# acids-ircam/RAVE

Measured on AMD Instinct MI355X. Metric: audio samples/sec/GPU (RAVE v2 training step, 44.1 kHz, n_signal=65536), higher is better.
Workload: dtype f32; 1 GPU; v2 config, batch 32 mono 44.1 kHz n_signal=65536, VAE-phase training step per GPU (--phase vae); global_batch=32, parallelism=dp1, phase=vae

## Files before the change

include/rave_hip.h:

```cpp
#ifndef RAVE_HIP_H
#define RAVE_HIP_H

#include <stddef.h>
#include <stdint.h>

#ifdef __cplusplus
extern "C" {
#endif

#define RH_VERSION 100

#define RH_OK 0
#define RH_ERR_INVALID (-1)
#define RH_ERR_UNSUPPORTED (-2)
#define RH_ERR_WORKSPACE (-3)

typedef void* rh_stream_t;

enum rh_act {
    RH_ACT_NONE = 0,
    RH_ACT_LEAKY = 1,
    RH_ACT_SNAKE = 2
};

typedef struct rh_conv1d_desc {
    int32_t batch;
    int32_t c_in;
    int32_t c_out;
    int32_t l_in;
    int32_t l_out;
    int32_t kernel;
    int32_t stride;
    int32_t dilation;
    int32_t pad_left;
    int32_t transposed;
    int32_t groups;
    int32_t inner;
    int32_t in_valid;
    int32_t act;
    float act_slope;
    int32_t out_act;
    float out_slope;
} rh_conv1d_desc;

int rh_version(void);
const char* rh_last_error(void);



int rh_weight_norm_fwd_f32(const float* v, const float* g, int64_t rows, int64_t cols, float* w,
                           float* norms, rh_stream_t stream);
int rh_weight_norm_bwd_f32(const float* dw, const float* v, const float* g, const float* norms,
                           int64_t rows, int64_t cols, float* dv, float* dg, rh_stream_t stream);
typedef struct rh_wn_bwd_item {
    const float* dw;
    const float* v;
    const float* g;
    const float* norms;
    float* dv;
    float* dg;
    int64_t rows;
    int64_t cols;
} rh_wn_bwd_item;
int rh_weight_norm_bwd_batched_f32(const rh_wn_bwd_item* items, int32_t n_items, rh_stream_t stream);
typedef struct rh_reduce_item {
    const float* part;
    float* out;
    int64_t n;
    int32_t Z;
    int32_t reserved;
} rh_reduce_item;
int rh_defer_reduce(rh_reduce_item* item);
int rh_reduce_partials_batched_f32(const rh_reduce_item* items, int32_t n_items, rh_stream_t stream);

int64_t rh_conv1d_packed_floats(const rh_conv1d_desc* d, int which);
int rh_conv1d_pack_f32(const rh_conv1d_desc* d, const float* w, float* wp_fwd, float* wp_bwd,
                       rh_stream_t stream);

int rh_conv1d_pack_wn_f32(const rh_conv1d_desc* d, const float* v, const float* g, float* norms,
                          float* scale, float* wp_fwd, float* wp_bwd, rh_stream_t stream);

int64_t rh_prep_item_bytes(void);
int64_t rh_prep_array_bytes(int32_t n);
int rh_prep_fill_item(const rh_conv1d_desc* d, const float* v, const float* g, float* norms, float* scale,
                      float* wp_fwd, float* wp_bwd, void* item_host);
int rh_prep_link(void* items_host, int32_t n, int64_t* total_rows, int64_t* total_blocks);
int rh_prep_run_f32(const void* items_dev, int32_t n, int64_t total_rows, int64_t total_blocks, rh_stream_t stream);


int rh_conv1d_fwd_f32(const rh_conv1d_desc* d, const float* x, const float* wp_fwd,
                      const float* bias, const float* snake_alpha, const float* residual,
                      float* y, void* workspace, int64_t workspace_bytes, rh_stream_t stream);
int64_t rh_conv1d_fwd_workspace_bytes(const rh_conv1d_desc* d);
int64_t rh_conv1d_bwd_data_workspace_bytes(const rh_conv1d_desc* d);
int rh_conv1d_kernel_family(const rh_conv1d_desc* d, int which, int has_bias, int has_add);
int rh_residual_unit_fused(const rh_conv1d_desc* d3, const rh_conv1d_desc* d1);
int rh_residual_unit_fwd_f32(const rh_conv1d_desc* d3, const rh_conv1d_desc* d1, const float* x, const float* wp3_fwd,
                             const float* wp1_fwd, float* h, float* y, rh_stream_t stream);

int rh_x6_uses_ranges(void);
int rh_x6_range_words(void);
int rh_x6_set_ranges(const uint32_t* in_a, const uint32_t* in_b, uint32_t* out, uint32_t* out2);
int rh_amax_f32(const float* x, int64_t n, uint32_t* slot, rh_stream_t stream);

int rh_conv1d_plan_info(const rh_conv1d_desc* d, int which, int has_bias, int has_add, int32_t* out8);
int rh_conv1d_bwd_weight_kernel_family(const rh_conv1d_desc* d);
int rh_conv1d_bwd_weight_plan_info(const rh_conv1d_desc* d, int32_t* out4);

int rh_conv1d_bwd_data_f32(const rh_conv1d_desc* d, const float* dy, const float* wp_bwd,
                           const float* x, const float* snake_alpha, const float* add, float* dx,
                           void* workspace, int64_t workspace_bytes, rh_stream_t stream);

int64_t rh_conv1d_workspace_bytes(const rh_conv1d_desc* d);
int rh_conv1d_bwd_weight_f32(const rh_conv1d_desc* d, const float* dy, const float* x,
                             const float* snake_alpha, float* dw, float* dbias, void* workspace,
                             int64_t workspace_bytes, rh_stream_t stream);
int rh_conv1d_bwd_weight_wn_f32(const rh_conv1d_desc* d, const float* dy, const float* x, const float* snake_alpha,
                                const float* v, const float* g, const float* norms, float* dw_scratch, float* dv,
                                float* dg, float* dbias, void* workspace, int64_t workspace_bytes, rh_stream_t stream);
int64_t rh_conv1d_bwd_weight_wn_fused_launches(void);


int rh_pqmf_analysis_fwd_f32(const float* x, const float* w, int32_t rows, int32_t t_len,
                             int32_t n_band, int32_t kernel, int32_t pad_left, int32_t n_frames,
                             float* y, rh_stream_t stream);
int rh_pqmf_analysis_bwd_f32(const float* dy, const float* w, int32_t rows, int32_t t_len,
                             int32_t n_band, int32_t kernel, int32_t pad_left, int32_t n_frames,
                             float* dx, rh_stream_t stream);
int rh_pqmf_synthesis_fwd_f32(const float* y, const float* w, int32_t rows, int32_t n_frames,
                              int32_t n_band, int32_t kernel, int32_t pad_left, int32_t n_out,
                              float* x, rh_stream_t stream);
int rh_pqmf_synthesis_bwd_f32(const float* dx, const float* w, int32_t rows, int32_t n_frames,
                              int32_t n_band, int32_t kernel, int32_t pad_left, int32_t n_out,
                              float* dy, rh_stream_t stream);

int rh_pqmf_fold_k1_f32(const float* in, const float* tab, int32_t rows, int32_t t_len, int32_t n_frames, int32_t o0,
                        float scale, float* out, rh_stream_t stream);
int rh_pqmf_fold_k2_f32(const float* in, const float* tab, int32_t rows, int32_t n_frames, int32_t n_out, int32_t dp,
                        float scale, float* out, rh_stream_t stream);


int rh_amp_tanh_fwd_f32(const float* x, int32_t batch, int32_t c, int32_t l, float* y,
                        rh_stream_t stream);
int rh_amp_tanh_bwd_f32(const float* dy, const float* x, int32_t batch, int32_t c, int32_t l,
                        float* dx, rh_stream_t stream);
int rh_act_fwd_f32(const float* x, const float* snake_alpha, int32_t act, float slope,
                   int32_t batch, int32_t c, int32_t l, float* y, rh_stream_t stream);
int64_t rh_snake_bwd_workspace_bytes(int32_t batch, int32_t c);
int rh_snake_bwd_f32(const float* dy, const float* x, const float* alpha, int32_t batch, int32_t c,
                     int32_t l, float* dx, float* dalpha, void* workspace, int64_t workspace_bytes,
                     rh_stream_t stream);
int rh_act_bwd_f32(const float* dy, const float* y, int32_t act, float slope, int64_t n, float* g, rh_stream_t stream);
int64_t rh_act_bwd_bias_workspace_bytes(int32_t M);
int rh_act_bwd_bias_f32(const float* dy, const float* y, int32_t act, float slope, int32_t B, int32_t M, int64_t plane, float* g,
                        float* dbias, void* workspace, int64_t workspace_bytes, rh_stream_t stream);
int rh_adain_stats_update_f32(const float* x, int64_t rows, int32_t l, const float* num_updates, float* mean_buf,
                              float* std_buf, rh_stream_t stream);
int rh_adain_transfer_f32(const float* x, int64_t rows, int32_t l, const float* mean_x, const float* std_x,
                          const float* mean_y, const float* std_y, float* y, rh_stream_t stream);
int rh_avgpool2_fwd_f32(const float* x, int64_t rows, int32_t l_in, float* y, rh_stream_t stream);
int rh_avgpool2_bwd_f32(const float* dy, int64_t rows, int32_t l_in, float* dx, rh_stream_t stream);


typedef struct rh_conv2d_desc {
    int32_t batch;
    int32_t c_in;
    int32_t c_out;
    int32_t h_in, w_in;
    int32_t h_out, w_out;
    int32_t kh, kw;
    int32_t sh, sw;
    int32_t dh, dw;
    int32_t ph, pw;
    int32_t act;
    float act_slope;
} rh_conv2d_desc;

int64_t rh_conv2d_packed_floats(const rh_conv2d_desc* d, int which);
int rh_conv2d_pack_f32(const rh_conv2d_desc* d, const float* w, float* wp_fwd, float* wp_bwd, rh_stream_t stream);
int rh_conv2d_fwd_f32(const rh_conv2d_desc* d, const float* x, const float* wp_fwd, const float* bias ,
                      float* y, rh_stream_t stream);
int rh_conv2d_bwd_data_f32(const rh_conv2d_desc* d, const float* dy, const float* y, const float* wp_bwd, float* dx,
                           rh_stream_t stream);
int rh_conv2d_plan_info(const rh_conv2d_desc* d, int32_t which, int64_t* out);
int rh_conv2d_bwd_weight_kernel_family(const rh_conv2d_desc* d);
int64_t rh_conv2d_workspace_bytes(const rh_conv2d_desc* d);
int rh_conv2d_bwd_weight_f32(const rh_conv2d_desc* d, const float* dy, const float* y, const float* x, float* dw,
                             float* dbias, void* workspace, int64_t workspace_bytes, rh_stream_t stream);


int64_t rh_vq_loss_partials(int64_t n_vectors);
int rh_vq_assign_f32(const float* x, const float* embed, int64_t n_vectors, int32_t dim, int32_t codebook_size,
                     int64_t* indices, float* residual, float* quantized_sum, float* loss_partials, rh_stream_t stream);
int64_t rh_vq_assign_workspace_bytes(int64_t n_vectors, int32_t dim, int32_t codebook_size);
int rh_vq_assign_ws_f32(const float* x, const float* embed, int64_t n_vectors, int32_t dim, int32_t codebook_size,
                        int64_t* indices, float* residual, float* quantized_sum, float* loss_partials, void* workspace,
                        int64_t workspace_bytes, rh_stream_t stream);
int rh_vq_ema_update_f32(const float* x, const int64_t* indices, int64_t n_vectors, int32_t dim, int32_t codebook_size,
                         float decay, float epsilon, float* cluster_size, float* embed_avg, float* embed,
                         rh_stream_t stream);


int rh_feed_batch_i16_f32(const int16_t* pcm, const int64_t* src_offset, const double* coef, const float* noise,
                          int32_t rows, int32_t n_signal, int32_t bit_depth, float* out, rh_stream_t stream);

typedef struct rh_feed_pitch_row {
    int64_t base;
    int64_t in_point;
    double mean;
    double coef[5];
    int32_t length;
    int32_t up, down;
    int32_t tap_offset;
    int32_t mute;
    int32_t reserved;
} rh_feed_pitch_row;
int rh_feed_batch_pitch_i16_f32(const int16_t* pcm, int64_t pcm_samples, const rh_feed_pitch_row* rows,
                                const rh_feed_pitch_row* rows_dev, const double* taps, int32_t n_taps, const float* noise,
                                int32_t n_rows, int32_t n_signal, int32_t bit_depth, float* out, rh_stream_t stream);


int rh_stft_frame_fwd_f32(const float* x, const float* window, int64_t rows, int32_t t_len, int32_t n_fft,
                          int32_t hop, int32_t n_frames, float* frames, rh_stream_t stream);
int rh_stft_frame_bwd_f32(const float* dframes, const float* window, int64_t rows, int32_t t_len, int32_t n_fft,
                          int32_t hop, int32_t n_frames, float* dx, rh_stream_t stream);
int rh_stft_frame_bwd_acc_f32(const float* dframes, const float* window, int64_t rows, int32_t t_len, int32_t n_fft,
                              int32_t hop, int32_t n_frames, float* dx, int32_t accumulate, rh_stream_t stream);

int64_t rh_spectral_distance_workspace_bytes(void);
int rh_spectral_distance_fwd_f32(const float* sx, const float* sy, int64_t n_complex, float eps, float* sums,
                                 void* workspace, int64_t workspace_bytes, rh_stream_t stream);
int rh_spectral_distance_bwd_f32(const float* sx, const float* sy, const float* sums, const float* grad_out,
                                 int64_t n_complex, float eps, float* dsx, float* dsy, int32_t half_bins,
                                 rh_stream_t stream);

int rh_spectral_total_f32(const float* sums, const float* inv_n, int32_t n_scales, float* out, rh_stream_t stream);

int rh_stft_loss_supported(int32_t n_fft, int32_t hop, int32_t t_len, int64_t rows);
int rh_stft_loss_plan_info(int32_t n_fft, int32_t t_len, int64_t rows, int64_t* out6);
int64_t rh_stft_loss_workspace_bytes(int32_t n_fft, int32_t t_len, int64_t rows);
int rh_stft_loss_fwd_f32(const float* x, const float* y, const float* window, const float* twiddle, int64_t rows,
                         int32_t t_len, int32_t n_fft, float eps, float* sums, void* workspace, int64_t workspace_bytes,
                         rh_stream_t stream);
int rh_stft_loss_finalize_all_f32(const float* const* partials, const int64_t* partial_bytes, int32_t n_scales,
                                  const float* inv_n, float* sums, float* total, rh_stream_t stream);
int rh_stft_loss_bwd_f32(const float* x, const float* y, const float* window, const float* twiddle, int64_t rows,
                         int32_t t_len, int32_t n_fft, float eps, const float* sums, const float* grad_out, float* dx,
                         float* dy, int32_t accumulate, rh_stream_t stream);

int rh_set_kernel_events(void* start_event, void* stop_event);
int rh_kernel_events_used(void);
int rh_event_create(void** event);
int rh_event_destroy(void* event);
int rh_event_elapsed_ms(void* start_event, void* stop_event, float* ms);

typedef struct rh_loss_item {
    const float* value;
    const float* w1_dev;
    float w1;
    float w2;
} rh_loss_item;
int rh_loss_combine_fwd_f32(const rh_loss_item* items, int32_t n_items, float* scaled, float* total, rh_stream_t stream);
int rh_loss_combine_bwd_f32(const rh_loss_item* items, int32_t n_items, const float* grad_total, float* grads,
                            rh_stream_t stream);

typedef struct rh_adam_item {
    float* p;
    const float* g;
    float* m;
    float* v;
    int64_t n;
    float* step;
} rh_adam_item;
int rh_adam_step_f32(const rh_adam_item* items, int32_t n_items, const float* lr, float beta1, float beta2, float eps,
                     float* aux, rh_stream_t stream);

typedef struct rh_pair_item {
    float* a;
    float* b;
    int64_t n;
} rh_pair_item;
int rh_ema_update_f32(const rh_pair_item* items, int32_t n_items, double factor, rh_stream_t stream);
int rh_swap_f32(const rh_pair_item* items, int32_t n_items, rh_stream_t stream);

typedef struct rh_fm_item {
    const float* f;
    float* df;
    int64_t half;
    float w;
} rh_fm_item;
int64_t rh_feature_matching_workspace_bytes(const rh_fm_item* items, int32_t n_items);
int rh_feature_matching_fwd_f32(const rh_fm_item* items, int32_t n_items, int32_t relative, void* workspace,
                                int64_t workspace_bytes, float* sums, float* out, rh_stream_t stream);
int rh_feature_matching_bwd_f32(const rh_fm_item* items, int32_t n_items, int32_t relative, const float* sums,
                                const float* grad_out, rh_stream_t stream);

int64_t rh_reparam_workspace_bytes(void);
int rh_reparam_fwd_f32(const float* z, const float* eps, int32_t batch, int32_t c, int32_t l, float* zs, float* kl,
                       void* workspace, int64_t workspace_bytes, rh_stream_t stream);
int rh_reparam_bwd_f32(const float* z, const float* eps, const float* dzs, const float* dkl, int32_t batch, int32_t c,
                       int32_t l, float* dz, rh_stream_t stream);

#ifdef __cplusplus
}
#endif
#endif
```

rave_amd/_lib.py:

```python
from __future__ import annotations

import ctypes as C
import os

import torch

_HERE = os.path.dirname(os.path.abspath(__file__))
LIB_PATH = os.environ.get("RAVE_HIP_LIB") or os.path.join(_HERE, "librave_hip.so")

ACT_NONE, ACT_LEAKY, ACT_SNAKE = 0, 1, 2


class ConvDesc(C.Structure):
    _fields_ = [
        ("batch", C.c_int32), ("c_in", C.c_int32), ("c_out", C.c_int32),
        ("l_in", C.c_int32), ("l_out", C.c_int32), ("kernel", C.c_int32),
        ("stride", C.c_int32), ("dilation", C.c_int32), ("pad_left", C.c_int32),
        ("transposed", C.c_int32), ("groups", C.c_int32), ("inner", C.c_int32),
        ("in_valid", C.c_int32), ("act", C.c_int32), ("act_slope", C.c_float),
        ("out_act", C.c_int32), ("out_slope", C.c_float),
    ]


class AdamItem(C.Structure):
    _fields_ = [("p", C.c_void_p), ("g", C.c_void_p), ("m", C.c_void_p), ("v", C.c_void_p), ("n", C.c_int64), ("step", C.c_void_p)]


class PairItem(C.Structure):
    _fields_ = [("a", C.c_void_p), ("b", C.c_void_p), ("n", C.c_int64)]


class WnBwdItem(C.Structure):
    _fields_ = [("dw", C.c_void_p), ("v", C.c_void_p), ("g", C.c_void_p), ("norms", C.c_void_p), ("dv", C.c_void_p),
                ("dg", C.c_void_p), ("rows", C.c_int64), ("cols", C.c_int64)]


class ReduceItem(C.Structure):
    _fields_ = [("part", C.c_void_p), ("out", C.c_void_p), ("n", C.c_int64), ("Z", C.c_int32), ("reserved", C.c_int32)]


class LossItem(C.Structure):
    _fields_ = [("value", C.c_void_p), ("w1_dev", C.c_void_p), ("w1", C.c_float), ("w2", C.c_float)]


class FmItem(C.Structure):
    _fields_ = [("f", C.c_void_p), ("df", C.c_void_p), ("half", C.c_int64), ("w", C.c_float)]


class Conv2dDesc(C.Structure):
    _fields_ = [(n, C.c_int32) for n in (
        "batch", "c_in", "c_out", "h_in", "w_in", "h_out", "w_out", "kh", "kw", "sh", "sw", "dh", "dw", "ph", "pw",
        "act")] + [("act_slope", C.c_float)]


def _load() -> C.CDLL:
    if not os.path.exists(LIB_PATH):
        raise RuntimeError(
            f"rave_amd: {LIB_PATH} not found. Build it with `python -m rave_amd.build` "
            "(or __graft_entry__.build()). There is no CPU / PyTorch fallback for the HIP hot path.")
    lib = C.CDLL(LIB_PATH)
    P, I32, I64, F = C.c_void_p, C.c_int32, C.c_int64, C.c_float
    D = C.POINTER(ConvDesc)
    D2 = C.POINTER(Conv2dDesc)
    sig = {
        "rh_version": ([], C.c_int),
        "rh_last_error": ([], C.c_char_p),
        "rh_weight_norm_fwd_f32": ([P, P, I64, I64, P, P, P], C.c_int),
        "rh_weight_norm_bwd_f32": ([P, P, P, P, I64, I64, P, P, P], C.c_int),
        "rh_weight_norm_bwd_batched_f32": ([C.POINTER(WnBwdItem), I32, P], C.c_int),
        "rh_defer_reduce": ([C.POINTER(ReduceItem)], C.c_int),
        "rh_reduce_partials_batched_f32": ([C.POINTER(ReduceItem), I32, P], C.c_int),
        "rh_conv1d_packed_floats": ([D, C.c_int], I64),
        "rh_conv1d_pack_f32": ([D, P, P, P, P], C.c_int),
        "rh_conv1d_pack_wn_f32": ([D, P, P, P, P, P, P, P], C.c_int),
        "rh_prep_item_bytes": ([], I64),
        "rh_prep_array_bytes": ([I32], I64),
        "rh_prep_fill_item": ([D, P, P, P, P, P, P, P], C.c_int),
        "rh_prep_link": ([P, I32, C.POINTER(I64), C.POINTER(I64)], C.c_int),
        "rh_prep_run_f32": ([P, I32, I64, I64, P], C.c_int),
        "rh_conv1d_fwd_f32": ([D, P, P, P, P, P, P, P, I64, P], C.c_int),
        "rh_conv1d_bwd_data_f32": ([D, P, P, P, P, P, P, P, I64, P], C.c_int),
        "rh_conv1d_kernel_family": ([D, C.c_int, C.c_int, C.c_int], C.c_int),
        "rh_conv1d_bwd_weight_kernel_family": ([D], C.c_int),
        "rh_conv1d_bwd_weight_plan_info": ([D, C.POINTER(C.c_int32)], C.c_int),
        "rh_residual_unit_fused": ([D, D], C.c_int),
        "rh_residual_unit_fwd_f32": ([D, D, P, P, P, P, P, P], C.c_int),
        "rh_conv1d_plan_info": ([D, C.c_int, C.c_int, C.c_int, C.POINTER(C.c_int32)], C.c_int),
        "rh_conv1d_fwd_workspace_bytes": ([D], I64),
        "rh_conv1d_bwd_data_workspace_bytes": ([D], I64),
        "rh_conv1d_workspace_bytes": ([D], I64),
        "rh_conv1d_bwd_weight_f32": ([D, P, P, P, P, P, P, I64, P], C.c_int),
        "rh_conv1d_bwd_weight_wn_f32": ([D, P, P, P, P, P, P, P, P, P, P, P, I64, P], C.c_int),
        "rh_conv1d_bwd_weight_wn_fused_launches": ([], I64),
        "rh_conv2d_packed_floats": ([D2, C.c_int], I64),
        "rh_conv2d_pack_f32": ([D2, P, P, P, P], C.c_int),
        "rh_conv2d_fwd_f32": ([D2, P, P, P, P, P], C.c_int),
        "rh_conv2d_bwd_data_f32": ([D2, P, P, P, P, P], C.c_int),
        "rh_conv2d_workspace_bytes": ([D2], I64),
        "rh_conv2d_plan_info": ([D2, I32, C.POINTER(I64)], C.c_int),
        "rh_conv2d_bwd_weight_kernel_family": ([D2], C.c_int),
        "rh_conv2d_bwd_weight_f32": ([D2, P, P, P, P, P, P, I64, P], C.c_int),
        "rh_feed_batch_i16_f32": ([P, P, P, P, I32, I32, I32, P, P], C.c_int),
        "rh_feed_batch_pitch_i16_f32": ([P, I64, P, P, P, I32, P, I32, I32, I32, P, P], C.c_int),
        "rh_vq_loss_partials": ([I64], I64),
        "rh_vq_assign_f32": ([P, P, I64, I32, I32, P, P, P, P, P], C.c_int),
        "rh_vq_assign_workspace_bytes": ([I64, I32, I32], I64),
        "rh_vq_assign_ws_f32": ([P, P, I64, I32, I32, P, P, P, P, P, I64, P], C.c_int),
        "rh_vq_ema_update_f32": ([P, P, I64, I32, I32, F, F, P, P, P, P], C.c_int),
        "rh_pqmf_analysis_fwd_f32": ([P, P, I32, I32, I32, I32, I32, I32, P, P], C.c_int),
        "rh_pqmf_analysis_bwd_f32": ([P, P, I32, I32, I32, I32, I32, I32, P, P], C.c_int),
        "rh_pqmf_synthesis_fwd_f32": ([P, P, I32, I32, I32, I32, I32, I32, P, P], C.c_int),
        "rh_pqmf_synthesis_bwd_f32": ([P, P, I32, I32, I32, I32, I32, I32, P, P], C.c_int),
        "rh_pqmf_fold_k1_f32": ([P, P, I32, I32, I32, I32, F, P, P], C.c_int),
        "rh_pqmf_fold_k2_f32": ([P, P, I32, I32, I32, I32, F, P, P], C.c_int),
        "rh_amp_tanh_fwd_f32": ([P, I32, I32, I32, P, P], C.c_int),
        "rh_amp_tanh_bwd_f32": ([P, P, I32, I32, I32, P, P], C.c_int),
        "rh_act_fwd_f32": ([P, P, I32, F, I32, I32, I32, P, P], C.c_int),
        "rh_act_bwd_f32": ([P, P, I32, F, I64, P, P], C.c_int),
        "rh_act_bwd_bias_workspace_bytes": ([I32], I64),
        "rh_act_bwd_bias_f32": ([P, P, I32, F, I32, I32, I64, P, P, P, I64, P], C.c_int),
        "rh_snake_bwd_workspace_bytes": ([I32, I32], I64),
        "rh_snake_bwd_f32": ([P, P, P, I32, I32, I32, P, P, P, I64, P], C.c_int),
        "rh_stft_frame_fwd_f32": ([P, P, I64, I32, I32, I32, I32, P, P], C.c_int),
        "rh_stft_frame_bwd_f32": ([P, P, I64, I32, I32, I32, I32, P, P], C.c_int),
        "rh_stft_frame_bwd_acc_f32": ([P, P, I64, I32, I32, I32, I32, P, I32, P], C.c_int),
        "rh_spectral_total_f32": ([P, P, I32, P, P], C.c_int),
        "rh_feature_matching_workspace_bytes": ([C.POINTER(FmItem), I32], I64),
        "rh_feature_matching_fwd_f32": ([C.POINTER(FmItem), I32, I32, P, I64, P, P, P], C.c_int),
        "rh_feature_matching_bwd_f32": ([C.POINTER(FmItem), I32, I32, P, P, P], C.c_int),
        "rh_reparam_workspace_bytes": ([], I64),
        "rh_reparam_fwd_f32": ([P, P, I32, I32, I32, P, P, P, I64, P], C.c_int),
        "rh_reparam_bwd_f32": ([P, P, P, P, I32, I32, I32, P, P], C.c_int),
        "rh_loss_combine_fwd_f32": ([C.POINTER(LossItem), I32, P, P, P], C.c_int),
        "rh_loss_combine_bwd_f32": ([C.POINTER(LossItem), I32, P, P, P], C.c_int),
        "rh_adam_step_f32": ([C.POINTER(AdamItem), I32, P, F, F, F, P, P], C.c_int),
        "rh_ema_update_f32": ([C.POINTER(PairItem), I32, C.c_double, P], C.c_int),
        "rh_swap_f32": ([C.POINTER(PairItem), I32, P], C.c_int),
        "rh_x6_uses_ranges": ([], C.c_int),
        "rh_x6_range_words": ([], C.c_int),
        "rh_x6_set_ranges": ([P, P, P, P], C.c_int),
        "rh_amax_f32": ([P, I64, P, P], C.c_int),
        "rh_set_kernel_events": ([P, P], C.c_int),
        "rh_kernel_events_used": ([], C.c_int),
        "rh_event_create": ([C.POINTER(C.c_void_p)], C.c_int),
        "rh_event_destroy": ([P], C.c_int),
        "rh_event_elapsed_ms": ([P, P, C.POINTER(C.c_float)], C.c_int),
        "rh_stft_loss_supported": ([I32, I32, I32, I64], C.c_int),
        "rh_stft_loss_plan_info": ([I32, I32, I64, C.POINTER(I64)], C.c_int),
        "rh_stft_loss_workspace_bytes": ([I32, I32, I64], I64),
        "rh_stft_loss_fwd_f32": ([P, P, P, P, I64, I32, I32, F, P, P, I64, P], C.c_int),
        "rh_stft_loss_finalize_all_f32": ([C.POINTER(C.c_void_p), C.POINTER(I64), I32, P, P, P, P], C.c_int),
        "rh_stft_loss_bwd_f32": ([P, P, P, P, I64, I32, I32, F, P, P, P, P, I32, P], C.c_int),
        "rh_spectral_distance_workspace_bytes": ([], I64),
        "rh_spectral_distance_fwd_f32": ([P, P, I64, F, P, P, I64, P], C.c_int),
        "rh_spectral_distance_bwd_f32": ([P, P, P, P, I64, F, P, P, I32, P], C.c_int),
        "rh_adain_stats_update_f32": ([P, I64, I32, P, P, P, P], C.c_int),
        "rh_adain_transfer_f32": ([P, I64, I32, P, P, P, P, P, P], C.c_int),
        "rh_avgpool2_fwd_f32": ([P, I64, I32, P, P], C.c_int),
        "rh_avgpool2_bwd_f32": ([P, I64, I32, P, P], C.c_int),
    }
    for name, (args, res) in sig.items():
        fn = getattr(lib, name)
        fn.argtypes = args
        fn.restype = res
    return lib


lib = _load()


def check(rc: int, what: str = "") -> None:
    if rc != 0:
        msg = lib.rh_last_error().decode(errors="replace")
        raise RuntimeError(f"librave_hip {what} failed (code {rc}): {msg}")


def ptr(t) -> int | None:
    return None if t is None else t.data_ptr()


def stream() -> int:
    return torch.cuda.current_stream().cuda_stream
```

rave_amd/csrc/conv_host.hip:

```cpp
#include "conv_params.hpp"

int64_t rh_wgrad_workspace(const rh_conv1d_desc* d);

namespace {

struct TapPlan {
    int nphase = 0;
    int oph[kMaxPhases], ntaps[kMaxPhases], tap0[kMaxPhases], minoff[kMaxPhases], maxoff[kMaxPhases];
    int nslots = 0;
    int kk[kMaxTaps], off[kMaxTaps];
    int is = 1, os = 1;
    int rows = 0;
    int C = 0, M = 0;
    bool src_m_major = true;
};

int validate(const rh_conv1d_desc* d) {
    RH_REQUIRE(d, RH_ERR_INVALID, "conv1d: null descriptor");
    RH_REQUIRE(d->batch >= 0 && d->c_in > 0 && d->c_out > 0 && d->l_in >= 0 && d->l_out >= 0,
               RH_ERR_INVALID, "conv1d: bad sizes");
    RH_REQUIRE(d->kernel >= 1 && d->stride >= 1 && d->dilation >= 1 && d->inner >= 1,
               RH_ERR_INVALID, "conv1d: kernel/stride/dilation/inner must be >= 1");
    RH_REQUIRE(d->groups == 1, RH_ERR_UNSUPPORTED, "conv1d: groups = %d not implemented", d->groups);
    RH_REQUIRE(d->kernel <= kMaxTaps, RH_ERR_UNSUPPORTED, "conv1d: kernel %d > %d", d->kernel, kMaxTaps);
// ... 506 lines not shown
    p->ncols = t.rows * d->inner;
    p->in_act = RH_ACT_NONE;
    p->in_slope = 0.f;
    p->epi_act = d->act;
    p->epi_slope = d->act_slope;
    p->out_act = RH_ACT_NONE;
    p->out_slope = 0.f;
    plan_to_x6(t, d->inner, p);
    return RH_OK;
}

extern "C" int64_t rh_conv1d_packed_floats(const rh_conv1d_desc* d, int which) {
    if (validate(d)) return -1;
    const int64_t M = which == 0 ? d->c_out : d->c_in;
    const int64_t C = which == 0 ? d->c_in : d->c_out;
    const int64_t n32 = (int64_t)d->kernel * C * round32((int)M);
    TapPlan t;
    if (build_plan(d, which, &t)) return -1;
    const long units = x6_units(t, x6_mode_of(t, d->inner), nullptr, d->inner);
    return (units > 0 && units * 4 < 0x7fffffffl) ? n32 + units * 4 + 4 : n32;
}

extern "C" int rh_conv1d_pack_f32(const rh_conv1d_desc* d, const float* w, float* wp_fwd,
                                  float* wp_bwd, rh_stream_t stream) {
    if (int e = validate(d)) return e;
    RH_REQUIRE(w, RH_ERR_INVALID, "conv1d_pack: null weight");
    return pack_both(d, w, nullptr, wp_fwd, wp_bwd, (hipStream_t)stream);
}

int rh_weight_norm_scales(const float* v, const float* g, int64_t rows, int64_t cols, float* norms, float* scale,
                          hipStream_t stream);

struct PrepItem {
    const float* v;
    const float* g;
    float* norms;
    float* scale;
    PackP fwd, bwd;
    long rows, cols;
    long row_begin;
    long blk_begin;
};

namespace {

__device__ __forceinline__ int find_item(const PrepItem* items, int n, long key, bool rows) {
    const long* tab = reinterpret_cast<const long*>(items + n) + (rows ? 0 : n);
    int lo = 0, hi = n - 1;
    while (lo < hi) {
        const int mid = (lo + hi + 1) >> 1;
        if (tab[mid] <= key) lo = mid; else hi = mid - 1;
    }
    return lo;
}

__global__ __launch_bounds__(256) void prep_range_kernel(const PrepItem* __restrict__ items, int n) {
    __shared__ float red[8];
    const PrepItem& p = items[blockIdx.x];
    float mx = 0.f, l1 = 0.f;
    for (long r = threadIdx.x; r < p.rows; r += 256) { mx = fmaxf(mx, p.scale[p.rows + r]); l1 = fmaxf(l1, p.scale[2 * p.rows + r]); }
#pragma unroll
    for (int o = 32; o > 0; o >>= 1) { mx = fmaxf(mx, __shfl_down(mx, o, 64)); l1 = fmaxf(l1, __shfl_down(l1, o, 64)); }
    if ((threadIdx.x & 63) == 0) { red[threadIdx.x >> 6] = mx; red[4 + (threadIdx.x >> 6)] = l1; }
    __syncthreads();
    if (threadIdx.x == 0) {
        const unsigned m = __float_as_uint(fmaxf(fmaxf(red[0], red[1]), fmaxf(red[2], red[3])));
        const unsigned l = __float_as_uint(fmaxf(fmaxf(red[4], red[5]), fmaxf(red[6], red[7])));
        for (unsigned* r : {p.fwd.range, p.bwd.range})
            if (r) { r[0] = m; r[1] = l; r[2] = 0u; r[3] = 0u; }
    }
}

__global__ __launch_bounds__(256) void prep_scales_kernel(const PrepItem* __restrict__ items, int n) {
    __shared__ float red[12];
    const int it = find_item(items, n, blockIdx.x, true);
    const PrepItem& p = items[it];
    const long r = (long)blockIdx.x - p.row_begin;
    const float* vr = p.v + r * p.cols;
    float s = 0.f, mx = 0.f, sm = 0.f;
    long e = threadIdx.x;
    for (; e + 768 < p.cols; e += 1024) {
        const float a0 = vr[e], a1 = vr[e + 256], a2 = vr[e + 512], a3 = vr[e + 768];
        s += a0 * a0; s += a1 * a1; s += a2 * a2; s += a3 * a3;
        mx = fmaxf(fmaxf(mx, fmaxf(fabsf(a0), fabsf(a1))), fmaxf(fabsf(a2), fabsf(a3)));
        sm += fabsf(a0); sm += fabsf(a1); sm += fabsf(a2); sm += fabsf(a3);
    }
    for (; e < p.cols; e += 256) {
        const float a = vr[e];
        s += a * a;
        mx = fmaxf(mx, fabsf(a));
        sm += fabsf(a);
    }
#pragma unroll
    for (int o = 32; o > 0; o >>= 1) {
        s += __shfl_down(s, o, 64);
        mx = fmaxf(mx, __shfl_down(mx, o, 64));
        sm += __shfl_down(sm, o, 64);
    }
    if ((threadIdx.x & 63) == 0) { red[threadIdx.x >> 6] = s; red[4 + (threadIdx.x >> 6)] = mx; red[8 + (threadIdx.x >> 6)] = sm; }
    __syncthreads();
    if (threadIdx.x == 0) {
        const float norm = sqrtf(red[0] + red[1] + red[2] + red[3]);
        const float sc = p.g[r] / norm;
        p.norms[r] = norm;
        p.scale[r] = sc;
        const float m = fabsf(sc) * fmaxf(fmaxf(red[4], red[5]), fmaxf(red[6], red[7]));
        const float l1 = fabsf(sc) * ((red[8] + red[9]) + (red[10] + red[11]));
        p.scale[p.rows + r] = m;
        p.scale[2 * p.rows + r] = l1;
    }
}

__global__ __launch_bounds__(256) void prep_pack_kernel(const PrepItem* __restrict__ items, int n) {
    __shared__ float lds[kPackSlots * 32 * 33];
    const int it = find_item(items, n, blockIdx.x, false);
    const PrepItem& p = items[it];
    const long t = (long)blockIdx.x - p.blk_begin;
    const long nf = pack_tiles(p.fwd);
    if (t < nf) pack_tile(p.fwd, t, lds);
    else if (t - nf < pack_tiles(p.bwd)) pack_tile(p.bwd, t - nf, lds);
}

}

extern "C" int64_t rh_prep_item_bytes(void) { return (int64_t)sizeof(PrepItem); }
extern "C" int64_t rh_prep_array_bytes(int32_t n) { return (int64_t)n * (int64_t)sizeof(PrepItem) + 2 * (int64_t)n * (int64_t)sizeof(long); }

extern "C" int rh_prep_fill_item(const rh_conv1d_desc* d, const float* v, const float* g, float* norms, float* scale,
                                 float* wp_fwd, float* wp_bwd, void* item) {
    if (int e = validate(d)) return e;
    RH_REQUIRE(v && g && norms && scale && wp_fwd && item, RH_ERR_INVALID, "prep_fill_item: null pointer");
    PrepItem* p = (PrepItem*)item;
    *p = PrepItem{};
    p->v = v; p->g = g; p->norms = norms; p->scale = scale;
    p->rows = d->transposed ? d->c_in : d->c_out;
    p->cols = (long)(d->transposed ? d->c_out : d->c_in) * d->kernel;
    if (int e = fill_pack(d, 0, v, scale, wp_fwd, &p->fwd)) return e;
    if (int e = fill_pack(d, 1, v, scale, wp_bwd, &p->bwd)) return e;
    return RH_OK;
}

extern "C" int rh_prep_link(void* items, int32_t n, int64_t* total_rows, int64_t* total_blocks) {
    RH_REQUIRE(items && total_rows && total_blocks && n >= 0, RH_ERR_INVALID, "prep_link: bad arguments");
    PrepItem* p = (PrepItem*)items;
    long rows = 0, blks = 0;
    for (int i = 0; i < n; ++i) {
        p[i].row_begin = rows;
        p[i].blk_begin = blks;
        rows += p[i].rows;
        for (const PackP* q : {&p[i].fwd, &p[i].bwd}) blks += pack_tiles(*q);
    }
    long* tab = reinterpret_cast<long*>(p + n);
    for (int i = 0; i < n; ++i) { tab[i] = p[i].row_begin; tab[n + i] = p[i].blk_begin; }
    *total_rows = rows;
    *total_blocks = blks;
    return RH_OK;
}

extern "C" int rh_prep_run_f32(const void* items_dev, int32_t n, int64_t total_rows, int64_t total_blocks,
                               rh_stream_t stream) {
    RH_REQUIRE(items_dev && n > 0, RH_ERR_INVALID, "prep_run: bad arguments");
    if (total_rows > 0) {
        hipLaunchKernelGGL(prep_scales_kernel, dim3((unsigned)total_rows), dim3(256), 0, (hipStream_t)stream,
                           (const PrepItem*)items_dev, n);
        if (int e = rh_check_launch("prep_scales")) return e;
        hipLaunchKernelGGL(prep_range_kernel, dim3((unsigned)n), dim3(256), 0, (hipStream_t)stream, (const PrepItem*)items_dev, n);
        if (int e = rh_check_launch("prep_range")) return e;
    }
    if (total_blocks > 0) {
        hipLaunchKernelGGL(prep_pack_kernel, dim3((unsigned)total_blocks), dim3(256), 0, (hipStream_t)stream,
                           (const PrepItem*)items_dev, n);
        return rh_check_launch("prep_pack");
    }
    return RH_OK;
}

extern "C" int rh_conv1d_pack_wn_f32(const rh_conv1d_desc* d, const float* v, const float* g, float* norms,
                                     float* scale, float* wp_fwd, float* wp_bwd, rh_stream_t stream) {
    if (int e = validate(d)) return e;
    RH_REQUIRE(v && g && norms && scale, RH_ERR_INVALID, "conv1d_pack_wn: null pointer");
    const int64_t rows = d->transposed ? d->c_in : d->c_out;
    const int64_t cols = (int64_t)(d->transposed ? d->c_out : d->c_in) * d->kernel;
    if (int e = rh_weight_norm_scales(v, g, rows, cols, norms, scale, (hipStream_t)stream)) return e;
    return pack_both(d, v, scale, wp_fwd, wp_bwd, (hipStream_t)stream);
}

extern "C" int64_t rh_conv1d_fwd_workspace_bytes(const rh_conv1d_desc* d) {
    ConvP p{};
    if (rh_conv_fill_fwd(d, &p)) return -1;
    return rh_conv_splitk_workspace(p);
}

extern "C" int64_t rh_conv1d_bwd_data_workspace_bytes(const rh_conv1d_desc* d) {
    ConvP p{};
    if (rh_conv_fill_dgrad(d, &p)) return -1;
    p.epi_act = d->act;
    return rh_conv_splitk_workspace(p);
}

extern "C" int rh_conv1d_kernel_family(const rh_conv1d_desc* d, int which, int has_bias, int has_add) {
    ConvP p{};
    if (int e = which == 0 ? rh_conv_fill_fwd(d, &p) : rh_conv_fill_dgrad(d, &p)) return e;
    if (which == 0 ? rh_smallc_fwd_eligible(d, has_add != 0) : rh_smallc_dgrad_eligible(d, has_add != 0)) return 2;
    alignas(16) static const float dummy[4] = {0.f, 0.f, 0.f, 0.f};
    p.in = dummy; p.wp = dummy; p.wq = reinterpret_cast<const unsigned*>(dummy);
    p.bias = has_bias ? dummy : nullptr;
    p.add = has_add ? dummy : nullptr;
    p.mul_src = (which == 1 && d->act != RH_ACT_NONE) ? dummy : nullptr;
    if (p.B <= 0 || p.ncols <= 0 || p.M <= 0 || !rh_conv_dma_eligible(p)) return 0;
    return (rh_conv_x6_workspace(p) >= 0 || rh_conv_c2x_query(p)) ? 1 : 0;
}

extern "C" int rh_conv1d_plan_info(const rh_conv1d_desc* d, int which, int has_bias, int has_add, int32_t* out8) {
    RH_REQUIRE(out8, RH_ERR_INVALID, "conv1d_plan_info: null output");
    for (int i = 0; i < 8; ++i) out8[i] = 0;
    ConvP p{};
    if (int e = which == 0 ? rh_conv_fill_fwd(d, &p) : rh_conv_fill_dgrad(d, &p)) return e;
    if (which == 0 ? rh_smallc_fwd_eligible(d, has_add != 0) : rh_smallc_dgrad_eligible(d, has_add != 0)) { out8[0] = 2; return RH_OK; }
    alignas(16) static const float dummy[4] = {0.f, 0.f, 0.f, 0.f};
    p.in = dummy; p.wp = dummy; p.wq = reinterpret_cast<const unsigned*>(dummy);
    p.bias = has_bias ? dummy : nullptr;
    p.add = has_add ? dummy : nullptr;
    p.mul_src = (which == 1 && d->act != RH_ACT_NONE) ? dummy : nullptr;
    if (p.B <= 0 || p.ncols <= 0 || p.M <= 0 || !rh_conv_dma_eligible(p)) return RH_OK;
    int q[7];
    if (rh_conv_x6_plan_query(p, q)) {
        out8[0] = 1;
        for (int i = 0; i < 7; ++i) out8[i + 1] = q[i];
    }
    return RH_OK;
}

extern "C" int rh_conv1d_fwd_f32(const rh_conv1d_desc* d, const float* x, const float* wp_fwd,
                                 const float* bias, const float* snake_alpha, const float* residual,
                                 float* y, void* workspace, int64_t workspace_bytes, rh_stream_t stream) {
    const RhKernelEventsScope events;
    ConvP p{};
    rh_take_ranges(nullptr, &p.in_range, &p.out_range, nullptr);
    const unsigned* const in_range = p.in_range;
    unsigned* const out_range = p.out_range;
    if (int e = rh_conv_fill_fwd(d, &p)) return e;
    p.in_range = in_range; p.out_range = out_range;
    if (d->batch == 0 || d->l_out == 0) return RH_OK;
    RH_REQUIRE(x && wp_fwd && y, RH_ERR_INVALID, "conv1d_fwd: null pointer");
    RH_REQUIRE(d->act != RH_ACT_SNAKE || snake_alpha, RH_ERR_INVALID, "conv1d_fwd: snake needs alpha");
    if (rh_smallc_fwd_eligible(d, residual != nullptr)) {
        return rh_smallc_fwd(d, x, wp_fwd, bias, y, (hipStream_t)stream, p.out_range);
    }
    p.in = x; p.wp = wp_fwd; p.out = y; p.bias = bias; p.add = residual; p.mul_src = nullptr;
    p.wq = reinterpret_cast<const unsigned*>(wp_fwd + p.x6_wofs);
    p.in_alpha = snake_alpha; p.mul_alpha = nullptr;
    return rh_conv_launch(p, (hipStream_t)stream, d->transposed ? "conv_transpose1d_fwd" : "conv1d_fwd", workspace,
                          workspace_bytes);
}

extern "C" int rh_conv1d_bwd_data_f32(const rh_conv1d_desc* d, const float* dy, const float* wp_bwd,
                                      const float* x, const float* snake_alpha, const float* add,
                                      float* dx, void* workspace, int64_t workspace_bytes,
                                      rh_stream_t stream) {
    const RhKernelEventsScope events;
    ConvP p{};
    rh_take_ranges(nullptr, &p.in_range, &p.out_range, nullptr);
    const unsigned* const in_range = p.in_range;
    unsigned* const out_range = p.out_range;
    if (int e = rh_conv_fill_dgrad(d, &p)) return e;
    p.in_range = in_range; p.out_range = out_range;
    if (d->batch == 0 || d->l_in == 0) return RH_OK;
    RH_REQUIRE(dy && wp_bwd && dx, RH_ERR_INVALID, "conv1d_bwd_data: null pointer");
    RH_REQUIRE(d->act == RH_ACT_NONE || x, RH_ERR_INVALID, "conv1d_bwd_data: act needs the forward input");
    RH_REQUIRE(d->act != RH_ACT_SNAKE || snake_alpha, RH_ERR_INVALID, "conv1d_bwd_data: snake needs alpha");
    if (rh_smallc_dgrad_eligible(d, add != nullptr)) {
        TapPlan t;
        if (int e = build_plan(d, 1, &t)) return e;
        int slot_of_tap[kMaxTaps];
        for (int i = 0; i < t.nslots; ++i) slot_of_tap[t.kk[i]] = i;
        if (int e = rh_smallc_dgrad(d, dy, wp_bwd, slot_of_tap, dx, (hipStream_t)stream)) return e;
        p.out = dx;
        return rh_range_after(p, (hipStream_t)stream);
    }
    p.in = dy; p.wp = wp_bwd; p.out = dx; p.bias = nullptr; p.add = add;
    p.wq = reinterpret_cast<const unsigned*>(wp_bwd + p.x6_wofs);
    p.mul_src = d->act == RH_ACT_NONE ? nullptr : x;
    p.in_alpha = nullptr; p.mul_alpha = snake_alpha;
    return rh_conv_launch(p, (hipStream_t)stream, d->transposed ? "conv_transpose1d_bwd_data" : "conv1d_bwd_data",
                          workspace, workspace_bytes);
}

extern "C" int64_t rh_conv1d_workspace_bytes(const rh_conv1d_desc* d) {
    if (validate(d)) return -1;
    return rh_wgrad_workspace(d);
}

extern "C" int rh_conv1d_bwd_weight_f32(const rh_conv1d_desc* d, const float* dy, const float* x,
                                        const float* snake_alpha, float* dw, float* dbias,
                                        void* workspace, int64_t workspace_bytes, rh_stream_t stream) {
    const RhKernelEventsScope events;
    const RhWgradArmed armed = rh_wgrad_take_armed(true);
    if (int e = validate(d)) return e;
    RH_REQUIRE(dw && (d->batch == 0 || (dy && x)), RH_ERR_INVALID, "conv1d_bwd_weight: null pointer");
    RH_REQUIRE(d->act != RH_ACT_SNAKE || snake_alpha, RH_ERR_INVALID, "conv1d_bwd_weight: snake needs alpha");
    return rh_wgrad_run(d, dy, x, snake_alpha, dw, dbias, workspace, workspace_bytes, (hipStream_t)stream, armed);
}

extern "C" int rh_conv1d_bwd_weight_wn_f32(const rh_conv1d_desc* d, const float* dy, const float* x, const float* snake_alpha,
                                           const float* v, const float* g, const float* norms, float* dw_scratch, float* dv,
                                           float* dg, float* dbias, void* workspace, int64_t workspace_bytes, rh_stream_t stream) {
    const RhKernelEventsScope events;
    const RhWgradArmed armed = rh_wgrad_take_armed(false);
    if (int e = validate(d)) return e;
    RH_REQUIRE(dw_scratch && v && g && norms && dv && dg && (d->batch == 0 || (dy && x)), RH_ERR_INVALID,
               "conv1d_bwd_weight_wn: null pointer");
    RH_REQUIRE(d->act != RH_ACT_SNAKE || snake_alpha, RH_ERR_INVALID, "conv1d_bwd_weight_wn: snake needs alpha");
    const RhWnTail tail{v, g, norms, dv, dg};
    return rh_wgrad_run(d, dy, x, snake_alpha, dw_scratch, dbias, workspace, workspace_bytes, (hipStream_t)stream, armed, &tail);
}
```

rave_amd/csrc/conv_params.hpp:

```cpp
#pragma once
#include "common.hpp"

constexpr int kMaxPhases = 8;
constexpr int kMaxTaps = 64;

struct ConvP {
    const float* in;
    const float* wp;
    float* out;
    const float* bias;
    const float* mul_src;
    const float* add;
    const float* in_alpha;
    const float* mul_alpha;
    int B, C, M, Mp;
    int in_row, in_valid, out_row, out_valid;
    int ncols, inner, is, os;
    int bnl, bnl_shift, nb, tiles_per_b;
    int pitch;
    int ck;
    int wlds_floats;
    int in_act, epi_act, out_act;
    float in_slope, epi_slope, out_slope;
    int segs;
    unsigned magic_segs, magic_ck, magic_lpr;
    int stage_floats;
    int ksplit;
    int chunks_per_split;
    float* part;
    unsigned* tickets;
    long part_stride;
    unsigned in_bytes, w_bytes;
    const unsigned* wq;
    unsigned wq_bytes;
    const unsigned* in_range;
    unsigned* out_range;
    const unsigned* w_range;
    int x6_mode;
    int x6_P;
    int x6_a_units, x6_b_units;
    int x6_nu;
    int v_s;
    long v_q2ofs;
    int vs;
    int Mr;
    int v_o0;
    int v_U, v_b0;
    long ph_q2ofs[kMaxPhases];
    long x6_wofs;
    int nphase;
    int ph_oph[kMaxPhases], ph_ntaps[kMaxPhases], ph_tap0[kMaxPhases], ph_minoff[kMaxPhases],
        ph_maxoff[kMaxPhases];
    long ph_wofs[kMaxPhases];
    int off[kMaxTaps];
};

struct WgradP {
    const float* R;
    const float* S;
    float* out;
    const float* r_alpha;
    const float* s_alpha;
    int B, M, C, T;
    int r_row;
    int s_row, s_valid;
    int inner, is;
    int r_act, s_act;
    float r_slope, s_slope;
    int rk;
    int chunks_per_b;
    int total_chunks;
    int chunks_per_z;
    int pr;
    int ps;
    int nc_max;
    int minoff, maxoff;
    unsigned magic_ps, magic_cpb, magic_pr, magic_lpr_r, magic_lpr_s;
    int vec;
    int r_floats, s_floats;
    int stage_floats;
    unsigned r_bytes, s_bytes;
    int off[kMaxTaps];
};

struct PackP {
    const float* w;
    const float* scale;
    float* wp;
    unsigned* wq;
    unsigned* range;
    long total;
    int C, M, Mp, k;
    int nslots;
    int m_major;
    int x6_mode;
    int x6_nu;
    int bf16x3;
    int x6_vs, x6_U, x6_Mvp, vz_n;
    long x6_vofs;
    int q2j[kMaxTaps], vq2a[kMaxTaps];
    int vz_j[2 * kMaxPhases], vz_u[2 * kMaxPhases];
    int kk[kMaxTaps];
    int q2a[kMaxTaps];
    int q2n[kMaxTaps];
};
int rh_pack_launch(const PackP& a, const PackP& b, hipStream_t stream, const char* what, const float* w = nullptr, long rows = 0,
                   long cols = 0);
int64_t rh_bias_grad_workspace(int M);
int rh_bias_grad_launch(const float* dy, const float* y, float* part, float* db, int B, int M, long plane, int act,
                        float slope, hipStream_t stream, float* g_out = nullptr, unsigned* g_range = nullptr);
int rh_reduce_partials_launch(const float* part, float* out, long n, int Z, hipStream_t stream, const char* what);
struct RhWnTail {
    const float* v;
    const float* g;
    const float* norms;
    float* dv;
    float* dg;
};
struct RhWgradArmed {
    rh_reduce_item* defer;
    const unsigned* dy_range;
    const unsigned* x_range;
};
RhWgradArmed rh_wgrad_take_armed(bool may_defer);
int rh_wgrad_run(const rh_conv1d_desc* d, const float* dy, const float* x, const float* alpha, float* dw, float* dbias, void* ws,
                 int64_t ws_bytes, hipStream_t stream, const RhWgradArmed& armed, const RhWnTail* tail = nullptr);

int rh_conv_fill_fwd(const rh_conv1d_desc* d, ConvP* p);
int rh_conv_fill_dgrad(const rh_conv1d_desc* d, ConvP* p);
int rh_conv_launch(ConvP& p, hipStream_t stream, const char* what, void* ws = nullptr, int64_t ws_bytes = 0);
int rh_conv_launch_sync(ConvP& p, hipStream_t stream, const char* what);
int rh_range_after(const ConvP& p, hipStream_t stream);
int rh_conv_launch_dma(ConvP& p, hipStream_t stream, const char* what, void* ws, int64_t ws_bytes);
bool rh_conv_dma_eligible(const ConvP& p);
int64_t rh_conv_splitk_workspace(ConvP p);
int64_t rh_conv_x6_workspace(ConvP p);
inline int rh_x6_mode(int C, int nphase, int is, int inner, int ntaps0, const int* off, const int* kk) {
    if (is == 1) return (C & 15) == 0 ? 1 : 0;
    if (is == 3) return (nphase == 1 && inner == 1 && (C & 15) == 0) ? 1 : 0;
    if (nphase != 1 || inner != 1 || (is != 2 && is != 4) || (C * is) % 16 != 0) return 0;
    for (int t = 0; t < ntaps0; ++t)
        if (off[t] != off[0] + t || kk[t] != t) return 0;
    return is;
}
inline bool rh_x6_epi_instantiated(int is, int tm, bool leaky, int epi) {
    const int m = epi & 15, v = epi >> 4;
    if (v) {
        if (is != 1 || tm < 2 || v > 2) return false;
        return leaky ? (m == 0 || m == 1 || m == 5) : (m == 0 || m == 1 || m == 2 || m == 4 || m == 5 || m == 6);
    }
    return leaky ? (m == 0 || m == 1 || m == 4 || m == 5) : (m == 0 || m == 1 || m == 2 || m == 4 || m == 5 || m == 6 || m == 9 || m == 13);
}
int rh_conv_launch_x6(ConvP& p, hipStream_t stream, const char* what, void* ws, int64_t ws_bytes, bool* used);
int rh_conv_launch_c2x(ConvP& p, hipStream_t stream, const char* what, bool* used);
bool rh_conv_c2x_query(ConvP p);
bool rh_conv_x6_plan_query(ConvP p, int* out7);

bool rh_smallc_fwd_eligible(const rh_conv1d_desc* d, bool has_residual);
int rh_smallc_fwd(const rh_conv1d_desc* d, const float* x, const float* wp_fwd, const float* bias, float* y, hipStream_t stream,
                  unsigned* out_range = nullptr);
bool rh_smallc_dgrad_eligible(const rh_conv1d_desc* d, bool has_add);
int rh_smallc_dgrad(const rh_conv1d_desc* d, const float* dy, const float* wp_bwd, const int* slot_of_tap, float* dx,
                    hipStream_t stream);
bool rh_smallc_wgrad_eligible(const rh_conv1d_desc* d);
int64_t rh_smallc_wgrad_workspace(const rh_conv1d_desc* d);
int rh_smallc_wgrad(const rh_conv1d_desc* d, const float* dy, const float* x, float* dw, float* dbias, void* ws,
                    hipStream_t stream);
```

rave_amd/csrc/conv_wgrad.hip:

```cpp
#include <atomic>
#include <cstdlib>
#include <mutex>
#include "conv_params.hpp"

namespace {

template <int TM, int TN, int WM, int WN>
__global__ __launch_bounds__(WM* WN * 64) void wgrad_kernel(const WgradP p) {
    constexpr int BM = TM * WM * 32, BN = TN * WN * 32;
    constexpr int NW = WM * WN;
    extern __shared__ __attribute__((aligned(16))) float smem[];
    float* r_lds = smem;
    float* s_lds = smem + BM * p.pr;

    const int tid = threadIdx.x, lane = tid & 63, wave = tid >> 6;
    const int j = lane & 31, kh = lane >> 5;
    const int wm = wave / WN, wn = wave - wm * WN;
    const int m0 = blockIdx.y * BM, col0 = blockIdx.x * BN, z = blockIdx.z;
    const int ncols = p.C * p.T;
    const int inner = p.inner, is = p.is;
    const int c_lo = col0 / p.T;

    int sb[TN], ar[TM];
#pragma unroll
// ... 378 lines not shown
        const int lo = q0 * is + p.minoff;
        const bool interior = (q0 + p.rk <= r_rows) && lo >= 0 && lo + 4 * ((s_width + 3) >> 2) <= p.s_valid;
        if (!interior) { issue(ch, stage); return; }
        const unsigned rbase = (b * p.M) * (unsigned)p.r_row + (unsigned)q0;
        const unsigned sbase = (b * p.C) * (unsigned)p.s_row + (unsigned)lo;
        float* ss = stage + p.r_floats;
#pragma unroll
        for (int i = 0; i < kNI; ++i) {
            if (i < ni_r && (wave + NW * i) * 256 < p.r_floats) {
                const unsigned off = rc[i] == kOOB ? kOOB : (rbase + rc[i]) * 4u;
                __builtin_amdgcn_raw_ptr_buffer_load_lds(r_rsrc, (lds_void*)(stage + (wave + NW * i) * 256), 16, off, 0, 0, 0);
            }
        }
#pragma unroll
        for (int i = 0; i < kNI; ++i) {
            if (i < ni_s && (wave + NW * i) * 256 < p.s_floats) {
                const unsigned off = sc[i] == kOOB ? kOOB : (sbase + sc[i]) * 4u;
                __builtin_amdgcn_raw_ptr_buffer_load_lds(s_rsrc, (lds_void*)(ss + (wave + NW * i) * 256), 16, off, 0, 0, 0);
            }
        }
    };

    const int ch0 = z * p.chunks_per_z;
    const int nch = min(p.chunks_per_z, p.total_chunks - ch0);
    if (nch > 0) issue_any(ch0, smem);
    for (int i = 0; i < nch; ++i) {
        asm volatile("s_waitcnt vmcnt(0)" ::: "memory");
        __syncthreads();
        if (i + 1 < nch) issue_any(ch0 + i + 1, smem + ((i + 1) & 1) * p.stage_floats);
        const float* r_lds = smem + (i & 1) * p.stage_floats;
        const float* s_lds = r_lds + p.r_floats;
        for (int w = 0; w < inner; ++w) {
            const float* rl = r_lds + w;
            const float* sl = s_lds + w;
            int rr = 0;
            if (p.vec) {
                for (; rr + 8 <= p.rk; rr += 8) {
                    f32x4 a4[TM];
                    float bb[4][TN];
#pragma unroll
                    for (int tm = 0; tm < TM; ++tm)
                        a4[tm] = *reinterpret_cast<const f32x4*>(rl + ar[tm] - kh + rr + 4 * kh);
#pragma unroll
                    for (int u = 0; u < 4; ++u)
#pragma unroll
                        for (int tn = 0; tn < TN; ++tn) bb[u][tn] = sl[sb[tn] - kh * is + (rr + 4 * kh + u) * is];
                    __builtin_amdgcn_sched_barrier(0);
#pragma unroll
                    for (int u = 0; u < 4; ++u) {
#pragma unroll
                        for (int tn = 0; tn < TN; ++tn)
                            if (SLEAKY) bb[u][tn] = bb[u][tn] > 0.f ? bb[u][tn] : bb[u][tn] * p.s_slope;
#pragma unroll
                        for (int tm = 0; tm < TM; ++tm) {
                            float av = a4[tm][u];
                            if (RLEAKY) av = av > 0.f ? av : av * p.r_slope;
#pragma unroll
                            for (int tn = 0; tn < TN; ++tn)
                                acc[tm][tn] = __builtin_amdgcn_mfma_f32_32x32x2f32(av, bb[u][tn], acc[tm][tn], 0, 0, 0);
                        }
                    }
                    __builtin_amdgcn_sched_barrier(0);
                }
            }
            for (; rr + 8 <= p.rk; rr += 8) {
                float a[4][TM], bb[4][TN];
#pragma unroll
                for (int u = 0; u < 4; ++u) {
#pragma unroll
                    for (int tm = 0; tm < TM; ++tm) a[u][tm] = rl[ar[tm] + (rr + 2 * u) * inner];
#pragma unroll
                    for (int tn = 0; tn < TN; ++tn) bb[u][tn] = sl[sb[tn] + (rr + 2 * u) * is * inner];
                }
                __builtin_amdgcn_sched_barrier(0);
#pragma unroll
                for (int u = 0; u < 4; ++u) {
#pragma unroll
                    for (int tm = 0; tm < TM; ++tm)
                        if (RLEAKY) a[u][tm] = a[u][tm] > 0.f ? a[u][tm] : a[u][tm] * p.r_slope;
#pragma unroll
                    for (int tn = 0; tn < TN; ++tn)
                        if (SLEAKY) bb[u][tn] = bb[u][tn] > 0.f ? bb[u][tn] : bb[u][tn] * p.s_slope;
#pragma unroll
                    for (int tm = 0; tm < TM; ++tm)
#pragma unroll
                        for (int tn = 0; tn < TN; ++tn)
                            acc[tm][tn] = __builtin_amdgcn_mfma_f32_32x32x2f32(a[u][tm], bb[u][tn], acc[tm][tn], 0, 0, 0);
                }
                __builtin_amdgcn_sched_barrier(0);
            }
            for (; rr < p.rk; rr += 2) {
                float a[TM], bb[TN];
#pragma unroll
                for (int tm = 0; tm < TM; ++tm) {
                    float v = rl[ar[tm] + rr * inner];
                    if (RLEAKY) v = v > 0.f ? v : v * p.r_slope;
                    a[tm] = v;
                }
#pragma unroll
                for (int tn = 0; tn < TN; ++tn) {
                    float v = sl[sb[tn] + rr * is * inner];
                    if (SLEAKY) v = v > 0.f ? v : v * p.s_slope;
                    bb[tn] = v;
                }
#pragma unroll
                for (int tm = 0; tm < TM; ++tm)
#pragma unroll
                    for (int tn = 0; tn < TN; ++tn)
                        acc[tm][tn] = __builtin_amdgcn_mfma_f32_32x32x2f32(a[tm], bb[tn], acc[tm][tn], 0, 0, 0);
            }
        }
    }
    float* out = p.out + (long)z * p.M * ncols;
#pragma unroll
    for (int tn = 0; tn < TN; ++tn) {
        const int col = col0 + (wn * TN + tn) * 32 + j;
        if (col >= ncols) continue;
#pragma unroll
        for (int tm = 0; tm < TM; ++tm)
#pragma unroll
            for (int r = 0; r < 16; ++r) {
                const int m = m0 + (wm * TM + tm) * 32 + (r & 3) + 8 * (r >> 2) + 4 * kh;
                if (m < p.M) out[(long)m * ncols + col] = acc[tm][tn][r];
            }
    }
}

struct WPlan {
    int bm, bn, mt, ct, Z, rk, chunks_per_b, total_chunks, chunks_per_z;
};

void fill(const rh_conv1d_desc* d, WgradP* p) {
    const int k = d->kernel;
    p->B = d->batch;
    p->T = k;
    p->inner = d->inner;
    p->is = d->stride;
    const int x_valid = d->in_valid ? d->in_valid : d->l_in * d->inner;
    if (!d->transposed) {
        p->M = d->c_out; p->C = d->c_in;
        p->r_row = d->l_out * d->inner;
        p->s_row = x_valid; p->s_valid = x_valid;
        p->r_act = RH_ACT_NONE; p->s_act = d->act;
        p->r_slope = 0.f; p->s_slope = d->act_slope;
        for (int t = 0; t < k; ++t) p->off[t] = t * d->dilation - d->pad_left;
    } else {
        p->M = d->c_in; p->C = d->c_out;
        p->r_row = d->l_in;
        p->s_row = d->l_out; p->s_valid = d->l_out;
        p->r_act = d->act; p->s_act = RH_ACT_NONE;
        p->r_slope = d->act_slope; p->s_slope = 0.f;
        for (int t = 0; t < k; ++t) p->off[t] = t - d->pad_left;
    }
    int lo = p->off[0], hi = p->off[0];
    for (int t = 1; t < k; ++t) { lo = lo < p->off[t] ? lo : p->off[t]; hi = hi > p->off[t] ? hi : p->off[t]; }
    p->minoff = lo; p->maxoff = hi;
}

void tile_of(int M, int ncols, int* bm, int* bn) {
    if (M <= 32) { *bm = 32; *bn = 256; }
    else if (M <= 64) { *bm = 64; *bn = 128; }
    else if (M % 96 == 0 || M < 96) {
        *bm = 96;
        *bn = (ncols % 96 == 0 && ncols % 128 != 0) ? 96 : 128;
    }
    else { *bm = 128; *bn = 128; }
}

WPlan plan(const WgradP& p) {
    WPlan w{};
    tile_of(p.M, p.C * p.T, &w.bm, &w.bn);
    w.mt = rh_cdiv(p.M, w.bm);
    w.ct = rh_cdiv(p.C * p.T, w.bn);
    static const int rk_env = [] { const char* e = getenv("RH_WGRAD_RK"); return e ? atoi(e) : 0; }();
    static const int rk_inner_env = [] { const char* e = getenv("RH_WGRAD_RK_INNER"); return e ? atoi(e) : 0; }();
    int rk = ((rk_env > 0 ? rk_env : 32) / p.inner) & ~1;
    if (p.inner > 1) rk = ((rk_inner_env > 0 ? rk_inner_env : 32) / p.inner) & ~1;
    if (rk < 2) rk = 2;
    const int r_rows = p.r_row / p.inner;
    if (r_rows < rk) rk = (r_rows + 1) & ~1;
    if (rk < 2) rk = 2;
    w.rk = rk;
    w.chunks_per_b = rh_cdiv(r_rows, rk);
    w.total_chunks = p.B * w.chunks_per_b;
    static const int ztarget = [] { const char* e = getenv("RH_WGRAD_BLOCKS"); return e ? atoi(e) : 1024; }();
    static const int zmin_chunks = [] { const char* e = getenv("RH_WGRAD_MINCHUNKS"); return e ? atoi(e) : 16; }();
    int Z = ztarget / (w.mt * w.ct);
    const int zmax = w.total_chunks / (rk * p.inner >= 64 ? zmin_chunks / 2 : zmin_chunks);
    if (Z > zmax) Z = zmax;
    if (Z < 1) Z = 1;
    w.chunks_per_z = rh_cdiv(w.total_chunks, Z);
    w.Z = rh_cdiv(w.total_chunks, w.chunks_per_z);
    if (w.Z < 1) w.Z = 1;
    return w;
}

inline unsigned magic_of(int d) { return d <= 1 ? 0u : (unsigned)(((1ull << 32) + d - 1) / (unsigned long long)d); }

template <int TM, int TN, int WM, int WN>
int launch_w(WgradP& p, const WPlan& w, hipStream_t stream) {
    constexpr int BM = TM * WM * 32, BN = TN * WN * 32;
    p.rk = w.rk;
    p.chunks_per_b = w.chunks_per_b;
    p.total_chunks = w.total_chunks;
    p.chunks_per_z = w.chunks_per_z;
    {
        const unsigned long long rb = 4ull * p.B * p.M * (unsigned long long)p.r_row;
        const unsigned long long sbytes = 4ull * p.B * p.C * (unsigned long long)p.s_row;
        const bool ok = p.r_act != RH_ACT_SNAKE && p.s_act != RH_ACT_SNAKE && rb < 0x7fffffffull &&
                        sbytes < 0x7fffffffull && w.rk * p.inner <= 64 && w.total_chunks < 32768;
        if (ok) {
            p.nc_max = (BN - 1) / p.T + 2;
            if (p.nc_max > p.C) p.nc_max = p.C;
            const int s_width = ((w.rk - 1) * p.is + (p.maxoff - p.minoff) + 1) * p.inner;
            static const int novec = [] { const char* e = getenv("RH_WGRAD_NOVEC"); return e ? atoi(e) : 0; }();
            p.vec = !novec && p.inner == 1 && (w.rk % 4) == 0 && (p.r_row % 4) == 0 && (p.s_row % 4) == 0 &&
                    ((uintptr_t)p.R % 16) == 0 && ((uintptr_t)p.S % 16) == 0;
            if (p.vec) {
                p.pr = w.rk + 4;
                p.ps = ((s_width + 3) & ~3) + 4;
                if ((p.ps & 31) == 0) p.ps += 4;
                const int ni_r = rh_cdiv(BM * (p.pr >> 2), 64 * WM * WN);
                const int ni_s = rh_cdiv(p.nc_max * (p.ps >> 2), 64 * WM * WN);
                if (ni_r > 12 || ni_s > 12) p.vec = 0;
            }
            if (!p.vec) {
                p.ps = s_width | 1;
                p.pr = (w.rk * p.inner) | 1;
            }
            p.magic_pr = magic_of(p.pr);
            p.magic_lpr_r = magic_of(p.pr >> 2);
            p.magic_lpr_s = magic_of(p.ps >> 2);
            p.r_floats = (BM * p.pr + 255) & ~255;
            p.s_floats = (p.nc_max * p.ps + 255) & ~255;
            p.stage_floats = p.r_floats + p.s_floats;
            p.magic_ps = magic_of(p.ps);
            p.magic_cpb = magic_of(w.chunks_per_b);
            p.r_bytes = (unsigned)rb;
            p.s_bytes = (unsigned)sbytes;
            const size_t lds = sizeof(float) * 2 * (size_t)p.stage_floats;
            if (lds <= 160 * 1024 && (unsigned)p.s_floats < (1u << 15)) {
                dim3 grid(w.ct, w.mt, w.Z);
                auto go = [&](auto kern) {
                    static std::once_flag once;
                    std::call_once(once, [&] { (void)hipFuncSetAttribute(reinterpret_cast<const void*>(kern), hipFuncAttributeMaxDynamicSharedMemorySize, 160 * 1024); });
                    rh_launch_main(kern, grid, dim3(WM * WN * 64), lds, stream, p);
                };
                if (p.r_act == RH_ACT_LEAKY) go(wgrad_dma_kernel<TM, TN, WM, WN, true, false>);
                else if (p.s_act == RH_ACT_LEAKY) go(wgrad_dma_kernel<TM, TN, WM, WN, false, true>);
                else go(wgrad_dma_kernel<TM, TN, WM, WN, false, false>);
                return rh_check_launch("conv1d_bwd_weight(dma)");
            }
        }
    }
    p.pr = (w.rk * p.inner) | 1;
    p.ps = (((w.rk - 1) * p.is + (p.maxoff - p.minoff) + 1) * p.inner) | 1;
    p.nc_max = (BN - 1) / p.T + 2;
    if (p.nc_max > p.C) p.nc_max = p.C;
    const size_t lds = sizeof(float) * ((size_t)BM * p.pr + (size_t)p.nc_max * p.ps);
    RH_REQUIRE(lds <= 160 * 1024, RH_ERR_UNSUPPORTED, "conv1d_bwd_weight: tile needs %zu B of LDS", lds);
    auto kern = wgrad_kernel<TM, TN, WM, WN>;
    static std::once_flag once;
    std::call_once(once, [&] {
        (void)hipFuncSetAttribute(reinterpret_cast<const void*>(kern),
                                  hipFuncAttributeMaxDynamicSharedMemorySize, 160 * 1024);
    });
    dim3 grid(w.ct, w.mt, w.Z);
    rh_launch_main(kern, grid, dim3(WM * WN * 64), lds, stream, p);
    return rh_check_launch("conv1d_bwd_weight");
}

}

int64_t rh_wgrad_x6_workspace(const WgradP& w);
int rh_wgrad_x6_launch(const WgradP& w, float* dw, float* rsum_out, void* ws, hipStream_t stream, bool* used, int* left_z,
                       const unsigned* r_range, const unsigned* s_range);
int rh_reduce_wn_bwd_launch(const float* part, int Z, long M, long N, const float* v, const float* g, const float* norms,
                            float* dv, float* dg, hipStream_t stream, bool* used);

extern "C" int rh_conv1d_bwd_weight_kernel_family(const rh_conv1d_desc* d) {
    if (!d || d->batch <= 0) return 0;
    WgradP p{};
    fill(d, &p);
    if (rh_smallc_wgrad_eligible(d)) return 2;
    alignas(16) static const float dummy[4] = {0.f, 0.f, 0.f, 0.f};
    p.R = dummy; p.S = dummy;
    return d->act != RH_ACT_SNAKE && rh_wgrad_x6_workspace(p) >= 0 ? 1 : 0;
}

bool rh_wgrad_x6_plan_info(const WgradP& w, int32_t* out4);

extern "C" int rh_conv1d_bwd_weight_plan_info(const rh_conv1d_desc* d, int32_t* out4) {
    if (!d || !out4) return RH_ERR_INVALID;
    for (int i = 0; i < 4; ++i) out4[i] = 0;
    if (d->batch <= 0 || rh_conv1d_bwd_weight_kernel_family(d) != 1) return RH_OK;
    WgradP p{};
    fill(d, &p);
    alignas(16) static const float dummy[4] = {0.f, 0.f, 0.f, 0.f};
    p.R = dummy; p.S = dummy;
    (void)rh_wgrad_x6_plan_info(p, out4);
    return RH_OK;
}

int64_t rh_wgrad_workspace(const rh_conv1d_desc* d) {
    WgradP p{};
    fill(d, &p);
    const int64_t bias = rh_bias_grad_workspace(d->c_out);
    if (rh_smallc_wgrad_eligible(d)) return bias + rh_smallc_wgrad_workspace(d);
    int64_t x6 = -1;
    if (d->act != RH_ACT_SNAKE) {
        x6 = rh_wgrad_x6_workspace(p);
        if (x6 >= 0 && !RH_X6_F16) return bias + x6;
    }
    const WPlan w = plan(p);
    const int64_t f32 = w.Z <= 1 ? 0 : (int64_t)w.Z * p.M * p.C * p.T * (int64_t)sizeof(float);
    return bias + (x6 > f32 ? x6 : f32);
}

extern "C" int rh_weight_norm_bwd_f32(const float* dw, const float* v, const float* g, const float* norms, int64_t rows,
                                      int64_t cols, float* dv, float* dg, rh_stream_t stream);

thread_local rh_reduce_item* g_defer_item = nullptr;
extern "C" int rh_defer_reduce(rh_reduce_item* item) {
    g_defer_item = item;
    if (item) *item = rh_reduce_item{};
    return RH_OK;
}

extern "C" int rh_reduce_partials_batched_f32(const rh_reduce_item* items, int32_t n_items, rh_stream_t stream) {
    RH_REQUIRE(n_items >= 0 && (n_items == 0 || items), RH_ERR_INVALID, "reduce_partials_batched: bad arguments");
    for (int i0 = 0; i0 < n_items; i0 += kReduceBatch) {
        ReduceTable tb{};
        long blocks = 0;
        for (int i = i0; i < n_items && i < i0 + kReduceBatch; ++i) {
            const rh_reduce_item& q = items[i];
            if (q.Z <= 0 || q.n <= 0) continue;
            RH_REQUIRE(q.part && q.out, RH_ERR_INVALID, "reduce_partials_batched: null pointer in item %d", i);
            const int k = tb.items++;
            tb.part[k] = q.part; tb.out[k] = q.out; tb.Z[k] = q.Z;
            tb.vec4[k] = reduce_is_vec4(q.part, q.out, q.n, q.Z) ? 1 : 0;
            tb.n[k] = tb.vec4[k] ? q.n / 4 : q.n;
            tb.blk_begin[k] = blocks;
            blocks += tb.vec4[k] ? rh_cdiv64(tb.n[k], 256) : rh_cdiv64(q.n, 64);
        }
        if (tb.items == 0) continue;
        tb.blk_begin[tb.items] = blocks;
        RH_REQUIRE(blocks < 0x7fffffffl, RH_ERR_UNSUPPORTED, "reduce_partials_batched: too many workgroups");
        hipLaunchKernelGGL(reduce_partials_batched_kernel, dim3((unsigned)blocks), dim3(256), 0, (hipStream_t)stream, tb);
        if (int e = rh_check_launch("reduce_partials_batched")) return e;
    }
    return RH_OK;
}

RhWgradArmed rh_wgrad_take_armed(bool may_defer) {
    RhWgradArmed a{may_defer ? g_defer_item : nullptr, nullptr, nullptr};
    g_defer_item = nullptr;
    rh_take_ranges(&a.dy_range, &a.x_range, nullptr, nullptr);
    return a;
}

int rh_wgrad_run(const rh_conv1d_desc* d, const float* dy, const float* x, const float* alpha,
                 float* dw, float* dbias, void* ws, int64_t ws_bytes, hipStream_t stream, const RhWgradArmed& armed,
                 const RhWnTail* tail) {
    rh_reduce_item* const defer = tail ? nullptr : armed.defer;
    WgradP p{};
    fill(d, &p);
    const unsigned* const dy_range = armed.dy_range;
    const unsigned* const x_range = armed.x_range;
    const bool have_ranges = !RH_X6_F16 || (dy_range && x_range);
    auto through_dw = [&](int e) {
        if (e || !tail) return e;
        return rh_weight_norm_bwd_f32(dw, tail->v, tail->g, tail->norms, p.M, (int64_t)p.C * p.T, tail->dv, tail->dg, (rh_stream_t)stream);
    };
    if (!d->transposed) { p.R = dy; p.S = x; p.r_alpha = nullptr; p.s_alpha = alpha; }
    else                { p.R = x; p.S = dy; p.r_alpha = alpha; p.s_alpha = nullptr; }
    const long nw = (long)p.M * p.C * p.T;
    const int64_t bias_ws = rh_bias_grad_workspace(d->c_out);
    if (rh_smallc_wgrad_eligible(d)) {
        const int64_t need = rh_smallc_wgrad_workspace(d);
        RH_REQUIRE(ws && ws_bytes >= need, RH_ERR_WORKSPACE, "conv1d_bwd_weight: workspace %lld B < %lld B",
                   (long long)ws_bytes, (long long)need);
        return through_dw(rh_smallc_wgrad(d, dy, x, dw, dbias, ws, stream));
    }
    const bool x6_path = have_ranges && d->act != RH_ACT_SNAKE && p.B > 0 && p.r_row > 0 && rh_wgrad_x6_workspace(p) >= 0;
    const bool fuse_bias = x6_path && !d->transposed && dbias != nullptr;
    if (dbias && d->batch > 0 && !fuse_bias) {
        RH_REQUIRE(ws && ws_bytes >= bias_ws, RH_ERR_WORKSPACE, "conv1d_bwd_weight: workspace %lld B < %lld B",
                   (long long)ws_bytes, (long long)bias_ws);
        if (int e = rh_bias_grad_launch(dy, nullptr, (float*)ws, dbias, d->batch, d->c_out,
                                        (long)d->l_out * d->inner, RH_ACT_NONE, 0.f, stream))
            return e;
    }
    ws = ws ? (void*)((char*)ws + bias_ws) : nullptr;
    ws_bytes = ws_bytes > bias_ws ? ws_bytes - bias_ws : 0;
    if (p.B <= 0 || p.r_row <= 0) {
        (void)hipMemsetAsync(dw, 0, nw * sizeof(float), stream);
        if (dbias) (void)hipMemsetAsync(dbias, 0, d->c_out * sizeof(float), stream);
        return through_dw(RH_OK);
    }
    if (d->act != RH_ACT_SNAKE && have_ranges) {
        const int64_t x6 = rh_wgrad_x6_workspace(p);
        if (x6 >= 0) {
            RH_REQUIRE(x6 == 0 || (ws && ws_bytes >= x6), RH_ERR_WORKSPACE,
                       "conv1d_bwd_weight: workspace %lld B < %lld B", (long long)ws_bytes, (long long)x6);
            bool used = false;
            int left_z = 0;
            if (int e = rh_wgrad_x6_launch(p, dw, fuse_bias ? dbias : nullptr, ws, stream, &used, (tail || defer) ? &left_z : nullptr,
                                           d->transposed ? x_range : dy_range, d->transposed ? dy_range : x_range))
                return e;
            if (used && left_z > 1 && defer) {
                defer->part = (const float*)ws; defer->out = dw; defer->n = nw; defer->Z = left_z;
                return RH_OK;
            }
            if (used && left_z > 1) {
                bool fused = false;
                if (int e = rh_reduce_wn_bwd_launch((const float*)ws, left_z, p.M, (long)p.C * p.T, tail->v, tail->g, tail->norms,
                                                    tail->dv, tail->dg, stream, &fused))
                    return e;
                if (fused) return RH_OK;
                return through_dw(rh_reduce_partials_launch((const float*)ws, dw, nw, left_z, stream, "conv1d_bwd_weight_reduce"));
            }
            if (used) return through_dw(RH_OK);
        }
    }
    const WPlan w = plan(p);
    const int64_t need = w.Z > 1 ? (int64_t)w.Z * nw * (int64_t)sizeof(float) : 0;
    RH_REQUIRE(need == 0 || (ws && ws_bytes >= need), RH_ERR_WORKSPACE,
               "conv1d_bwd_weight: workspace %lld B < %lld B", (long long)ws_bytes, (long long)need);
    p.out = w.Z > 1 ? (float*)ws : dw;
    int e;
    if (w.bm == 32) e = launch_w<1, 2, 1, 4>(p, w, stream);
    else if (w.bm == 64) e = launch_w<2, 1, 1, 4>(p, w, stream);
    else if (w.bm == 96 && w.bn == 96) e = launch_w<3, 1, 1, 3>(p, w, stream);
    else if (w.bm == 96) e = launch_w<3, 1, 1, 4>(p, w, stream);
    else e = launch_w<2, 2, 2, 2>(p, w, stream);
    if (e) return e;
    if (w.Z > 1) {
        if (tail) {
            bool fused = false;
            if (int e2 = rh_reduce_wn_bwd_launch((const float*)ws, w.Z, p.M, nw / p.M, tail->v, tail->g, tail->norms, tail->dv,
                                                 tail->dg, stream, &fused))
                return e2;
            if (fused) return RH_OK;
        }
        if (defer) {
            defer->part = (const float*)ws; defer->out = dw; defer->n = nw; defer->Z = w.Z;
            return RH_OK;
        }
        reduce_partials_go((const float*)ws, dw, nw, w.Z, stream);
        return through_dw(rh_check_launch("conv1d_bwd_weight_reduce"));
    }
    return through_dw(RH_OK);
}

int rh_reduce_partials_launch(const float* part, float* out, long n, int Z, hipStream_t stream, const char* what) {
    if (n <= 0) return RH_OK;
    reduce_partials_go(part, out, n, Z, stream);
    return rh_check_launch(what);
}

static std::atomic<int64_t> g_rwn_launches{0};
int rh_reduce_wn_bwd_launch(const float* part, int Z, long M, long N, const float* v, const float* g, const float* norms,
                            float* dv, float* dg, hipStream_t stream, bool* used) {
    *used = false;
    const char* e = getenv("RH_WN_FUSED");
    if (!(e && atoi(e) == 1)) return RH_OK;
    if (Z < 2 || M <= 0 || N <= 0 || (N & 3) || N > kRwnMaxN || ((uintptr_t)part & 15)) return RH_OK;
    const long n = M * N;
    const int order4 = Z <= 16 && n >= (1l << 16);
    hipLaunchKernelGGL(reduce_wn_bwd_kernel, dim3((unsigned)M), dim3(1024), (size_t)(4096 + N) * sizeof(float), stream, part, n, Z,
                       (int)N, order4, v, g, norms, dv, dg);
    *used = true;
    ++g_rwn_launches;
    return rh_check_launch("conv1d_bwd_weight_reduce_wn");
}

extern "C" int64_t rh_conv1d_bwd_weight_wn_fused_launches(void) { return g_rwn_launches.load(); }

int64_t rh_bias_grad_workspace(int M) { return (int64_t)M * kBiasSlices * (int64_t)sizeof(float); }

int rh_bias_grad_launch(const float* dy, const float* y, float* part, float* db, int B, int M, long plane, int act,
                        float slope, hipStream_t stream, float* g_out, unsigned* g_range) {
    hipLaunchKernelGGL(bias_grad2d_kernel, dim3(M, kBiasSlices), dim3(256), 0, stream, dy, y, part, B, M, plane, act, slope, g_out,
                       g_out ? g_range : nullptr);
    if (int e = rh_check_launch("bias_grad")) return e;
    hipLaunchKernelGGL(bias_grad2d_finalize_kernel, dim3(rh_cdiv(M, 64)), dim3(64), 0, stream, (const float*)part, db, M);
    return rh_check_launch("bias_grad_finalize");
}

extern "C" int64_t rh_act_bwd_bias_workspace_bytes(int32_t M) { return rh_bias_grad_workspace(M); }
extern "C" int rh_act_bwd_bias_f32(const float* dy, const float* y, int32_t act, float slope, int32_t B, int32_t M, int64_t plane,
                                   float* g, float* dbias, void* workspace, int64_t workspace_bytes, rh_stream_t stream) {
    unsigned* g_range = nullptr;
    rh_take_ranges(nullptr, nullptr, &g_range, nullptr);
    RH_REQUIRE(dy && y && g && dbias && B >= 0 && M > 0 && plane > 0, RH_ERR_INVALID, "act_bwd_bias: bad arguments");
    RH_REQUIRE(act == RH_ACT_NONE || act == RH_ACT_LEAKY, RH_ERR_UNSUPPORTED, "act_bwd_bias: activation must be none or leaky");
    RH_REQUIRE(workspace && workspace_bytes >= rh_bias_grad_workspace(M), RH_ERR_WORKSPACE, "act_bwd_bias: workspace too small");
    if (B == 0) return hipMemsetAsync(dbias, 0, (size_t)M * sizeof(float), (hipStream_t)stream) == hipSuccess ? RH_OK : RH_ERR_INVALID;
    return rh_bias_grad_launch(dy, y, (float*)workspace, dbias, B, M, plane, act, slope, (hipStream_t)stream, g, g_range);
}
```

rave_amd/csrc/conv_wgrad_x6.hip:

```cpp
#include <cstdlib>
#include <mutex>
#include <type_traits>
#include "conv_params.hpp"

namespace {

typedef unsigned u32x4 __attribute__((ext_vector_type(4)));
constexpr unsigned kOOB = 0x80000000u;

struct Wx6P {
    const float* R;
    const float* S;
    float* out;
    float* rsum;
    int B, M, C, T, N;
    int r_row, s_row, s_valid, is;
    float r_slope, s_slope;
    int steps_per_b;
    int total_steps, steps_per_z;
    unsigned r_bytes, s_bytes;
    int minoff, maxoff;
    int p8, cpb, chmax;
    int av;
    unsigned b_stage;
    const unsigned* r_range;
    const unsigned* s_range;
    int off[kMaxTaps];
};

typedef u32x4 u32x4_u __attribute__((aligned(2)));

__device__ __forceinline__ void emit(const float (&v)[8], float slope, float sc, u32x4* dst, int piece_stride) {
#if RH_X6_F16
    u32x4 hi, lo;
#pragma unroll
    for (int k = 0; k < 4; ++k) {
        float a = v[2 * k] * sc, b = v[2 * k + 1] * sc;
        a = rh_max1(a, a * slope);
        b = rh_max1(b, b * slope);
        const rh_h2 h = rh_h2_split(a, b);
        hi[k] = h.hi; lo[k] = h.lo;
    }
    dst[0] = hi;
    dst[piece_stride] = lo;
#else
    unsigned h[3][8];
#pragma unroll
    for (int i = 0; i < 8; ++i) {
        const float x = rh_max1(v[i], v[i] * slope);
        rh_bf3_split(x, h[0][i], h[1][i], h[2][i]);
    }
#pragma unroll
    for (int s3 = 0; s3 < 3; ++s3) {
        u32x4 pk;
#pragma unroll
        for (int k = 0; k < 4; ++k) pk[k] = __builtin_amdgcn_perm(h[s3][2 * k + 1], h[s3][2 * k], 0x07060302u);
        dst[s3 * piece_stride] = pk;
    }
#endif
}

constexpr int kKS = 2;
constexpr int kOct = 2 * kKS;
constexpr int kSpan = 16 * kKS;

constexpr int wx6_gs(int rows) { return kX6P * rows + 4; }
constexpr int wx6_stage(int rows) { return kKS * 2 * wx6_gs(rows); }
constexpr int wx6_slot(int o, int row, int rows) { return (o >> 1) * 2 * wx6_gs(rows) + (o & 1) * wx6_gs(rows) + row; }

struct Wx6Scale { float r, s, out; };
__device__ __forceinline__ Wx6Scale wx6_scales(const Wx6P& p) {
#if RH_X6_F16
    int inv_r, inv_s;
    Wx6Scale sc;
    sc.r = __uint_as_float(rh_x6_scale_bits(rh_range_max(p.r_range), &inv_r));
    sc.s = __uint_as_float(rh_x6_scale_bits(rh_range_max(p.s_range), &inv_s));
    sc.out = __uint_as_float(rh_x6_unscale_bits(inv_r, inv_s));
    return sc;
#else
    return Wx6Scale{1.f, 1.f, 1.f};
#endif
}

struct Wx6Step {
    int n;
    unsigned rs, ss;
    bool r_tail, s_edge;
};
template <bool PL>
__device__ __forceinline__ Wx6Step wx6_step(const Wx6P& p, int st) {
    Wx6Step sp;
    const int b = st / p.steps_per_b;
    sp.n = (st - b * p.steps_per_b) * kSpan;
    sp.rs = (unsigned)((b * p.M * p.r_row + sp.n) * 4);
    sp.ss = (unsigned)((b * p.C * p.s_row + sp.n * p.is) * 4);
    sp.r_tail = sp.n + kSpan > p.r_row;
    sp.s_edge = PL ? (sp.n + p.minoff < 0 || sp.n + p.minoff + 8 * p.p8 > p.s_valid || sp.r_tail)
                   : (sp.n * p.is + p.minoff < 0 || (sp.n + kSpan - 1) * p.is + p.maxoff >= p.s_valid || sp.r_tail);
    return sp;
}

template <int NT, int BM>
struct Wx6RTasks {
    static constexpr int NA = (kOct * BM + NT - 1) / NT;
    unsigned off[NA];
    int dst[NA], pos[NA];
    float v[NA][8];
    float sum[NA];

    __device__ __forceinline__ void init(const Wx6P& p, int tid, int m0) {
#pragma unroll
        for (int q = 0; q < NA; ++q) {
            const int u = tid + NT * q;
            const int o = u % kOct, m = u / kOct;
            const bool ok = m < BM && m0 + m < p.M;
            dst[q] = m < BM ? wx6_slot(o, m, BM) : -1;
            pos[q] = 8 * o;
            off[q] = ok ? (unsigned)(((m0 + m) * p.r_row + 8 * o) * 4) : kOOB;
            sum[q] = 0.f;
#pragma unroll
            for (int i = 0; i < 8; ++i) v[q][i] = 0.f;
        }
    }
    template <class RSRC>
    __device__ __forceinline__ void load(const Wx6P& p, RSRC rsrc, const Wx6Step& sp, bool av) {
#pragma unroll
        for (int q = 0; q < NA; ++q) {
            const unsigned base = off[q] == kOOB ? kOOB : off[q] + sp.rs;
            if (av) {
#pragma unroll
                for (int h = 0; h < 2; ++h) {
                    unsigned o = base == kOOB ? kOOB : base + 16u * h;
                    if (sp.r_tail) o = sp.n + pos[q] + 4 * h < p.r_row ? o : kOOB;
                    const u32x4 x = __builtin_bit_cast(u32x4, __builtin_amdgcn_raw_buffer_load_b128(rsrc, o, 0, 0));
#pragma unroll
                    for (int i = 0; i < 4; ++i) v[q][4 * h + i] = __uint_as_float(x[i]);
                }
            } else {
#pragma unroll
                for (int i = 0; i < 8; ++i) {
                    unsigned o = base == kOOB ? kOOB : base + 4u * i;
                    if (sp.r_tail) o = sp.n + pos[q] + i < p.r_row ? o : kOOB;
                    v[q][i] = __builtin_bit_cast(float, __builtin_amdgcn_raw_buffer_load_b32(rsrc, o, 0, 0));
                }
            }
        }
    }
    __device__ __forceinline__ void add_rows() {
#pragma unroll
        for (int q = 0; q < NA; ++q)
            sum[q] += ((v[q][0] + v[q][1]) + (v[q][2] + v[q][3])) + ((v[q][4] + v[q][5]) + (v[q][6] + v[q][7]));
    }
    __device__ __forceinline__ void store_sums(const Wx6P& p, int tid, int m0, int z) const {
#pragma unroll
        for (int q = 0; q < NA; ++q) {
            float s = sum[q];
            s += __shfl_xor(s, 1, 64);
            s += __shfl_xor(s, 2, 64);
            const int u = tid + NT * q;
            const int m = u / kOct;
            if ((u % kOct) == 0 && m < BM && m0 + m < p.M) p.rsum[(long)z * p.M + m0 + m] = s;
        }
    }
    __device__ __forceinline__ void convert(const Wx6P& p, float sc, u32x4* a_stage) const {
#pragma unroll
        for (int q = 0; q < NA; ++q)
            if (dst[q] >= 0) emit(v[q], p.r_slope, sc, a_stage + dst[q], BM);
    }
};

template <int NT, int NB, int BN, bool PL>
struct Wx6STasks {
    static_assert(PL || NT * NB == kOct * BN, "the (column, octet) tasks fill NB whole rounds");
    unsigned off[NB];
    int dst[NB], p0[NB];
    float v[NB][8];
    int c_lo;
    unsigned piece;

    __device__ __forceinline__ void init(const Wx6P& p, int first, int n0, bool part) {
        c_lo = PL ? n0 / p.T : 0;
        const int n_ch = PL ? min(p.N - 1, n0 + BN - 1) / p.T - c_lo + 1 : 0;
        piece = PL ? (unsigned)(p.chmax * p.cpb) : 16u * BN;
#pragma unroll
        for (int q = 0; q < NB; ++q) {
            const int u = first + NT * q;
            if constexpr (PL) {
                const int ch = u / p.p8, o = u - ch * p.p8;
                const bool ok = ch < n_ch;
                dst[q] = ok ? ch * p.cpb + o * 16 : -1;
                p0[q] = p.minoff + 8 * o;
                off[q] = ok ? (unsigned)(((c_lo + ch) * p.s_row + p0[q]) * 4) : kOOB;
            } else {
                const int o = u % kOct, col = u / kOct;
                const int cc = (n0 + col) / p.T, t = (n0 + col) - cc * p.T;
                const bool ok = n0 + col < p.N;
                dst[q] = (ok || !part) ? wx6_slot(o, col, BN) * 16 : -1;
                p0[q] = 8 * o * p.is + (ok ? p.off[t] : 0);
                off[q] = ok ? (unsigned)((cc * p.s_row + p0[q]) * 4) : kOOB;
            }
        }
    }
    __device__ __forceinline__ unsigned column(const Wx6P& p, int n, int tn) const {
        if constexpr (PL) {
            if (n >= p.N) return 0u;
            const int cc = n / p.T, t = n - cc * p.T;
            return (unsigned)((cc - c_lo) * p.cpb + (p.off[t] - p.minoff) * 2);
        } else {
            return 16u * 32u * tn;
        }
    }
    __device__ __forceinline__ static int kblock(int kb, int g, int colj) {
        return PL ? (kb * 16 + g * 8) * 2 : (kb * 2 * wx6_gs(BN) + g * wx6_gs(BN) + colj) * 16;
    }
    template <class RSRC>
    __device__ __forceinline__ void load(const Wx6P& p, RSRC rsrc, const Wx6Step& sp, int nq) {
#pragma unroll
        for (int q = 0; q < NB; ++q) {
            if (q >= nq) continue;
            const unsigned base = off[q] == kOOB ? kOOB : off[q] + sp.ss;
#pragma unroll
            for (int i = 0; i < 8; ++i) {
                unsigned o = base == kOOB ? kOOB : base + 4u * (unsigned)(i * p.is);
                if (sp.s_edge) {
                    const int pos = sp.n * p.is + p0[q] + i * p.is;
                    o = (pos >= 0 && pos < p.s_valid) ? o : kOOB;
                }
                v[q][i] = __builtin_bit_cast(float, __builtin_amdgcn_raw_buffer_load_b32(rsrc, o, 0, 0));
            }
        }
    }
    __device__ __forceinline__ void convert(const Wx6P& p, float sc, unsigned char* b_stage, int nq) const {
#pragma unroll
        for (int q = 0; q < NB; ++q) {
            if (q >= nq || dst[q] < 0) continue;
            emit(v[q], p.s_slope, sc, reinterpret_cast<u32x4*>(b_stage + dst[q]), (int)(piece >> 4));
        }
    }
};

template <int TM, int TN, int BM, bool PL>
__device__ __forceinline__ void wx6_mma(f32x16 (&acc)[TM][TN], const u32x4* al, const unsigned char* bl, const unsigned (&bcol)[TN],
                                        unsigned piece, bool live2) {
    constexpr int SA[RH_X6_NPROD] = RH_X6_SA, SB[RH_X6_NPROD] = RH_X6_SB;
    rh_x6_frag afr[TM][kX6P], bfr[TN][kX6P];
#pragma unroll
    for (int tm = 0; tm < TM; ++tm)
#pragma unroll
        for (int s3 = 0; s3 < kX6P; ++s3) afr[tm][s3] = __builtin_bit_cast(rh_x6_frag, al[s3 * BM + tm * 32]);
#pragma unroll
    for (int tn = 0; tn < TN; ++tn)
#pragma unroll
        for (int s3 = 0; s3 < kX6P; ++s3) {
            const unsigned char* f = bl + bcol[tn] + (unsigned)s3 * piece;
            if constexpr (PL) bfr[tn][s3] = __builtin_bit_cast(rh_x6_frag, *reinterpret_cast<const u32x4_u*>(f));
            else bfr[tn][s3] = __builtin_bit_cast(rh_x6_frag, *reinterpret_cast<const u32x4*>(f));
        }
#pragma unroll
    for (int q = 0; q < RH_X6_NPROD; ++q)
#pragma unroll
        for (int tm = 0; tm < TM; ++tm) {
            acc[tm][0] = RH_X6_MFMA(afr[tm][SA[q]], bfr[0][SB[q]], acc[tm][0]);
            if constexpr (TN == 2) {
                if (live2) acc[tm][1] = RH_X6_MFMA(afr[tm][SA[q]], bfr[1][SB[q]], acc[tm][1]);
            }
        }
}

__device__ __forceinline__ void wx6_store_tile(const Wx6P& p, float* __restrict__ outz, const f32x16& acc, int mb, int col, float osc) {
#pragma unroll
    for (int r = 0; r < 16; ++r) {
        const int m = mb + (r & 3) + 8 * (r >> 2);
        if (m < p.M) outz[(long)m * p.N + col] = RH_X6_F16 ? acc[r] * osc : acc[r];
    }
}

template <int TM, int WM, int WN, bool AV, bool PART, bool PL>
__global__ __launch_bounds__(256, 2) void wgrad_x6_kernel(const Wx6P p) {
    static_assert(WM * WN == 4, "four waves");
    constexpr int NT = 256, BM = 32 * TM * WM, BN = 64 * WN;
    constexpr int NB = PL ? ((BN / 2 + 2) * 7 + NT - 1) / NT : kOct * BN / NT;
    extern __shared__ __attribute__((aligned(16))) unsigned char smem_raw[];
    u32x4* const a_st = reinterpret_cast<u32x4*>(smem_raw);
    unsigned char* const b_st = smem_raw + wx6_stage(BM) * 16;

    const int tid = threadIdx.x, lane = tid & 63;
    const int wave = __builtin_amdgcn_readfirstlane(tid >> 6);
    const int j = lane & 31, g = lane >> 5;
    const int wm = wave / WN, wn = wave - wm * WN;
    const int m0 = blockIdx.y * BM, n0 = blockIdx.x * BN, z = blockIdx.z;

    const auto r_rsrc = __builtin_amdgcn_make_buffer_rsrc(const_cast<float*>(p.R), 0, p.r_bytes, 0x00020000);
    const auto s_rsrc = __builtin_amdgcn_make_buffer_rsrc(const_cast<float*>(p.S), 0, p.s_bytes, 0x00020000);
    const Wx6Scale sc = wx6_scales(p);

    Wx6RTasks<NT, BM> rt;
    Wx6STasks<NT, NB, BN, PL> stk;
    rt.init(p, tid, m0);
    stk.init(p, tid, n0, PART);
    unsigned bcol[2];
#pragma unroll
    for (int tn = 0; tn < 2; ++tn) bcol[tn] = stk.column(p, n0 + wn * 64 + tn * 32 + j, tn);

    f32x16 acc[TM][2];
#pragma unroll
    for (int tm = 0; tm < TM; ++tm)
#pragma unroll
        for (int tn = 0; tn < 2; ++tn)
#pragma unroll
            for (int r = 0; r < 16; ++r) acc[tm][tn][r] = 0.f;

    const bool want_rsum = p.rsum != nullptr && blockIdx.x == 0;
    auto load = [&](int st) {
        const Wx6Step sp = wx6_step<PL>(p, st);
        rt.load(p, r_rsrc, sp, AV);
        stk.load(p, s_rsrc, sp, NB);
    };
    auto convert = [&]() {
        if (want_rsum) rt.add_rows();
        rt.convert(p, sc.r, a_st);
        stk.convert(p, sc.s, b_st, NB);
    };

    const int st0 = z * p.steps_per_z;
    const int nst = min(p.steps_per_z, p.total_steps - st0);
    if (nst > 0) {
        load(st0);
        convert();
    }
    __syncthreads();
    const u32x4* const al = a_st + g * wx6_gs(BM) + wm * TM * 32 + j;
    const int live_tn = !PART ? 2 : (n0 + wn * 64 >= p.N ? 0 : (n0 + wn * 64 + 32 >= p.N ? 1 : 2));
    const bool live1 = live_tn >= 1, live2 = live_tn == 2;
    for (int s = 0; s < nst; ++s) {
        const bool more = s + 1 < nst;
        if (more) load(st0 + s + 1);
        if (live1) {
#pragma unroll
            for (int kb = 0; kb < kKS; ++kb)
                wx6_mma<TM, 2, BM, PL>(acc, al + kb * 2 * wx6_gs(BM), b_st + stk.kblock(kb, g, wn * 64 + j), bcol, stk.piece, live2);
        }
        __syncthreads();
        if (more) convert();
        __syncthreads();
    }

    if (want_rsum) rt.store_sums(p, tid, m0, z);
    float* __restrict__ outz = p.out + (long)z * p.M * p.N;
#pragma unroll
    for (int tn = 0; tn < 2; ++tn) {
        const int col = n0 + wn * 64 + tn * 32 + j;
        if (col >= p.N) continue;
#pragma unroll
        for (int tm = 0; tm < TM; ++tm) wx6_store_tile(p, outz, acc[tm][tn], m0 + (wm * TM + tm) * 32 + 4 * g, col, sc.out);
    }
}

template <int NW, bool PL>
__global__ __launch_bounds__(64 * NW) void wgrad_x6_wide_kernel(const Wx6P p) {
    constexpr int TM = 3, BM = 32 * TM, BN = 32 * NW, NT = 64 * NW;
    constexpr int NB = 2;
    extern __shared__ __attribute__((aligned(16))) unsigned char smem_raw[];
    u32x4* const a_st = reinterpret_cast<u32x4*>(smem_raw);
    unsigned char* const b_st = smem_raw + 2 * wx6_stage(BM) * 16;

    const int tid = threadIdx.x, lane = tid & 63;
    const int wave = __builtin_amdgcn_readfirstlane(tid >> 6);
    const int j = lane & 31, g = lane >> 5;
    const int z = blockIdx.x;

    const auto r_rsrc = __builtin_amdgcn_make_buffer_rsrc(const_cast<float*>(p.R), 0, p.r_bytes, 0x00020000);
    const auto s_rsrc = __builtin_amdgcn_make_buffer_rsrc(const_cast<float*>(p.S), 0, p.s_bytes, 0x00020000);
    const Wx6Scale sc = wx6_scales(p);

    Wx6RTasks<NT, BM> rt;
    Wx6STasks<NT, NB, BN, PL> stk;
    rt.init(p, tid, 0);
    stk.init(p, NT - 1 - tid, 0, true);
    const int nq = PL ? (p.C * p.p8 + NT - 1) / NT : NB;
    const bool r_wave = !(NT > kOct * BM && 64 * wave >= kOct * BM);
    const int col = 32 * wave + j;
    const bool live = 32 * wave < p.N;
    const unsigned bcol[1] = {stk.column(p, col, 0)};

    f32x16 acc[TM][1];
#pragma unroll
    for (int tm = 0; tm < TM; ++tm)
#pragma unroll
        for (int r = 0; r < 16; ++r) acc[tm][0][r] = 0.f;

    const bool want_rsum = p.rsum != nullptr;
    auto load = [&](int st) {
        const Wx6Step sp = wx6_step<PL>(p, st);
        if (r_wave) rt.load(p, r_rsrc, sp, p.av != 0);
        stk.load(p, s_rsrc, sp, nq);
    };
    auto convert = [&](int stage) {
        if (want_rsum) rt.add_rows();
        rt.convert(p, sc.r, a_st + stage * wx6_stage(BM));
        stk.convert(p, sc.s, b_st + stage * p.b_stage, nq);
    };
    auto multiply = [&](int stage) {
        const u32x4* const al = a_st + stage * wx6_stage(BM) + g * wx6_gs(BM) + j;
        const unsigned char* const bs = b_st + stage * p.b_stage;
#pragma unroll
        for (int kb = 0; kb < kKS; ++kb)
            wx6_mma<TM, 1, BM, PL>(acc, al + kb * 2 * wx6_gs(BM), bs + stk.kblock(kb, g, col), bcol, stk.piece, false);
    };

    const int st0 = z * p.steps_per_z;
    const int nst = min(p.steps_per_z, p.total_steps - st0);
    if (nst > 0) {
        load(st0);
        convert(0);
    }
    __syncthreads();
    for (int s = 0; s < nst; ++s) {
        const bool more = s + 1 < nst;
        if (more) load(st0 + s + 1);
        if (live) multiply(s & 1);
        if (more) convert((s + 1) & 1);
        __syncthreads();
    }

    if (want_rsum) rt.store_sums(p, tid, 0, z);
    if (col < p.N) {
        float* __restrict__ outz = p.out + (long)z * p.M * p.N;
#pragma unroll
        for (int tm = 0; tm < TM; ++tm) wx6_store_tile(p, outz, acc[tm][0], tm * 32 + 4 * g, col, sc.out);
    }
}

struct Wx6Plan {
    int tm, wm, rt, ct, Z, steps_per_z;
    int planes;
    int nw;
    int own_z;
    size_t lds;
};

struct Wx6Env {
    bool off;
    int planes;
    int wide;
    int blocks;
    int all;
    int tm;
    bool forced_tm() const { return tm >= 1 && tm <= 3; }
};

Wx6Env read_wx6_env() {
    const auto num = [](const char* name, int dflt) { const char* e = getenv(name); return e ? atoi(e) : dflt; };
    static const int all = num("RH_WGRAD_X6_ALL", 0), tm = num("RH_WGRAD_X6_TM", 0);
    const char* pe = getenv("RH_WGRAD_X6_PLANES");
    return Wx6Env{num("RH_WGRAD_X6", 1) == 0, pe ? (pe[0] == '1' ? 1 : 0) : -1, num("RH_WGRAD_X6_WIDE", 1), num("RH_WGRAD_X6_BLOCKS", 0), all, tm};
}

bool wx6_eligible(const WgradP& w, const Wx6Env& env, const unsigned* r_range, const unsigned* s_range) {
    if (env.off) return false;
    if (RH_X6_F16 && (!r_range || !s_range)) return false;
    if (w.inner != 1 || w.T > kMaxTaps || w.B <= 0 || w.r_row <= 0) return false;
    if ((w.r_act != RH_ACT_NONE && w.r_act != RH_ACT_LEAKY) || (w.s_act != RH_ACT_NONE && w.s_act != RH_ACT_LEAKY)) return false;
    if ((w.r_act == RH_ACT_LEAKY && !(w.r_slope >= 0.f && w.r_slope <= 1.f)) || (w.s_act == RH_ACT_LEAKY && !(w.s_slope >= 0.f && w.s_slope <= 1.f))) return false;
    if (w.M < 32 || (long)w.C * w.T < 64) return false;
    if (!env.all && w.M <= 64 && w.r_row > 1024) return false;
    return 4ull * w.B * w.M * (unsigned long long)w.r_row < 0x7fffffffull && 4ull * w.B * w.C * (unsigned long long)w.s_row < 0x7fffffffull;
}

bool wx6_plane_geometry(const WgradP& w, int chmax, Wx6P* p, size_t* bytes) {
    const int reach = w.maxoff - w.minoff;
    p->p8 = (32 + reach + 7) / 8;
    p->cpb = 16 * ((p->p8 & 1) ? p->p8 : p->p8 + 1);
    p->chmax = chmax;
    *bytes = (size_t)kX6P * chmax * p->cpb + 32;
    return w.is == 1 && w.T >= 2 && reach >= 0 && p->p8 <= 7 && 4l * (w.s_row + 64) * w.C * w.B < 0x7fffffffl;
}

int wx6_choose_tile(const WgradP& w, const Wx6Env& env, Wx6P* p, Wx6Plan* pl) {
    const int Mp = (w.M + 31) & ~31;
    pl->tm = (Mp % 128 == 0 && Mp >= 256 && w.T > 1) ? 2 : (Mp % 96 == 0 ? 3 : (Mp % 64 == 0 ? 2 : 1));
    if (env.forced_tm()) pl->tm = env.tm;
    pl->wm = Mp >= 64 * pl->tm ? 2 : 1;
    const int BM = 32 * pl->tm * pl->wm, BN = 64 * (4 / pl->wm);
    pl->rt = rh_cdiv(w.M, BM);
    pl->ct = rh_cdiv(p->N, BN);
    const int four_wave_tiles = pl->rt * pl->ct;
    pl->nw = 0; pl->own_z = 0;
    size_t plane_bytes;
    if (env.wide != 0 && env.planes < 0 && !env.forced_tm() && w.M > 64 && w.M <= 96 && p->N <= 288) {
        const int tiles = rh_cdiv(p->N, 32);
        pl->nw = tiles <= 3 ? 3 : (tiles <= 4 ? 4 : (tiles <= 6 ? 6 : 9));
        pl->own_z = env.wide != 2;
        pl->tm = 3; pl->wm = 1; pl->rt = 1; pl->ct = 1;
        pl->planes = wx6_plane_geometry(w, w.C, p, &plane_bytes);
        p->av = w.r_row % 4 == 0 && ((uintptr_t)w.R & 15) == 0;
        p->b_stage = (unsigned)(pl->planes ? (plane_bytes + 15) / 16 * 16 : (size_t)wx6_stage(32 * pl->nw) * 16);
        pl->lds = 2 * ((size_t)wx6_stage(96) * 16 + p->b_stage);
    } else {
        const bool on = env.planes >= 0 ? env.planes == 1 : Mp <= 96;
        pl->planes = wx6_plane_geometry(w, BN / w.T + 2, p, &plane_bytes) && on && pl->tm >= 2;
        pl->lds = (size_t)wx6_stage(BM) * 16 + (pl->planes ? plane_bytes : (size_t)wx6_stage(BN) * 16);
    }
    return four_wave_tiles;
}

void wx6_slice_k(const Wx6Env& env, int four_wave_tiles, Wx6P* p, Wx6Plan* pl) {
    const int dflt = pl->nw == 9 && pl->own_z ? 256 : 512;
    const int target = env.blocks > 0 ? env.blocks : (env.blocks < 0 ? (pl->tm == 2 ? 768 : 512) : dflt);
    int Z = rh_cdiv(target, pl->own_z ? 1 : four_wave_tiles);
    const int zmax = p->total_steps / 4 > 0 ? p->total_steps / 4 : 1;
    if (Z > zmax) Z = zmax;
    if (Z < 1) Z = 1;
    pl->steps_per_z = rh_cdiv(p->total_steps, Z);
    pl->Z = rh_cdiv(p->total_steps, pl->steps_per_z);
    p->steps_per_z = pl->steps_per_z;
}

bool plan_wx6(const WgradP& w, Wx6P* p, Wx6Plan* pl, const unsigned* r_range, const unsigned* s_range) {
    const Wx6Env env = read_wx6_env();
    if (!wx6_eligible(w, env, r_range, s_range)) return false;
    *p = Wx6P{};
    p->R = w.R; p->S = w.S;
    p->B = w.B; p->M = w.M; p->C = w.C; p->T = w.T; p->N = w.C * w.T;
    p->r_row = w.r_row; p->s_row = w.s_row; p->s_valid = w.s_valid; p->is = w.is;
    p->r_slope = w.r_act == RH_ACT_LEAKY ? w.r_slope : 1.f;
    p->s_slope = w.s_act == RH_ACT_LEAKY ? w.s_slope : 1.f;
    p->steps_per_b = rh_cdiv(w.r_row, kSpan);
    p->total_steps = w.B * p->steps_per_b;
    p->r_bytes = (unsigned)(4ull * w.B * w.M * w.r_row); p->s_bytes = (unsigned)(4ull * w.B * w.C * w.s_row);
    p->minoff = w.minoff; p->maxoff = w.maxoff;
    p->r_range = r_range; p->s_range = s_range;
    for (int t = 0; t < w.T; ++t) p->off[t] = w.off[t];
    wx6_slice_k(env, wx6_choose_tile(w, env, p, pl), p, pl);
    return true;
}

using Wx6Launch = void (*)(dim3 grid, int threads, size_t lds, hipStream_t stream, const Wx6P& p);

template <void (*KERN)(Wx6P)>
void launch_wx6(dim3 grid, int threads, size_t lds, hipStream_t stream, const Wx6P& p) {
    static std::once_flag once;
    std::call_once(once, [] {
        (void)hipFuncSetAttribute(reinterpret_cast<const void*>(KERN), hipFuncAttributeMaxDynamicSharedMemorySize, 160 * 1024);
    });
    rh_launch_main(KERN, grid, dim3(threads), lds, stream, p);
}

template <int... Vs, class F>
Wx6Launch wx6_pick(int v, F f) {
    Wx6Launch r = nullptr;
    ((v == Vs ? (void)(r = f(std::integral_constant<int, Vs>{})) : (void)0), ...);
    return r;
}

Wx6Launch wx6_instance(const Wx6P& p, const Wx6Plan& pl) {
    if (pl.nw > 0)
        return wx6_pick<3, 4, 6, 9>(pl.nw, [&](auto NW) {
            return wx6_pick<0, 1>(pl.planes, [&](auto PL) -> Wx6Launch { return launch_wx6<wgrad_x6_wide_kernel<decltype(NW)::value, decltype(PL)::value != 0>>; });
        });
    const int av = p.r_row % 4 == 0 && ((uintptr_t)p.R & 15) == 0;
    const int part = rh_cdiv(p.N, 32) % (2 * (4 / pl.wm)) != 0;
    return wx6_pick<1, 2, 3>(pl.tm, [&](auto TM) {
        return wx6_pick<1, 2>(pl.wm, [&](auto WM) {
            return wx6_pick<0, 1>(av, [&](auto AV) {
                return wx6_pick<0, 1>(part, [&](auto PART) {
                    return wx6_pick<0, 1>(pl.planes, [&](auto PL) -> Wx6Launch {
                        constexpr int tm = decltype(TM)::value, wm = decltype(WM)::value;
                        constexpr bool planes = decltype(PL)::value != 0 && tm >= 2;
                        return launch_wx6<wgrad_x6_kernel<tm, wm, 4 / wm, decltype(AV)::value != 0, decltype(PART)::value != 0, planes>>;
                    });
                });
            });
        });
    });
}

}

int64_t rh_wgrad_x6_workspace(const WgradP& w) {
    Wx6P p;
    Wx6Plan pl{};
    static const unsigned any_range[kRangeSlotWords] = {};
    if (!plan_wx6(w, &p, &pl, any_range, any_range)) return -1;
    return (pl.Z > 1 ? (int64_t)pl.Z * w.M * w.C * w.T : 0) * (int64_t)sizeof(float) + (int64_t)pl.Z * w.M * (int64_t)sizeof(float);
}

bool rh_wgrad_x6_plan_info(const WgradP& w, int32_t* out4) {
    Wx6P p;
    Wx6Plan pl{};
    static const unsigned any_range[kRangeSlotWords] = {};
    if (!plan_wx6(w, &p, &pl, any_range, any_range)) return false;
    out4[0] = pl.nw > 0 ? pl.nw : 4;
    out4[1] = pl.rt * pl.ct * pl.Z;
    out4[2] = pl.Z;
    out4[3] = pl.planes;
    return true;
}

int rh_wgrad_x6_launch(const WgradP& w, float* dw, float* rsum_out, void* ws, hipStream_t stream, bool* used, int* left_z,
                       const unsigned* r_range, const unsigned* s_range) {
    *used = false;
    if (left_z) *left_z = 0;
    Wx6P p;
    Wx6Plan pl{};
    if (!plan_wx6(w, &p, &pl, r_range, s_range)) return RH_OK;
    p.out = pl.Z > 1 ? (float*)ws : dw;
    float* const rs_part = (float*)ws + (pl.Z > 1 ? (long)pl.Z * w.M * w.C * w.T : 0);
    p.rsum = rsum_out ? (pl.Z > 1 ? rs_part : rsum_out) : nullptr;
    const dim3 grid = pl.nw > 0 ? dim3(pl.Z) : dim3(pl.ct, pl.rt, pl.Z);
    wx6_instance(p, pl)(grid, pl.nw > 0 ? 64 * pl.nw : 256, pl.lds, stream, p);
    if (int e = rh_check_launch("conv1d_bwd_weight_x6")) return e;
    *used = true;
    if (pl.Z > 1) {
        if (left_z) *left_z = pl.Z;
        else if (int e = rh_reduce_partials_launch((const float*)ws, dw, (long)w.M * w.C * w.T, pl.Z, stream, "conv1d_bwd_weight_reduce")) return e;
        if (rsum_out) return rh_reduce_partials_launch(rs_part, rsum_out, w.M, pl.Z, stream, "conv1d_bwd_bias_reduce");
    }
    return RH_OK;
}
```

rave_amd/ops.py:

```python
from __future__ import annotations

import ctypes as C
import os
from dataclasses import dataclass
from typing import Optional, Tuple

import torch

from . import _lib as L
from ._lib import ACT_LEAKY, ACT_NONE, ACT_SNAKE

Tensor = torch.Tensor


_PROFILE = None
_EVENT_POOL = []


def profile_begin() -> None:
    global _PROFILE
    _PROFILE = []


def _hip_event():
# ... 172 lines not shown

    def out_len(self, l_in: int, k: int) -> int:
        if self.transposed:
            return (l_in - 1) * self.stride - 2 * self.pad_left + k
        return (l_in + self.pad_left + self.pad_right - self.dilation * (k - 1) - 1) // self.stride + 1


def _desc(g: ConvGeom, batch, c_in, c_out, l_in, l_out, k, in_valid=0) -> L.ConvDesc:
    return L.ConvDesc(batch=batch, c_in=c_in, c_out=c_out, l_in=l_in, l_out=l_out, kernel=k,
                      stride=g.stride, dilation=g.dilation, pad_left=g.pad_left,
                      transposed=int(g.transposed), groups=1, inner=g.inner, in_valid=in_valid,
                      act=g.act, act_slope=g.slope, out_act=g.out_act, out_slope=g.out_slope)


def _ws(nbytes: int, device) -> Optional[Tensor]:
    return torch.empty(nbytes // 4, device=device, dtype=torch.float32) if nbytes > 0 else None


_RANGES = L.lib.rh_x6_uses_ranges() == 1
_RANGE_WORDS = L.lib.rh_x6_range_words()
_RANGE_SLOTS = 2048
_RANGE_POOLS = {}


def range_reset(device=None, _exhausted: bool = False) -> None:
    if not _RANGES:
        return
    for dev in ([device] if device is not None else list(_RANGE_POOLS)):
        st = _RANGE_POOLS.get(dev)
        prev = st[0] if st else None
        cur = torch.cuda.current_stream(dev)
        pool = torch.zeros(_RANGE_SLOTS * _RANGE_WORDS, device=dev, dtype=torch.int32)
        if _exhausted:
            ev = torch.cuda.Event()
            ev.record(cur)
            d_ = dev if isinstance(dev, torch.device) else torch.device(dev)
            for other in [st[3] if st else None, _SIDE.get(d_.index if d_.index is not None else torch.cuda.current_device())]:
                if other is not None and other != cur:
                    other.wait_event(ev)
            main = st[3] if st else cur
        else:
            main = cur
        _RANGE_POOLS[dev] = [pool, 0, prev, main, torch.cuda.is_current_stream_capturing()]


def range_capture_end(device=None) -> list:
    out = []
    for dev in ([device] if device is not None else list(_RANGE_POOLS)):
        st = _RANGE_POOLS.get(dev)
        if st is not None and st[4]:
            out += [t for t in (st[0], st[2]) if t is not None]
            del _RANGE_POOLS[dev]
    return out


def _ranges_on() -> bool:
    return _RANGES and os.environ.get("RH_CONV_X6", "1") != "0"


def _new_range(device) -> Tensor:
    st = _RANGE_POOLS.get(device)
    if st is not None and st[4] and not torch.cuda.is_current_stream_capturing():
        range_reset(device)
        st = _RANGE_POOLS[device]
    if st is None or st[1] >= _RANGE_SLOTS:
        range_reset(device, _exhausted=st is not None)
        st = _RANGE_POOLS[device]
    i = st[1]
    st[1] = i + 1
    return st[0][i * _RANGE_WORDS:(i + 1) * _RANGE_WORDS]


def _attach_range(t: Optional[Tensor], slot: Optional[Tensor]) -> None:
    if t is not None and slot is not None:
        t._rh_range = (slot, t._version)


def _disarm() -> None:
    L.lib.rh_x6_set_ranges(None, None, None, None)
    L.lib.rh_defer_reduce(None)


def _armed_call(fn):
    def wrapped(*a, **k):
        try:
            return fn(*a, **k)
        except BaseException:
            _disarm()
            raise
    return wrapped


_RANGE_MISS = None


def range_miss_log_begin() -> None:
    global _RANGE_MISS
    _RANGE_MISS = []


def range_miss_log_end():
    global _RANGE_MISS
    out, _RANGE_MISS = _RANGE_MISS, None
    return out


def _stream_of(handle, device) -> torch.cuda.Stream:
    cur = torch.cuda.current_stream(device)
    if cur.cuda_stream == handle:
        return cur
    for st in _SIDE.values():
        if st.cuda_stream == handle:
            return st
    return torch.cuda.ExternalStream(handle, device=device)


def _valid_slot(t: Tensor, s):
    r = getattr(t, "_rh_range", None)
    if r is None or r[1] != t._version or r[0].device != t.device:
        return None
    if len(r) > 2 and r[2][0] != s:
        _, captured, ev = r[2]
        now = torch.cuda.is_current_stream_capturing()
        if captured and not now:
            return None
        if captured == now:
            _stream_of(s, t.device).wait_event(ev)
    return r[0]


def _range_of(t: Tensor, s, tag: str = "") -> Tensor:
    slot = _valid_slot(t, s)
    if slot is not None:
        return slot
    base = t._base
    if base is not None and base.numel() == t.numel():
        slot = _valid_slot(base, s)
        if slot is not None:
            t._rh_range = (slot, t._version) + tuple(base._rh_range[2:])
            return slot
    if _RANGE_MISS is not None:
        _RANGE_MISS.append((tag, tuple(t.shape)))
    slot = _new_range(t.device)
    L.check(L.lib.rh_amax_f32(L.ptr(t), t.numel(), L.ptr(slot), s), "amax")
    _attach_range(t, slot)
    side = next((st for st in _SIDE.values() if st.cuda_stream == s), None)
    if side is not None:
        ev = torch.cuda.Event()
        ev.record(side)
        t._rh_range = (slot, t._version, (s, torch.cuda.is_current_stream_capturing(), ev))
    return slot


def _fwd(d, x, wp, bias, alpha, residual, y, s):
    _log_plan(d, 0, bias is not None, residual is not None)
    ws = _ws(L.lib.rh_conv1d_fwd_workspace_bytes(C.byref(d)), y.device)
    rin = rout = None
    if _ranges_on():
        if L.lib.rh_conv1d_kernel_family(C.byref(d), 0, int(bias is not None), int(residual is not None)) == 1:
            rin = _range_of(x, s, "fwd x")
        rout = _new_range(y.device)

    @_armed_call
    def run(out, ranges=True):
        if ranges and rout is not None:
            L.lib.rh_x6_set_ranges(None, L.ptr(rin), L.ptr(rout), None)
        return L.lib.rh_conv1d_fwd_f32(C.byref(d), L.ptr(x), L.ptr(wp), L.ptr(bias), L.ptr(alpha), L.ptr(residual), L.ptr(out),
                                       L.ptr(ws), ws.numel() * 4 if ws is not None else 0, s)

    rc = _launch("conv_fwd", d, lambda: run(y), bias is not None, residual is not None)
    if rc == 0:
        _attach_range(y, rout)
        _shadow("fwd", d, lambda o: run(o[0], False), [y])
    return rc


def _unit_fwd(d3, d1, x, wp3, wp1, h, y, s):
    rin = ry = rh = None
    if _RANGES:
        rin, ry = _range_of(x, s, "unit x"), _new_range(x.device)
        rh = _new_range(x.device) if h is not None else None

    @_armed_call
    def run(o_y, o_h):
        if rin is not None:
            L.lib.rh_x6_set_ranges(None, L.ptr(rin), L.ptr(ry), L.ptr(rh))
        return L.lib.rh_residual_unit_fwd_f32(C.byref(d3), C.byref(d1), L.ptr(x), L.ptr(wp3), L.ptr(wp1), L.ptr(o_h), L.ptr(o_y), s)

    if _PLAN_LOG is not None:
        _PLAN_LOG.append((2, (d3.c_in, d3.c_out, d3.kernel, d3.stride, d3.dilation, d3.l_in, d3.transposed), (3, d3.c_in // 32, 2, 1, 1, 1, 0, 0)))
    if _PROFILE is None:
        rc = run(y, h)
    else:
        f3, b3 = _conv_cost(d3)
        f1, b1 = _conv_cost(d1)
        rc = _timed("conv_fwd[x6]", f3 + f1, b3 + b1, lambda: run(y, h))
    if rc == 0:
        _attach_range(y, ry)
        _attach_range(h, rh)
    if rc == 0 and _SHADOW is not None:
        h2, y2 = torch.empty_like(x), torch.empty_like(x)
        with _ExactF32():
            nf3 = L.lib.rh_conv1d_fwd_workspace_bytes(C.byref(d3))
            nf1 = L.lib.rh_conv1d_fwd_workspace_bytes(C.byref(d1))
            ws = _ws(max(nf3, nf1, 4), x.device)
            L.check(L.lib.rh_conv1d_fwd_f32(C.byref(d3), L.ptr(x), L.ptr(wp3), None, None, None, L.ptr(h2), L.ptr(ws), ws.numel() * 4, s),
                    "shadow unit k3")
            L.check(L.lib.rh_conv1d_fwd_f32(C.byref(d1), L.ptr(h2), L.ptr(wp1), None, None, L.ptr(x), L.ptr(y2), L.ptr(ws), ws.numel() * 4, s),
                    "shadow unit k1")
        key = (d3.c_in, d3.c_out, d3.kernel, d3.stride, d3.dilation, d3.l_in, d3.transposed, d3.batch)
        _SHADOW.append(("unit", key, _rel(y, y2)))
        if h is not None:
            _SHADOW.append(("unit_h", key, _rel(h, h2)))
    return rc


def _dgrad(d, dy, wp, x, alpha, add, dx, s):
    _log_plan(d, 1, False, add is not None)
    ws = _ws(L.lib.rh_conv1d_bwd_data_workspace_bytes(C.byref(d)), dx.device)
    rin = rout = None
    if _ranges_on():
        if L.lib.rh_conv1d_kernel_family(C.byref(d), 1, 0, int(add is not None)) == 1:
            rin = _range_of(dy, s, "dgrad dy")
        rout = _new_range(dx.device)

    @_armed_call
    def run(out, ranges=True):
        if ranges and rout is not None:
            L.lib.rh_x6_set_ranges(None, L.ptr(rin), L.ptr(rout), None)
        return L.lib.rh_conv1d_bwd_data_f32(C.byref(d), L.ptr(dy), L.ptr(wp), L.ptr(x), L.ptr(alpha), L.ptr(add), L.ptr(out),
                                            L.ptr(ws), ws.numel() * 4 if ws is not None else 0, s)

    rc = _launch("conv_dgrad", d, lambda: run(dx), False, add is not None)
    if rc == 0:
        _attach_range(dx, rout)
        _shadow("dgrad", d, lambda o: run(o[0], False), [dx])
    return rc


_SIDE = {}
_SIDE_PENDING = [None]
_SIDE_HOLD = []


def _side_enabled() -> bool:
    import os
    return os.environ.get("RH_BWD_SIDE_STREAM", "1") != "0"


def _side_stream(device):
    k = device.index if device.index is not None else torch.cuda.current_device()
    st = _SIDE.get(k)
    if st is None:
        st = _SIDE[k] = torch.cuda.Stream(device=device)
    return st


_WN_PENDING = []
import os as _os
_WN_BATCH_MAX = int(_os.environ.get("RH_WN_BATCH_MAX", "64"))


def _wn_batch_enabled() -> bool:
    import os
    return os.environ.get("RH_WN_BATCH", "1") != "0"


_RED_PENDING = []
_RED_BATCH = 8


def _reduce_batch() -> int:
    import os
    e = os.environ.get("RH_REDUCE_BATCH")
    if e is not None:
        return int(e)
    return _RED_BATCH if torch.cuda.is_current_stream_capturing() else 0


def _flush_reduce_pending(stream_ptr) -> None:
    items, _RED_PENDING[:] = list(_RED_PENDING), []
    if not items:
        return
    arr = (L.ReduceItem * len(items))()
    for a, (it, _, _) in zip(arr, items):
        a.part, a.out, a.n, a.Z = it.part, it.out, it.n, it.Z
    L.check(L.lib.rh_reduce_partials_batched_f32(arr, len(items), stream_ptr), "reduce_partials_batched")


def _flush_wn_pending(stream_ptr) -> None:
    _flush_reduce_pending(stream_ptr)
    items, _WN_PENDING[:] = list(_WN_PENDING), []
    if not items:
        return
    arr = (L.WnBwdItem * len(items))()
    for a, (dw, v, g, norms, dv, dg) in zip(arr, items):
        a.dw, a.v, a.g, a.norms, a.dv, a.dg = L.ptr(dw), L.ptr(v), L.ptr(g), L.ptr(norms), L.ptr(dv), L.ptr(dg)
        a.rows = v.shape[0]
        a.cols = v.numel() // max(v.shape[0], 1)
    L.check(L.lib.rh_weight_norm_bwd_batched_f32(arr, len(items), stream_ptr), "weight_norm_bwd_batched")


def side_stream_for_collective(device):
    pend = _SIDE_PENDING[0]
    if pend is None:
        return None
    side = pend[1]
    if _WN_PENDING or _RED_PENDING:
        with torch.cuda.stream(side):
            _flush_wn_pending(L.stream())
    side.wait_stream(torch.cuda.current_stream(device))
    return side


def _graph_task_id() -> int:
    f = getattr(torch._C, "_current_graph_task_id", None)
    return int(f()) if f is not None else -1


def join_side_streams() -> None:
    pend = _SIDE_PENDING[0]
    if pend is not None:
        main, side = pend[0], pend[1]
        if _WN_PENDING or _RED_PENDING:
            with torch.cuda.stream(side):
                _flush_wn_pending(L.stream())
        main.wait_stream(side)
        torch.cuda.current_stream().wait_stream(side)
        _SIDE_PENDING[0] = None
        _SIDE_HOLD.clear()


def abandon_side_streams(rejoin: bool = False) -> None:
    if rejoin:
        cur = torch.cuda.current_stream()
        for st in _SIDE.values():
            try:
                cur.wait_stream(st)
            except Exception:
                pass
    _SIDE_PENDING[0] = None
    _SIDE_HOLD.clear()
    _WN_PENDING.clear()
    _RED_PENDING.clear()


def _note_use(ctx, *params) -> None:
    ps = [p for p in params if p is not None and p.requires_grad]
    for p in ps:
        p._rh_pending = getattr(p, "_rh_pending", 0) + 1
        if p._rh_pending > 1:
            p._rh_shared = True
    ctx.rh_params = ps


def _single_use(ctx) -> bool:
    ok = True
    for p in getattr(ctx, "rh_params", ()):
        n = getattr(p, "_rh_pending", 1)
        ok = ok and n == 1 and not getattr(p, "_rh_shared", False)
        if p.grad is not None:
            ok = False
        slot = getattr(p, "_rh_grad_slot", None)
        if slot is not None and len(slot) > 2 and slot[2] and not slot[1]:
            ok = False
        p._rh_pending = max(n - 1, 0)
        if p._rh_pending == 0:
            p._rh_shared = False
    return ok


class _OnSide:

    def __init__(self, device, *tensors, allow: bool = True, hold=()):
        self.device = device
        self.tensors = [t for t in tensors if t is not None]
        self.hold = [t for t in hold if t is not None]
        import os
        self.active = allow and _side_enabled()

    def __enter__(self):
        if not self.active:
            return self
        self.main = torch.cuda.current_stream(self.device)
        self.side = _side_stream(self.device)
        self.side.wait_stream(self.main)
        self.ctx = torch.cuda.stream(self.side)
        self.ctx.__enter__()
        return self

    def keep(self, *tensors):
        self.tensors += [t for t in tensors if t is not None]

    def __exit__(self, *exc):
        if not self.active:
            return False
        self.ctx.__exit__(*exc)
        for t in self.tensors:
            t.record_stream(self.side)
        task = _graph_task_id()
        pend = _SIDE_PENDING[0]
        if pend is not None and pend[2] != task:
            join_side_streams()
            pend = None
        if os.environ.get("RH_SIDE_HOLD", "1") != "0":
            _SIDE_HOLD.extend(self.hold)
        if pend is None:
            _SIDE_PENDING[0] = (self.main, self.side, task)
            try:
                torch.autograd.Variable._execution_engine.queue_callback(join_side_streams)
            except RuntimeError:
                join_side_streams()
        return False


def _arm_wgrad_ranges(dy, x, s, d=None) -> None:
    if _RANGES and os.environ.get("RH_WGRAD_X6", "1") != "0" and (d is None or L.lib.rh_conv1d_bwd_weight_kernel_family(C.byref(d)) == 1):
        L.lib.rh_x6_set_ranges(L.ptr(_range_of(dy, s, "wgrad dy")), L.ptr(_range_of(x, s, "wgrad x")), None, None)


def _wgrad(d, dy, x, alpha, dw, db, ws, nbytes, s, defer=None):
    @_armed_call
    def run(o_dw, o_db):
        _arm_wgrad_ranges(dy, x, s, d)
        if defer is not None:
            L.lib.rh_defer_reduce(C.byref(defer))
        return L.lib.rh_conv1d_bwd_weight_f32(C.byref(d), L.ptr(dy), L.ptr(x), L.ptr(alpha), L.ptr(o_dw), L.ptr(o_db), L.ptr(ws),
                                              nbytes, s)

    rc = _launch("conv_wgrad", d, lambda: run(dw, db))
    if rc == 0 and _SHADOW is not None:
        def run_exact(o):
            L.lib.rh_x6_set_ranges(None, None, None, None)
            nb2 = L.lib.rh_conv1d_workspace_bytes(C.byref(d))
            ws2 = torch.empty(max(nb2, 4) // 4, device=dy.device, dtype=torch.float32)
            return L.lib.rh_conv1d_bwd_weight_f32(C.byref(d), L.ptr(dy), L.ptr(x), L.ptr(alpha), L.ptr(o[0]), L.ptr(o[1]), L.ptr(ws2),
                                                  nb2, s)
        _shadow("wgrad", d, run_exact, [dw, db])
    return rc


def _shapes(x: Tensor, weight: Tensor, g: ConvGeom):
    k = weight.shape[2]
    if g.transposed:
        c_in, c_out = weight.shape[0], weight.shape[1]
    else:
        c_out, c_in = weight.shape[0], weight.shape[1]
    b = x.shape[0]
    if x.shape[1] != c_in:
        raise RuntimeError(f"rave_amd conv: input has {x.shape[1]} channels, weight expects {c_in}")
    in_valid = 0
    if g.inner > 1:
        if g.fold:
            t = x.shape[2]
            l_in = -(-t // g.inner)
            in_valid = t if l_in * g.inner != t else 0
        else:
            if x.dim() != 4 or x.shape[3] != g.inner:
                raise RuntimeError("rave_amd conv: expected (B, C, H, W) with W == inner")
            l_in = x.shape[2]
        l_out = g.out_len(l_in, k)
        out_shape = (b, c_out, l_out, g.inner)
    else:
        l_in = x.shape[2]
        l_out = g.out_len(l_in, k)
        out_shape = (b, c_out, l_out)
    return b, c_in, c_out, l_in, l_out, k, in_valid, out_shape


def _pack(d, w3, g, need_bwd, dev, s, prepacked=None):
    if prepacked is not None:
        return prepacked
    dref = C.byref(d)
    wp_f = torch.empty(L.lib.rh_conv1d_packed_floats(dref, 0), device=dev, dtype=torch.float32)
    wp_b = torch.empty(L.lib.rh_conv1d_packed_floats(dref, 1), device=dev, dtype=torch.float32) if need_bwd else None
    norms = None
    if g is not None:
        rows = w3.shape[0]
        ns = torch.empty(2, rows, device=dev, dtype=torch.float32)
        norms = ns[0]
        L.check(L.lib.rh_conv1d_pack_wn_f32(dref, L.ptr(w3), L.ptr(g), L.ptr(ns[0]), L.ptr(ns[1]), L.ptr(wp_f),
                                            L.ptr(wp_b), s), "conv1d_pack_wn")
    else:
        L.check(L.lib.rh_conv1d_pack_f32(dref, L.ptr(w3), L.ptr(wp_f), L.ptr(wp_b), s), "conv1d_pack")
    return wp_f, wp_b, norms


def _slot_of(p):
    return getattr(p, "_rh_grad_slot", None) if p is not None else None


def _grad_out(slot, shape, device) -> Tensor:
    if slot is not None and slot[1] and tuple(slot[0].shape) == tuple(shape) and slot[0].device == device:
        slot[1] = False
        return slot[0].detach()
    return torch.empty(tuple(shape), device=device, dtype=torch.float32)


def _wn_bwd(dw, v, g, norms, s, slot_v=None, slot_g=None):
    rows = v.shape[0]
    cols = v.numel() // max(rows, 1)
    dv = _grad_out(slot_v, v.shape, v.device)
    dg = _grad_out(slot_g, g.shape, g.device)
    L.check(L.lib.rh_weight_norm_bwd_f32(L.ptr(dw), L.ptr(v), L.ptr(g), L.ptr(norms), rows, cols, L.ptr(dv), L.ptr(dg), s),
            "weight_norm_bwd")
    return dv, dg


def _wgrad_wn(d, dy, x, alpha, dw, db, v, g, norms, ws, nbytes, s, slot_v=None, slot_g=None, side=None):
    if _PROFILE is not None or _SHADOW is not None:
        L.check(_wgrad(d, dy, x, alpha, dw, db, ws, nbytes, s), "conv1d_bwd_weight")
        return _wn_bwd(dw, v, g, norms, s, slot_v, slot_g)
    dv = _grad_out(slot_v, v.shape, v.device)
    dg = _grad_out(slot_g, g.shape, g.device)
    if side is not None and side.active and _wn_batch_enabled():
        nred = _reduce_batch()
        if nred > 0:
            own = torch.empty(max(nbytes, 4) // 4, device=dy.device, dtype=torch.float32)
            item = L.ReduceItem()
            L.check(_wgrad(d, dy, x, alpha, dw, db, own, nbytes, s, defer=item), "conv1d_bwd_weight")
            if item.Z > 1:
                _RED_PENDING.append((item, own, dw))
                if len(_RED_PENDING) >= nred:
                    _flush_reduce_pending(s)
        else:
            L.check(_wgrad(d, dy, x, alpha, dw, db, ws, nbytes, s), "conv1d_bwd_weight")
        _WN_PENDING.append((dw, v, g, norms, dv.detach(), dg.detach()))
        if len(_WN_PENDING) >= _WN_BATCH_MAX:
            _flush_wn_pending(s)
        return dv, dg

    @_armed_call
    def run():
        _arm_wgrad_ranges(dy, x, s, d)
        return L.lib.rh_conv1d_bwd_weight_wn_f32(C.byref(d), L.ptr(dy), L.ptr(x), L.ptr(alpha), L.ptr(v), L.ptr(g), L.ptr(norms),
                                                 L.ptr(dw), L.ptr(dv), L.ptr(dg), L.ptr(db), L.ptr(ws), nbytes, s)

    L.check(run(), "conv1d_bwd_weight_wn")
    return dv, dg


class _ConvFn(torch.autograd.Function):

    @staticmethod
    def forward(ctx, x, weight, g, bias, alpha, residual, geom: ConvGeom, prepacked=None):
        ctx.slots = (_slot_of(weight), _slot_of(g), _slot_of(bias))
        _note_use(ctx, weight, g, bias)
        _log_gate((weight, g, bias), x, geom.act)
        x = _chk(x, "x"); weight = _chk(weight, "weight"); g = _chk(g, "weight_g"); bias = _chk(bias, "bias")
        alpha = _chk(alpha, "alpha"); residual = _chk(residual, "residual")
        w3 = weight.reshape(weight.shape[0], weight.shape[1], -1) if weight.dim() == 4 else weight
        b, c_in, c_out, l_in, l_out, k, in_valid, out_shape = _shapes(x, w3, geom)
        d = _desc(geom, b, c_in, c_out, l_in, l_out, k, in_valid)
        s = L.stream()
        wp_f, wp_b, norms = _pack(d, w3, g, ctx.needs_input_grad[0], x.device, s, prepacked)
        y = torch.empty(out_shape, device=x.device, dtype=torch.float32)
        if residual is not None and residual.shape != y.shape:
            raise RuntimeError(f"rave_amd conv: residual shape {tuple(residual.shape)} != output {tuple(y.shape)}")
        L.check(_fwd(d, x, wp_f, bias, alpha, residual, y, s), "conv1d_fwd")
        ctx.save_for_backward(x, wp_b, alpha, weight if g is not None else None, g, norms,
                              y if geom.out_act != ACT_NONE else None)
        ctx.x_range = getattr(x, "_rh_range", None)
        ctx.d = d
        ctx.wshape = tuple(weight.shape)
        ctx.has_bias = bias is not None
        ctx.has_res = residual is not None
        return y

    @staticmethod
    def backward(ctx, dy):
        x, wp_b, alpha, v, g, norms, y_act = ctx.saved_tensors
        if ctx.x_range is not None and getattr(x, "_rh_range", None) is None:
            x._rh_range = ctx.x_range
        d = ctx.d
        dref = C.byref(d)
        dy = _chk(dy, "dy")
        s = L.stream()
        dx = dw = dg = db = dres = None
        side_ok = _single_use(ctx) and not (ctx.has_res and ctx.needs_input_grad[5])
        dy_in = dy if y_act is None else None
        if y_act is not None:
            gpre = torch.empty_like(dy)
            L.check(L.lib.rh_act_bwd_f32(L.ptr(dy), L.ptr(y_act), d.out_act, d.out_slope, dy.numel(), L.ptr(gpre), s),
                    "act_bwd")
            dy = gpre
        if ctx.needs_input_grad[0]:
            dx = torch.empty_like(x)
            L.check(_dgrad(d, dy, wp_b, x, alpha, None, dx, s), "conv1d_bwd_data")
        need_w = ctx.needs_input_grad[1] or (g is not None and ctx.needs_input_grad[2])
        need_b = ctx.has_bias and ctx.needs_input_grad[3]
        if need_w or need_b:
            slot_w, slot_g, slot_b = ctx.slots
            dw = _grad_out(slot_w if g is None else None, ctx.wshape, dy.device)
            if need_b:
                db = _grad_out(slot_b, (d.c_out,), dy.device)
            nbytes = L.lib.rh_conv1d_workspace_bytes(dref)
            ws = torch.empty(max(nbytes, 4) // 4, device=dy.device, dtype=torch.float32)
            with _OnSide(dy.device, dy, x, ws, dw, db, v, g, norms, alpha, allow=side_ok, hold=(dy_in,)) as side:
                s2 = L.stream()
                if g is None:
                    L.check(_wgrad(d, dy, x, alpha, dw, db, ws, nbytes, s2), "conv1d_bwd_weight")
                else:
                    dw_full = dw
                    dw, dg = _wgrad_wn(d, dy, x, alpha, dw, db, v, g, norms, ws, nbytes, s2, slot_w, slot_g, side)
                    side.keep(dw_full, dw, dg)
        if alpha is not None and ctx.needs_input_grad[4]:
            raise NotImplementedError("rave_amd: gradient w.r.t. a fused Snake alpha; use rave_amd.blocks.Snake + conv")
        if ctx.has_res and ctx.needs_input_grad[5]:
            dres = dy
        return dx, dw, dg, db, None, dres, None, None


def conv1d(x: Tensor, weight: Tensor, bias: Optional[Tensor] = None, *, geom: ConvGeom,
           alpha: Optional[Tensor] = None, residual: Optional[Tensor] = None,
           weight_g: Optional[Tensor] = None, prepacked=None) -> Tensor:
    return _ConvFn.apply(x, weight, weight_g, bias, alpha, residual, geom, prepacked)


class _WeightNormFn(torch.autograd.Function):

    @staticmethod
    def forward(ctx, v, g):
        v = _chk(v, "weight_v"); g = _chk(g, "weight_g")
        rows = v.shape[0]
        cols = v.numel() // max(rows, 1)
        w = torch.empty_like(v)
        norms = torch.empty(rows, device=v.device, dtype=torch.float32)
        L.check(L.lib.rh_weight_norm_fwd_f32(L.ptr(v), L.ptr(g), rows, cols, L.ptr(w), L.ptr(norms), L.stream()),
                "weight_norm_fwd")
        ctx.save_for_backward(v, g, norms)
        return w

    @staticmethod
    def backward(ctx, dw):
        v, g, norms = ctx.saved_tensors
        dw = _chk(dw, "dw")
        rows = v.shape[0]
        cols = v.numel() // max(rows, 1)
        dv = torch.empty_like(v)
        dg = torch.empty_like(g)
        L.check(L.lib.rh_weight_norm_bwd_f32(L.ptr(dw), L.ptr(v), L.ptr(g), L.ptr(norms), rows, cols,
                                             L.ptr(dv), L.ptr(dg), L.stream()), "weight_norm_bwd")
        return dv, dg


def weight_norm(v: Tensor, g: Tensor) -> Tensor:
    return _WeightNormFn.apply(v, g)


class _ResidualUnitFn(torch.autograd.Function):

    @staticmethod
    def forward(ctx, x, w3, g3w, w1, g1w, alpha0, alpha2, g3: ConvGeom, g1: ConvGeom, pre3=None, pre1=None):
        ctx.slots = (_slot_of(w3), _slot_of(g3w), _slot_of(w1), _slot_of(g1w))
        _note_use(ctx, w3, g3w, w1, g1w)
        gate_ids = ((w3, g3w), (w1, g1w))
        x = _chk(x, "x"); w3 = _chk(w3, "w3"); w1 = _chk(w1, "w1"); g3w = _chk(g3w, "g3"); g1w = _chk(g1w, "g1")
        alpha0 = _chk(alpha0, "alpha0"); alpha2 = _chk(alpha2, "alpha2")
        b, c, l = x.shape
        k = w3.shape[2]
        d3 = _desc(g3, b, c, c, l, l, k)
        d1 = _desc(g1, b, c, c, l, l, 1)
        s = L.stream()
        wp3f, wp3b, n3 = _pack(d3, w3, g3w, True, x.device, s, pre3)
        wp1f, wp1b, n1 = _pack(d1, w1, g1w, True, x.device, s, pre1)
        y = torch.empty_like(x)
        if alpha0 is None and alpha2 is None and L.lib.rh_residual_unit_fused(C.byref(d3), C.byref(d1)) == 1:
            h = torch.empty_like(x) if any(ctx.needs_input_grad[:5]) else None
            L.check(_unit_fwd(d3, d1, x, wp3f, wp1f, h, y, s), "residual_unit_fwd")
        else:
            h = torch.empty_like(x)
            L.check(_fwd(d3, x, wp3f, None, alpha0, None, h, s), "unit k3")
            L.check(_fwd(d1, h, wp1f, None, alpha2, x, y, s), "unit k1")
        _log_gate(gate_ids[0], x, g3.act)
        if h is not None:
            _log_gate(gate_ids[1], h, g1.act)
        ctx.save_for_backward(x, h, wp3b, wp1b, alpha0, alpha2, w3 if g3w is not None else None, g3w, n3,
                              w1 if g1w is not None else None, g1w, n1)
        ctx.d3, ctx.d1 = d3, d1
        ctx.w3shape, ctx.w1shape = tuple(w3.shape), tuple(w1.shape)
        ctx.x_range = getattr(x, "_rh_range", None)
        ctx.h_range = getattr(h, "_rh_range", None) if h is not None else None
        return y

    @staticmethod
    def backward(ctx, dy):
        x, h, wp3b, wp1b, alpha0, alpha2, v3, g3w, n3, v1, g1w, n1 = ctx.saved_tensors
        if ctx.x_range is not None and getattr(x, "_rh_range", None) is None:
            x._rh_range = ctx.x_range
        if ctx.h_range is not None and getattr(h, "_rh_range", None) is None:
            h._rh_range = ctx.h_range
        d3, d1 = ctx.d3, ctx.d1
        r3, r1 = C.byref(d3), C.byref(d1)
        dy = _chk(dy, "dy")
        s = L.stream()
        dev = dy.device
        if (alpha0 is not None and ctx.needs_input_grad[5]) or (alpha2 is not None and ctx.needs_input_grad[6]):
            raise NotImplementedError("rave_amd: Snake alpha gradient in the fused residual unit")
        dh = torch.empty_like(h)
        L.check(_dgrad(d1, dy, wp1b, h, alpha2, None, dh, s), "unit k1 dgrad")
        dw1 = dw3 = dg1 = dg3 = dx = None
        nb1 = L.lib.rh_conv1d_workspace_bytes(r1)
        nb3 = L.lib.rh_conv1d_workspace_bytes(r3)
        ws = torch.empty(max(nb1, nb3, 4) // 4, device=dev)
        with _OnSide(dev, dy, h, dh, x, ws, v3, g3w, n3, v1, g1w, n1, alpha0, alpha2, allow=_single_use(ctx), hold=(dy,)) as side:
            s2 = L.stream()
            if ctx.needs_input_grad[3] or (g1w is not None and ctx.needs_input_grad[4]):
                s3w, s3g, s1w, s1g = ctx.slots
                dw1 = _grad_out(s1w if g1w is None else None, ctx.w1shape, dev)
                side.keep(dw1)
                if g1w is None:
                    L.check(_wgrad(d1, dy, h, alpha2, dw1, None, ws, nb1, s2), "unit k1 wgrad")
                else:
                    dw1, dg1 = _wgrad_wn(d1, dy, h, alpha2, dw1, None, v1, g1w, n1, ws, nb1, s2, s1w, s1g, side)
                    side.keep(dw1, dg1)
            if ctx.needs_input_grad[1] or (g3w is not None and ctx.needs_input_grad[2]):
                s3w, s3g, s1w, s1g = ctx.slots
                dw3 = _grad_out(s3w if g3w is None else None, ctx.w3shape, dev)
                side.keep(dw3)
                if g3w is None:
                    L.check(_wgrad(d3, dh, x, alpha0, dw3, None, ws, nb3, s2), "unit k3 wgrad")
                else:
                    dw3, dg3 = _wgrad_wn(d3, dh, x, alpha0, dw3, None, v3, g3w, n3, ws, nb3, s2, s3w, s3g, side)
                    side.keep(dw3, dg3)
        if ctx.needs_input_grad[0]:
            dx = torch.empty_like(x)
            L.check(_dgrad(d3, dh, wp3b, x, alpha0, dy, dx, s), "unit k3 dgrad")
        return dx, dw3, dg3, dw1, dg1, None, None, None, None, None, None


def residual_unit(x, w3, w1, g3: ConvGeom, g1: ConvGeom, alpha0=None, alpha2=None, w3_g=None, w1_g=None,
                  pre3=None, pre1=None) -> Tensor:
    return _ResidualUnitFn.apply(x, w3, w3_g, w1, w1_g, alpha0, alpha2, g3, g1, pre3, pre1)


def _pair(v):
    return (int(v), int(v)) if isinstance(v, int) else (int(v[0]), int(v[1]))


def _conv2d_cost(d: "L.Conv2dDesc"):
    flops = 2.0 * d.batch * d.c_out * d.c_in * d.kh * d.kw * d.h_out * d.w_out
    elems = d.batch * (d.c_in * d.h_in * d.w_in + d.c_out * d.h_out * d.w_out) + d.c_out * d.c_in * d.kh * d.kw
    return flops, 4.0 * elems


def _launch2(kind: str, d, fn):
    if _PROFILE is None:
        return fn()
    if kind in ("conv2d_fwd", "conv2d_dgrad"):
        info = (C.c_int64 * 16)()
        if L.lib.rh_conv2d_plan_info(C.byref(d), 0 if kind == "conv2d_fwd" else 1, info) == 0:
            kind += _FAMILY.get(int(info[0]), "[f32]")
    elif kind == "conv2d_wgrad":
        kind += _FAMILY.get(L.lib.rh_conv2d_bwd_weight_kernel_family(C.byref(d)), "[f32]")
    f, b = _conv2d_cost(d)
    return _timed(kind, f, b, fn)


def _conv2d_ranges(d, which: int, t: Tensor, dev, s, tag: str):
    if not _ranges_on():
        return None, None
    info = (C.c_int64 * 16)()
    fam = int(info[0]) if L.lib.rh_conv2d_plan_info(C.byref(d), which, info) == 0 else 0
    rin = _range_of(t, s, tag) if fam == 1 else None
    return rin, _new_range(dev)


class _Conv2dFn(torch.autograd.Function):

    @staticmethod
    def forward(ctx, x, weight, bias, stride, padding, dilation, act: int, slope: float):
        x = _chk(x, "x"); weight = _chk(weight, "weight"); bias = _chk(bias, "bias")
        if x.dim() != 4 or weight.dim() != 4:
            raise RuntimeError("rave_amd conv2d: expects x (B,C,H,W) and weight (Co,Ci,kh,kw)")
        b, c_in, h_in, w_in = x.shape
        c_out, c_in_w, kh, kw = weight.shape
        if c_in != c_in_w:
            raise RuntimeError(f"rave_amd conv2d: input has {c_in} channels, weight expects {c_in_w}")
        (sh, sw), (ph, pw), (dh, dw) = _pair(stride), _pair(padding), _pair(dilation)
        h_out = (h_in + 2 * ph - dh * (kh - 1) - 1) // sh + 1
        w_out = (w_in + 2 * pw - dw * (kw - 1) - 1) // sw + 1
        d = L.Conv2dDesc(batch=b, c_in=c_in, c_out=c_out, h_in=h_in, w_in=w_in, h_out=h_out, w_out=w_out, kh=kh, kw=kw,
                         sh=sh, sw=sw, dh=dh, dw=dw, ph=ph, pw=pw, act=act, act_slope=slope)
        dref = C.byref(d)
        s = L.stream()
        dev = x.device
        nf = L.lib.rh_conv2d_packed_floats(dref, 0)
        if nf < 0:
            L.check(-1, "conv2d geometry")
        wp_f = torch.empty(nf, device=dev, dtype=torch.float32)
        wp_b = torch.empty(L.lib.rh_conv2d_packed_floats(dref, 1), device=dev, dtype=torch.float32) \
            if ctx.needs_input_grad[0] else None
        L.check(L.lib.rh_conv2d_pack_f32(dref, L.ptr(weight), L.ptr(wp_f), L.ptr(wp_b), s), "conv2d_pack")
        y = torch.empty(b, c_out, h_out, w_out, device=dev, dtype=torch.float32)
        rin, rout = _conv2d_ranges(d, 0, x, dev, s, "conv2d x")

        @_armed_call
        def run_fwd():
            if rout is not None:
                L.lib.rh_x6_set_ranges(None, L.ptr(rin), L.ptr(rout), None)
            return L.lib.rh_conv2d_fwd_f32(dref, L.ptr(x), L.ptr(wp_f), L.ptr(bias), L.ptr(y), s)

        L.check(_launch2("conv2d_fwd", d, run_fwd), "conv2d_fwd")
        _attach_range(y, rout)
        ctx.save_for_backward(x, y if act != ACT_NONE else None, wp_b)
        ctx.d = d
        ctx.wshape = tuple(weight.shape)
        ctx.has_bias = bias is not None
        return y

    @staticmethod
    def backward(ctx, dy):
        x, y, wp_b = ctx.saved_tensors
        d = ctx.d
        dy = _chk(dy, "dy")
        s = L.stream()
        dx = dw = db = None
        need_b = ctx.has_bias and ctx.needs_input_grad[2]
        if y is not None:
            g = torch.empty_like(dy)
            if need_b:
                db = torch.empty(d.c_out, device=dy.device, dtype=torch.float32)
                nb = L.lib.rh_act_bwd_bias_workspace_bytes(d.c_out)
                wsb = torch.empty(max(nb, 4) // 4, device=dy.device, dtype=torch.float32)
                rg = _new_range(dy.device) if _ranges_on() else None
                if rg is not None:
                    L.lib.rh_x6_set_ranges(None, None, L.ptr(rg), None)
                L.check(L.lib.rh_act_bwd_bias_f32(L.ptr(dy), L.ptr(y), d.act, d.act_slope, d.batch, d.c_out, d.h_out * d.w_out,
                                                  L.ptr(g), L.ptr(db), L.ptr(wsb), nb, s), "act_bwd_bias")
                _attach_range(g, rg)
                need_b = False
            else:
                L.check(L.lib.rh_act_bwd_f32(L.ptr(dy), L.ptr(y), d.act, d.act_slope, dy.numel(), L.ptr(g), s), "act_bwd")
            dy, y = g, None
            d = L.Conv2dDesc.from_buffer_copy(d)
            d.act = ACT_NONE
        dref = C.byref(d)
        if ctx.needs_input_grad[0]:
            dx = torch.empty_like(x)
            rin, rout = _conv2d_ranges(d, 1, dy, dy.device, s, "conv2d dy") if y is None else (None, None)

            @_armed_call
            def run_dgrad():
                if rout is not None:
                    L.lib.rh_x6_set_ranges(None, L.ptr(rin), L.ptr(rout), None)
                return L.lib.rh_conv2d_bwd_data_f32(dref, L.ptr(dy), L.ptr(y), L.ptr(wp_b), L.ptr(dx), s)

            L.check(_launch2("conv2d_dgrad", d, run_dgrad), "conv2d_bwd_data")
            _attach_range(dx, rout)
        if ctx.needs_input_grad[1] or need_b:
            dw = torch.empty(ctx.wshape, device=dy.device, dtype=torch.float32)
            if need_b:
                db = torch.empty(d.c_out, device=dy.device, dtype=torch.float32)
            nbytes = L.lib.rh_conv2d_workspace_bytes(dref)
            ws = torch.empty(max(nbytes, 4) // 4, device=dy.device, dtype=torch.float32)
            use_r = _ranges_on() and y is None and L.lib.rh_conv2d_bwd_weight_kernel_family(dref) == 1
            rdy = _range_of(dy, s, "conv2d wgrad dy") if use_r else None
            rx = _range_of(x, s, "conv2d wgrad x") if use_r else None

            @_armed_call
            def run_wgrad():
                if use_r:
                    L.lib.rh_x6_set_ranges(L.ptr(rdy), L.ptr(rx), None, None)
                return L.lib.rh_conv2d_bwd_weight_f32(dref, L.ptr(dy), L.ptr(y), L.ptr(x), L.ptr(dw), L.ptr(db) if need_b else None,
                                                      L.ptr(ws), nbytes, s)

            L.check(_launch2("conv2d_wgrad", d, run_wgrad), "conv2d_bwd_weight")
        return dx, dw, db, None, None, None, None, None


def conv2d(x: Tensor, weight: Tensor, bias: Optional[Tensor] = None, stride=1, padding=0, dilation=1,
           act: int = ACT_NONE, slope: float = 0.2) -> Tensor:
    return _Conv2dFn.apply(x, weight, bias, stride, padding, dilation, act, float(slope))


class _PqmfAnalysisFn(torch.autograd.Function):
    @staticmethod
    def forward(ctx, x, w, pad: Tuple[int, int], fold=None):
        x = _chk(x, "x"); w = _chk(w, "forward_conv.weight")
        rows, one, t = x.shape
        if one != 1:
            raise RuntimeError("pqmf analysis expects (B*C, 1, T)")
        m, _, k = w.shape
        n_frames = (t + pad[0] + pad[1] - k) // m + 1
        y = torch.empty(rows, m, n_frames, device=x.device, dtype=torch.float32)
        if fold is not None:
            tab, lpad = fold
            ry = _new_range(x.device) if _ranges_on() else None
            if ry is not None:
                L.lib.rh_x6_set_ranges(None, None, L.ptr(ry), None)
            L.check(L.lib.rh_pqmf_fold_k1_f32(L.ptr(x), L.ptr(tab), rows, t, n_frames, lpad - pad[0], 1.0, L.ptr(y), L.stream()),
                    "pqmf_fold_k1")
            _attach_range(y, ry)
        else:
            L.check(L.lib.rh_pqmf_analysis_fwd_f32(L.ptr(x), L.ptr(w), rows, t, m, k, pad[0], n_frames, L.ptr(y), L.stream()),
                    "pqmf_analysis_fwd")
        ctx.save_for_backward(w)
        ctx.geo = (rows, t, m, k, pad[0], n_frames)
        ctx.fold = fold
        return y

    @staticmethod
    def backward(ctx, dy):
        (w,) = ctx.saved_tensors
        rows, t, m, k, pl, n_frames = ctx.geo
        dy = _chk(dy, "dy")
        dx = torch.empty(rows, 1, t, device=dy.device, dtype=torch.float32)
        if ctx.fold is not None:
            tab, lpad = ctx.fold
            L.check(L.lib.rh_pqmf_fold_k2_f32(L.ptr(dy), L.ptr(tab), rows, n_frames, t, pl - lpad, 1.0, L.ptr(dx), L.stream()),
                    "pqmf_fold_k2")
        else:
            L.check(L.lib.rh_pqmf_analysis_bwd_f32(L.ptr(dy), L.ptr(w), rows, t, m, k, pl, n_frames, L.ptr(dx), L.stream()),
                    "pqmf_analysis_bwd")
        return dx, None, None, None


class _PqmfSynthesisFn(torch.autograd.Function):
    @staticmethod
    def forward(ctx, y, w, pad: Tuple[int, int], fold=None):
        y = _chk(y, "y"); w = _chk(w, "inverse_conv.weight")
        rows, m, n_frames = y.shape
        k = w.shape[2]
        n_out = n_frames + pad[0] + pad[1] - k + 1
        x = torch.empty(rows, 1, n_out * m, device=y.device, dtype=torch.float32)
        if fold is not None:
            tab, lpad = fold
            L.check(L.lib.rh_pqmf_fold_k2_f32(L.ptr(y), L.ptr(tab), rows, n_frames, n_out * m, 496 - 16 * pad[0] - lpad, 16.0,
                                              L.ptr(x), L.stream()), "pqmf_fold_k2")
        else:
            L.check(L.lib.rh_pqmf_synthesis_fwd_f32(L.ptr(y), L.ptr(w), rows, n_frames, m, k, pad[0], n_out, L.ptr(x), L.stream()),
                    "pqmf_synthesis_fwd")
        ctx.save_for_backward(w)
        ctx.geo = (rows, n_frames, m, k, pad[0], n_out)
        ctx.fold = fold
        return x

    @staticmethod
    def backward(ctx, dx):
        (w,) = ctx.saved_tensors
        rows, n_frames, m, k, pl, n_out = ctx.geo
        dx = _chk(dx, "dx")
        dy = torch.empty(rows, m, n_frames, device=dx.device, dtype=torch.float32)
        if ctx.fold is not None:
            tab, lpad = ctx.fold
            L.check(L.lib.rh_pqmf_fold_k1_f32(L.ptr(dx), L.ptr(tab), rows, n_out * m, n_frames, lpad - (496 - 16 * pl), 16.0,
                                              L.ptr(dy), L.stream()), "pqmf_fold_k1")
        else:
            L.check(L.lib.rh_pqmf_synthesis_bwd_f32(L.ptr(dx), L.ptr(w), rows, n_frames, m, k, pl, n_out, L.ptr(dy), L.stream()),
                    "pqmf_synthesis_bwd")
        return dy, None, None, None


def pqmf_analysis(x: Tensor, w: Tensor, pad: Tuple[int, int], fold=None) -> Tensor:
    return _PqmfAnalysisFn.apply(x, w, pad, fold)


def pqmf_synthesis(y: Tensor, w: Tensor, pad: Tuple[int, int], fold=None) -> Tensor:
    return _PqmfSynthesisFn.apply(y, w, pad, fold)


class _AmpTanhFn(torch.autograd.Function):
    @staticmethod
    def forward(ctx, x):
        x = _chk(x, "x")
        b, c2, l = x.shape
        y = torch.empty(b, c2 // 2, l, device=x.device, dtype=torch.float32)
        L.check(L.lib.rh_amp_tanh_fwd_f32(L.ptr(x), b, c2 // 2, l, L.ptr(y), L.stream()), "amp_tanh_fwd")
        ctx.save_for_backward(x)
        return y

    @staticmethod
    def backward(ctx, dy):
        (x,) = ctx.saved_tensors
        dy = _chk(dy, "dy")
        b, c2, l = x.shape
        dx = torch.empty_like(x)
        L.check(L.lib.rh_amp_tanh_bwd_f32(L.ptr(dy), L.ptr(x), b, c2 // 2, l, L.ptr(dx), L.stream()), "amp_tanh_bwd")
        return dx


def amp_tanh(x: Tensor) -> Tensor:
    return _AmpTanhFn.apply(x)


class _SnakeFn(torch.autograd.Function):

    @staticmethod
    def forward(ctx, x, alpha):
        x = _chk(x, "x"); alpha = _chk(alpha, "alpha")
        b, c, l = x.shape
        y = torch.empty_like(x)
        L.check(L.lib.rh_act_fwd_f32(L.ptr(x), L.ptr(alpha), ACT_SNAKE, 0.0, b, c, l, L.ptr(y), L.stream()), "snake_fwd")
        ctx.save_for_backward(x, alpha)
        return y

    @staticmethod
    def backward(ctx, dy):
        x, alpha = ctx.saved_tensors
        dy = _chk(dy, "dy")
        b, c, l = x.shape
        dx = torch.empty_like(x)
        da = torch.empty_like(alpha)
        nbytes = L.lib.rh_snake_bwd_workspace_bytes(b, c)
        ws = torch.empty(max(nbytes, 4) // 4, device=x.device, dtype=torch.float32)
        L.check(L.lib.rh_snake_bwd_f32(L.ptr(dy), L.ptr(x), L.ptr(alpha), b, c, l, L.ptr(dx), L.ptr(da), L.ptr(ws),
                                       nbytes, L.stream()), "snake_bwd")
        return dx, da


def snake(x: Tensor, alpha: Tensor) -> Tensor:
    return _SnakeFn.apply(x, alpha)


class _AdainTransferFn(torch.autograd.Function):

    @staticmethod
    def forward(ctx, x, mean_x, std_x, mean_y, std_y):
        x = _chk(x, "x")
        b, c, l = x.shape
        for t in (mean_x, std_x, mean_y, std_y):
            if t.dim() < 2 or b > t.shape[0] or t.shape[1] != c or t[:b].numel() != b * c:
                raise ValueError(f"adain statistics {tuple(t.shape)} do not cover a batch of {b} x {c} channels")
        stats = [_chk(t[:b], "statistics") for t in (mean_x, std_x, mean_y, std_y)]
        y = torch.empty_like(x)
        L.check(L.lib.rh_adain_transfer_f32(L.ptr(x), b * c, l, *[L.ptr(t) for t in stats], L.ptr(y), L.stream()), "adain_transfer")
        ctx.save_for_backward(stats[1], stats[3])
        return y

    @staticmethod
    def backward(ctx, dy):
        std_x, std_y = ctx.saved_tensors
        dy = _chk(dy, "dy")
        b, c, l = dy.shape
        zero = torch.zeros_like(std_x)
# ... 439 lines not shown
```

Measured before the change: 243.2 million samples/s.

## Group up to three same-shape conv1d weight-gradient problems into one x6 kernel launch

```diff
diff --git a/include/rave_hip.h b/include/rave_hip.h
--- a/include/rave_hip.h
+++ b/include/rave_hip.h
@@ -119,6 +119,20 @@
                                 const float* v, const float* g, const float* norms, float* dw_scratch, float* dv,
                                 float* dg, float* dbias, void* workspace, int64_t workspace_bytes, rh_stream_t stream);
 int64_t rh_conv1d_bwd_weight_wn_fused_launches(void);
+typedef struct rh_wgrad_group_item {
+    const float* dy;
+    const float* x;
+    const float* snake_alpha;
+    float* dw;
+    float* dbias;
+    void* workspace;
+    int64_t workspace_bytes;
+    const uint32_t* dy_range;
+    const uint32_t* x_range;
+} rh_wgrad_group_item;
+int rh_conv1d_bwd_weight_group_f32(const rh_conv1d_desc* descs, const rh_wgrad_group_item* items, int32_t n,
+                                   rh_reduce_item* defer, rh_stream_t stream);
+int rh_conv1d_bwd_weight_group_plan_info(const rh_conv1d_desc* descs, int32_t n, int32_t* out8);
 
 
 int rh_pqmf_analysis_fwd_f32(const float* x, const float* w, int32_t rows, int32_t t_len,
diff --git a/rave_amd/_lib.py b/rave_amd/_lib.py
--- a/rave_amd/_lib.py
+++ b/rave_amd/_lib.py
@@ -37,6 +37,11 @@
 
 class ReduceItem(C.Structure):
     _fields_ = [("part", C.c_void_p), ("out", C.c_void_p), ("n", C.c_int64), ("Z", C.c_int32), ("reserved", C.c_int32)]
+
+
+class WgradGroupItem(C.Structure):
+    _fields_ = [("dy", C.c_void_p), ("x", C.c_void_p), ("snake_alpha", C.c_void_p), ("dw", C.c_void_p), ("dbias", C.c_void_p),
+                ("workspace", C.c_void_p), ("workspace_bytes", C.c_int64), ("dy_range", C.c_void_p), ("x_range", C.c_void_p)]
 
 
 class LossItem(C.Structure):
@@ -92,6 +97,8 @@
         "rh_conv1d_bwd_weight_f32": ([D, P, P, P, P, P, P, I64, P], C.c_int),
         "rh_conv1d_bwd_weight_wn_f32": ([D, P, P, P, P, P, P, P, P, P, P, P, I64, P], C.c_int),
         "rh_conv1d_bwd_weight_wn_fused_launches": ([], I64),
+        "rh_conv1d_bwd_weight_group_f32": ([D, C.POINTER(WgradGroupItem), I32, C.POINTER(ReduceItem), P], C.c_int),
+        "rh_conv1d_bwd_weight_group_plan_info": ([D, I32, C.POINTER(C.c_int32)], C.c_int),
         "rh_conv2d_packed_floats": ([D2, C.c_int], I64),
         "rh_conv2d_pack_f32": ([D2, P, P, P, P], C.c_int),
         "rh_conv2d_fwd_f32": ([D2, P, P, P, P, P], C.c_int),
diff --git a/rave_amd/csrc/conv_host.hip b/rave_amd/csrc/conv_host.hip
--- a/rave_amd/csrc/conv_host.hip
+++ b/rave_amd/csrc/conv_host.hip
@@ -832,6 +832,19 @@
     return rh_wgrad_run(d, dy, x, snake_alpha, dw, dbias, workspace, workspace_bytes, (hipStream_t)stream, armed);
 }
 
+extern "C" int rh_conv1d_bwd_weight_group_f32(const rh_conv1d_desc* descs, const rh_wgrad_group_item* items, int32_t n,
+                                              rh_reduce_item* defer, rh_stream_t stream) {
+    const RhKernelEventsScope events;
+    RH_REQUIRE(descs && items && n >= 1 && n <= 3, RH_ERR_INVALID, "conv1d_bwd_weight_group: 1 ... 3 problems");
+    for (int i = 0; i < n; ++i) {
+        if (int e = validate(&descs[i])) return e;
+        RH_REQUIRE(items[i].dw && (descs[i].batch == 0 || (items[i].dy && items[i].x)), RH_ERR_INVALID, "conv1d_bwd_weight_group: null pointer");
+        RH_REQUIRE(descs[i].act != RH_ACT_SNAKE || items[i].snake_alpha, RH_ERR_INVALID, "conv1d_bwd_weight_group: snake needs alpha");
+        if (defer) defer[i] = rh_reduce_item{};
+    }
+    return rh_wgrad_group_run(n, descs, items, defer, (hipStream_t)stream);
+}
+
 extern "C" int rh_conv1d_bwd_weight_wn_f32(const rh_conv1d_desc* d, const float* dy, const float* x, const float* snake_alpha,
                                            const float* v, const float* g, const float* norms, float* dw_scratch, float* dv,
                                            float* dg, float* dbias, void* workspace, int64_t workspace_bytes, rh_stream_t stream) {
diff --git a/rave_amd/csrc/conv_params.hpp b/rave_amd/csrc/conv_params.hpp
--- a/rave_amd/csrc/conv_params.hpp
+++ b/rave_amd/csrc/conv_params.hpp
@@ -125,6 +125,7 @@
 RhWgradArmed rh_wgrad_take_armed(bool may_defer);
 int rh_wgrad_run(const rh_conv1d_desc* d, const float* dy, const float* x, const float* alpha, float* dw, float* dbias, void* ws,
                  int64_t ws_bytes, hipStream_t stream, const RhWgradArmed& armed, const RhWnTail* tail = nullptr);
+int rh_wgrad_group_run(int n, const rh_conv1d_desc* descs, const rh_wgrad_group_item* items, rh_reduce_item* defer, hipStream_t stream);
 
 int rh_conv_fill_fwd(const rh_conv1d_desc* d, ConvP* p);
 int rh_conv_fill_dgrad(const rh_conv1d_desc* d, ConvP* p);
diff --git a/rave_amd/csrc/conv_wgrad.hip b/rave_amd/csrc/conv_wgrad.hip
--- a/rave_amd/csrc/conv_wgrad.hip
+++ b/rave_amd/csrc/conv_wgrad.hip
@@ -704,6 +704,66 @@
     return RH_OK;
 }
 
+void rh_wgrad_x6_group_plan_info(int n, const WgradP* w, int32_t* out8);
+int rh_wgrad_x6_group_launch(int n, const WgradP* w, float* const* dw, float* const* rsum_out, void* const* ws, const int64_t* ws_bytes,
+                             hipStream_t stream, bool* used, int* left_z, const unsigned* const* r_range, const unsigned* const* s_range);
+constexpr int kWgradGroupMax = 3;
+
+extern "C" int rh_conv1d_bwd_weight_group_plan_info(const rh_conv1d_desc* descs, int32_t n, int32_t* out8) {
+    if (!descs || !out8 || n < 1 || n > kWgradGroupMax) return RH_ERR_INVALID;
+    for (int i = 0; i < 8; ++i) out8[i] = 0;
+    WgradP p[kWgradGroupMax] = {};
+    alignas(16) static const float dummy[4] = {0.f, 0.f, 0.f, 0.f};
+    for (int i = 0; i < n; ++i) {
+        if (descs[i].batch <= 0 || rh_conv1d_bwd_weight_kernel_family(&descs[i]) != 1) return RH_OK;
+        fill(&descs[i], &p[i]);
+        p[i].R = dummy; p[i].S = dummy;
+    }
+    rh_wgrad_x6_group_plan_info(n, p, out8);
+    return RH_OK;
+}
+
+int rh_wgrad_group_run(int n, const rh_conv1d_desc* descs, const rh_wgrad_group_item* it, rh_reduce_item* defer, hipStream_t stream) {
+    WgradP p[kWgradGroupMax] = {};
+    float* dw[kWgradGroupMax]; float* db[kWgradGroupMax]; void* ws[kWgradGroupMax]; int64_t wsb[kWgradGroupMax];
+    const unsigned* rr[kWgradGroupMax]; const unsigned* sr[kWgradGroupMax];
+    bool groupable = n >= 2;
+    for (int i = 0; i < n && groupable; ++i) {
+        const rh_conv1d_desc* d = &descs[i];
+        fill(d, &p[i]);
+        if (!d->transposed) { p[i].R = it[i].dy; p[i].S = it[i].x; p[i].s_alpha = it[i].snake_alpha; }
+        else                { p[i].R = it[i].x; p[i].S = it[i].dy; p[i].r_alpha = it[i].snake_alpha; }
+        groupable = (!RH_X6_F16 || (it[i].dy_range && it[i].x_range)) && d->act != RH_ACT_SNAKE && p[i].B > 0 && p[i].r_row > 0 &&
+                    !rh_smallc_wgrad_eligible(d) && rh_wgrad_x6_workspace(p[i]) >= 0 && (!it[i].dbias || !d->transposed);
+        const int64_t bias_ws = rh_bias_grad_workspace(d->c_out);
+        dw[i] = it[i].dw; db[i] = it[i].dbias;
+        ws[i] = it[i].workspace ? (void*)((char*)it[i].workspace + bias_ws) : nullptr;
+        wsb[i] = it[i].workspace_bytes > bias_ws ? it[i].workspace_bytes - bias_ws : 0;
+        rr[i] = d->transposed ? it[i].x_range : it[i].dy_range;
+        sr[i] = d->transposed ? it[i].dy_range : it[i].x_range;
+    }
+    if (groupable) {
+        bool used = false;
+        int left_z[kWgradGroupMax] = {};
+        if (int e = rh_wgrad_x6_group_launch(n, p, dw, db, ws, wsb, stream, &used, defer ? left_z : nullptr, rr, sr)) return e;
+        if (used) {
+            for (int i = 0; i < n && defer; ++i)
+                if (left_z[i] > 1) {
+                    defer[i].part = (const float*)ws[i]; defer[i].out = dw[i];
+                    defer[i].n = (int64_t)p[i].M * p[i].C * p[i].T; defer[i].Z = left_z[i];
+                }
+            return RH_OK;
+        }
+    }
+    for (int i = 0; i < n; ++i) {
+        const RhWgradArmed armed{defer ? &defer[i] : nullptr, it[i].dy_range, it[i].x_range};
+        if (int e = rh_wgrad_run(&descs[i], it[i].dy, it[i].x, it[i].snake_alpha, it[i].dw, it[i].dbias, it[i].workspace,
+                                 it[i].workspace_bytes, stream, armed))
+            return e;
+    }
+    return RH_OK;
+}
+
 int64_t rh_wgrad_workspace(const rh_conv1d_desc* d) {
     WgradP p{};
     fill(d, &p);
diff --git a/rave_amd/csrc/conv_wgrad_x6.hip b/rave_amd/csrc/conv_wgrad_x6.hip
--- a/rave_amd/csrc/conv_wgrad_x6.hip
+++ b/rave_amd/csrc/conv_wgrad_x6.hip
@@ -276,7 +276,7 @@
 }
 
 template <int TM, int WM, int WN, bool AV, bool PART, bool PL>
-__global__ __launch_bounds__(256, 2) void wgrad_x6_kernel(const Wx6P p) {
+__device__ __forceinline__ void wgrad_x6_tile(const Wx6P& p, const int bx, const int by, const int z) {
     static_assert(WM * WN == 4, "four waves");
     constexpr int NT = 256, BM = 32 * TM * WM, BN = 64 * WN;
     constexpr int NB = PL ? ((BN / 2 + 2) * 7 + NT - 1) / NT : kOct * BN / NT;
@@ -288,7 +288,7 @@
     const int wave = __builtin_amdgcn_readfirstlane(tid >> 6);
     const int j = lane & 31, g = lane >> 5;
     const int wm = wave / WN, wn = wave - wm * WN;
-    const int m0 = blockIdx.y * BM, n0 = blockIdx.x * BN, z = blockIdx.z;
+    const int m0 = by * BM, n0 = bx * BN;
 
     const auto r_rsrc = __builtin_amdgcn_make_buffer_rsrc(const_cast<float*>(p.R), 0, p.r_bytes, 0x00020000);
     const auto s_rsrc = __builtin_amdgcn_make_buffer_rsrc(const_cast<float*>(p.S), 0, p.s_bytes, 0x00020000);
@@ -310,7 +310,7 @@
 #pragma unroll
             for (int r = 0; r < 16; ++r) acc[tm][tn][r] = 0.f;
 
-    const bool want_rsum = p.rsum != nullptr && blockIdx.x == 0;
+    const bool want_rsum = p.rsum != nullptr && bx == 0;
     auto load = [&](int st) {
         const Wx6Step sp = wx6_step<PL>(p, st);
         rt.load(p, r_rsrc, sp, AV);
@@ -354,6 +354,25 @@
 #pragma unroll
         for (int tm = 0; tm < TM; ++tm) wx6_store_tile(p, outz, acc[tm][tn], m0 + (wm * TM + tm) * 32 + 4 * g, col, sc.out);
     }
+}
+
+template <int TM, int WM, int WN, bool AV, bool PART, bool PL>
+__global__ __launch_bounds__(256, 2) void wgrad_x6_kernel(const Wx6P p) {
+    wgrad_x6_tile<TM, WM, WN, AV, PART, PL>(p, blockIdx.x, blockIdx.y, blockIdx.z);
+}
+
+constexpr int kWx6Group = 3;
+struct Wx6Group {
+    Wx6P p[kWx6Group];
+    int z0[kWx6Group];
+};
+static_assert(sizeof(Wx6Group) <= 4096, "kernel-argument segment");
+
+template <int TM, int WM, int WN, bool AV, bool PART, bool PL>
+__global__ __launch_bounds__(256, 2) void wgrad_x6_group_kernel(const Wx6Group g) {
+    const int bz = blockIdx.z;
+    const int i = (bz >= g.z0[1] ? 1 : 0) + (bz >= g.z0[2] ? 1 : 0);
+    wgrad_x6_tile<TM, WM, WN, AV, PART, PL>(g.p[i], blockIdx.x, blockIdx.y, bz - g.z0[i]);
 }
 
 template <int NW, bool PL>
@@ -446,6 +465,7 @@
     int blocks;
     int all;
     int tm;
+    int group;
     bool forced_tm() const { return tm >= 1 && tm <= 3; }
 };
 
@@ -453,7 +473,8 @@
     const auto num = [](const char* name, int dflt) { const char* e = getenv(name); return e ? atoi(e) : dflt; };
     static const int all = num("RH_WGRAD_X6_ALL", 0), tm = num("RH_WGRAD_X6_TM", 0);
     const char* pe = getenv("RH_WGRAD_X6_PLANES");
-    return Wx6Env{num("RH_WGRAD_X6", 1) == 0, pe ? (pe[0] == '1' ? 1 : 0) : -1, num("RH_WGRAD_X6_WIDE", 1), num("RH_WGRAD_X6_BLOCKS", 0), all, tm};
+    return Wx6Env{num("RH_WGRAD_X6", 1) == 0, pe ? (pe[0] == '1' ? 1 : 0) : -1, num("RH_WGRAD_X6_WIDE", 1), num("RH_WGRAD_X6_BLOCKS", 0), all, tm,
+                  num("RH_WGRAD_X6_GROUP", 1)};
 }
 
 bool wx6_eligible(const WgradP& w, const Wx6Env& env, const unsigned* r_range, const unsigned* s_range) {
@@ -516,7 +537,7 @@
     p->steps_per_z = pl->steps_per_z;
 }
 
-bool plan_wx6(const WgradP& w, Wx6P* p, Wx6Plan* pl, const unsigned* r_range, const unsigned* s_range) {
+bool plan_wx6(const WgradP& w, Wx6P* p, Wx6Plan* pl, const unsigned* r_range, const unsigned* s_range, int share = 1) {
     const Wx6Env env = read_wx6_env();
     if (!wx6_eligible(w, env, r_range, s_range)) return false;
     *p = Wx6P{};
@@ -531,7 +552,7 @@
     p->minoff = w.minoff; p->maxoff = w.maxoff;
     p->r_range = r_range; p->s_range = s_range;
     for (int t = 0; t < w.T; ++t) p->off[t] = w.off[t];
-    wx6_slice_k(env, wx6_choose_tile(w, env, p, pl), p, pl);
+    wx6_slice_k(env, wx6_choose_tile(w, env, p, pl) * share, p, pl);
     return true;
 }
 
@@ -553,13 +574,46 @@
     return r;
 }
 
+int wx6_av(const Wx6P& p) { return p.r_row % 4 == 0 && ((uintptr_t)p.R & 15) == 0; }
+int wx6_part(const Wx6P& p, const Wx6Plan& pl) { return rh_cdiv(p.N, 32) % (2 * (4 / pl.wm)) != 0; }
+int wx6_instance_code(const Wx6P& p, const Wx6Plan& pl) {
+    if (pl.nw > 0) return 1000 + 2 * pl.nw + pl.planes;
+    return ((((pl.tm * 4 + pl.wm) * 2 + wx6_av(p)) * 2 + wx6_part(p, pl)) * 2) + (pl.planes && pl.tm >= 2 ? 1 : 0);
+}
+
+using Wx6GroupLaunch = void (*)(dim3 grid, size_t lds, hipStream_t stream, const Wx6Group& g);
+
+template <void (*KERN)(Wx6Group)>
+void launch_wx6_group(dim3 grid, size_t lds, hipStream_t stream, const Wx6Group& g) {
+    static std::once_flag once;
+    std::call_once(once, [] {
+        (void)hipFuncSetAttribute(reinterpret_cast<const void*>(KERN), hipFuncAttributeMaxDynamicSharedMemorySize, 160 * 1024);
+    });
+    rh_launch_main(KERN, grid, dim3(256), lds, stream, g);
+}
+
+Wx6GroupLaunch wx6_group_instance(const Wx6P& p, const Wx6Plan& pl) {
+    if (pl.nw > 0 || pl.wm != 2 || pl.planes || pl.tm < 2) return nullptr;
+    const int av = wx6_av(p), part = wx6_part(p, pl);
+    Wx6GroupLaunch r = nullptr;
+    const auto pick = [&](auto TM) {
+        constexpr int tm = decltype(TM)::value;
+        if (av && part) r = launch_wx6_group<wgrad_x6_group_kernel<tm, 2, 2, true, true, false>>;
+        else if (av) r = launch_wx6_group<wgrad_x6_group_kernel<tm, 2, 2, true, false, false>>;
+        else if (part) r = launch_wx6_group<wgrad_x6_group_kernel<tm, 2, 2, false, true, false>>;
+        else r = launch_wx6_group<wgrad_x6_group_kernel<tm, 2, 2, false, false, false>>;
+    };
+    if (pl.tm == 2) pick(std::integral_constant<int, 2>{});
+    else pick(std::integral_constant<int, 3>{});
+    return r;
+}
+
 Wx6Launch wx6_instance(const Wx6P& p, const Wx6Plan& pl) {
     if (pl.nw > 0)
         return wx6_pick<3, 4, 6, 9>(pl.nw, [&](auto NW) {
             return wx6_pick<0, 1>(pl.planes, [&](auto PL) -> Wx6Launch { return launch_wx6<wgrad_x6_wide_kernel<decltype(NW)::value, decltype(PL)::value != 0>>; });
         });
-    const int av = p.r_row % 4 == 0 && ((uintptr_t)p.R & 15) == 0;
-    const int part = rh_cdiv(p.N, 32) % (2 * (4 / pl.wm)) != 0;
+    const int av = wx6_av(p), part = wx6_part(p, pl);
     return wx6_pick<1, 2, 3>(pl.tm, [&](auto TM) {
         return wx6_pick<1, 2>(pl.wm, [&](auto WM) {
             return wx6_pick<0, 1>(av, [&](auto AV) {
@@ -575,6 +629,75 @@
     });
 }
 
+bool plan_wx6_group(int n, const WgradP* w, Wx6P* p, Wx6Plan* pl, const unsigned* const* r_range, const unsigned* const* s_range,
+                    Wx6GroupLaunch* launch) {
+    const Wx6Env env = read_wx6_env();
+    if (env.group == 0 || n < 2 || n > kWx6Group) return false;
+    const int share = env.group == 2 ? 1 : n;
+    for (int i = 0; i < n; ++i) {
+        if (!plan_wx6(w[i], &p[i], &pl[i], r_range[i], s_range[i], share)) return false;
+        if (pl[i].nw > 0) return false;
+        if (i > 0 && (wx6_instance_code(p[i], pl[i]) != wx6_instance_code(p[0], pl[0]) || pl[i].rt != pl[0].rt || pl[i].ct != pl[0].ct ||
+                      pl[i].lds != pl[0].lds))
+            return false;
+    }
+    *launch = wx6_group_instance(p[0], pl[0]);
+    return *launch != nullptr;
+}
+
+}
+
+void rh_wgrad_x6_group_plan_info(int n, const WgradP* w, int32_t* out8) {
+    static const unsigned any_range[kRangeSlotWords] = {};
+    const unsigned* const rr[kWx6Group] = {any_range, any_range, any_range};
+    Wx6P p[kWx6Group];
+    Wx6Plan pl[kWx6Group] = {};
+    Wx6GroupLaunch launch = nullptr;
+    for (int i = 0; i < 8; ++i) out8[i] = 0;
+    if (n < 1 || n > kWx6Group) return;
+    const bool grouped = plan_wx6_group(n, w, p, pl, rr, rr, &launch);
+    out8[0] = grouped ? 1 : 0;
+    for (int i = 0; i < n; ++i) {
+        if (!grouped && !plan_wx6(w[i], &p[i], &pl[i], any_range, any_range)) continue;
+        if (i == 0) { out8[1] = wx6_instance_code(p[0], pl[0]); out8[6] = pl[0].steps_per_z; out8[7] = pl[0].rt * pl[0].ct; }
+        out8[2] += pl[i].rt * pl[i].ct * pl[i].Z;
+        out8[3 + i] = pl[i].Z;
+    }
+}
+
+int rh_wgrad_x6_group_launch(int n, const WgradP* w, float* const* dw, float* const* rsum_out, void* const* ws, const int64_t* ws_bytes,
+                             hipStream_t stream, bool* used, int* left_z, const unsigned* const* r_range, const unsigned* const* s_range) {
+    *used = false;
+    Wx6Group g{};
+    Wx6Plan pl[kWx6Group] = {};
+    Wx6GroupLaunch launch = nullptr;
+    if (!plan_wx6_group(n, w, g.p, pl, r_range, s_range, &launch)) return RH_OK;
+    float* rs_part[kWx6Group] = {};
+    int zsum = 0;
+    for (int i = 0; i < kWx6Group; ++i) g.z0[i] = 0x7fffffff;
+    for (int i = 0; i < n; ++i) {
+        const int64_t nw = (int64_t)w[i].M * w[i].C * w[i].T;
+        const int64_t need = pl[i].Z > 1 ? (int64_t)pl[i].Z * (nw + w[i].M) * (int64_t)sizeof(float) : 0;
+        RH_REQUIRE(need == 0 || (ws[i] && ws_bytes[i] >= need), RH_ERR_WORKSPACE,
+                   "conv1d_bwd_weight_group: workspace %lld B < %lld B", (long long)ws_bytes[i], (long long)need);
+        g.p[i].out = pl[i].Z > 1 ? (float*)ws[i] : dw[i];
+        rs_part[i] = (float*)ws[i] + (pl[i].Z > 1 ? pl[i].Z * nw : 0);
+        g.p[i].rsum = rsum_out[i] ? (pl[i].Z > 1 ? rs_part[i] : rsum_out[i]) : nullptr;
+        g.z0[i] = zsum;
+        zsum += pl[i].Z;
+    }
+    launch(dim3(pl[0].ct, pl[0].rt, zsum), pl[0].lds, stream, g);
+    if (int e = rh_check_launch("conv1d_bwd_weight_x6_group")) return e;
+    *used = true;
+    for (int i = 0; i < n; ++i) {
+        if (left_z) left_z[i] = 0;
+        if (pl[i].Z <= 1) continue;
+        if (left_z) left_z[i] = pl[i].Z;
+        else if (int e = rh_reduce_partials_launch((const float*)ws[i], dw[i], (long)w[i].M * w[i].C * w[i].T, pl[i].Z, stream, "conv1d_bwd_weight_reduce")) return e;
+        if (rsum_out[i])
+            if (int e = rh_reduce_partials_launch(rs_part[i], rsum_out[i], w[i].M, pl[i].Z, stream, "conv1d_bwd_bias_reduce")) return e;
+    }
+    return RH_OK;
 }
 
 int64_t rh_wgrad_x6_workspace(const WgradP& w) {
diff --git a/rave_amd/ops.py b/rave_amd/ops.py
--- a/rave_amd/ops.py
+++ b/rave_amd/ops.py
@@ -498,6 +498,7 @@
 
 
 def side_stream_for_collective(device):
+    _wq_flush()
     pend = _SIDE_PENDING[0]
     if pend is None:
         return None
@@ -515,6 +516,7 @@
 
 
 def join_side_streams() -> None:
+    launched = _wq_flush()
     pend = _SIDE_PENDING[0]
     if pend is not None:
         main, side = pend[0], pend[1]
@@ -525,6 +527,12 @@
         torch.cuda.current_stream().wait_stream(side)
         _SIDE_PENDING[0] = None
         _SIDE_HOLD.clear()
+    else:
+        for side in launched:
+            if _WN_PENDING or _RED_PENDING:
+                with torch.cuda.stream(side):
+                    _flush_wn_pending(L.stream())
+            torch.cuda.current_stream().wait_stream(side)
 
 
 def abandon_side_streams(rejoin: bool = False) -> None:
@@ -539,10 +547,15 @@
     _SIDE_HOLD.clear()
     _WN_PENDING.clear()
     _RED_PENDING.clear()
+    _WQ.clear()
+    _WQ_TASK[0] = None
+
+
+_GRAD_MODE = [True]
 
 
 def _note_use(ctx, *params) -> None:
-    ps = [p for p in params if p is not None and p.requires_grad]
+    ps = [p for p in params if p is not None and p.requires_grad] if _GRAD_MODE[0] else []
     for p in ps:
         p._rh_pending = getattr(p, "_rh_pending", 0) + 1
         if p._rh_pending > 1:
@@ -634,6 +647,133 @@
                                                   nb2, s)
         _shadow("wgrad", d, run_exact, [dw, db])
     return rc
+
+
+_WQ = {}
+_WQ_TASK = [None]
+_WQ_OK = {}
+_WQ_GROUP = 3
+
+
+class _WqEntry:
+    __slots__ = ("d", "dy", "x", "alpha", "dw", "db", "ws", "nbytes", "rdy", "rx", "wn", "device")
+
+
+def _wq_key(d, dy, alpha, db, wn):
+    return (dy.device, d.batch, d.c_in, d.c_out, d.l_in, d.l_out, d.kernel, d.stride, d.transposed, d.inner, d.in_valid, d.act,
+            d.act_slope, d.out_act, d.out_slope, alpha is not None, db is not None, wn is not None,
+            os.environ.get("RH_WGRAD_X6_GROUP", "1"))
+
+
+def _wq_wanted(d, key) -> bool:
+    if os.environ.get("RH_WGRAD_X6_GROUP", "1") == "0" or _SHADOW is not None or not _RANGES or os.environ.get("RH_WGRAD_X6", "1") == "0":
+        return False
+    ok = _WQ_OK.get(key)
+    if ok is None:
+        out = (C.c_int32 * 8)()
+        pair = (L.ConvDesc * 2)(d, d)
+        ok = _WQ_OK[key] = L.lib.rh_conv1d_bwd_weight_group_plan_info(pair, 2, out) == 0 and out[0] == 1
+    return ok
+
+
+def _wq_launch(key) -> None:
+    entries = _WQ.pop(key, [])
+    if not entries:
+        return
+    n = len(entries)
+    s = L.stream()
+    on_side = any(st.cuda_stream == s for st in _SIDE.values())
+    descs = (L.ConvDesc * n)(*[e.d for e in entries])
+    items = (L.WgradGroupItem * n)()
+    for it, e in zip(items, entries):
+        it.dy, it.x, it.snake_alpha, it.dw, it.dbias = L.ptr(e.dy), L.ptr(e.x), L.ptr(e.alpha), L.ptr(e.dw), L.ptr(e.db)
+        it.workspace, it.workspace_bytes, it.dy_range, it.x_range = L.ptr(e.ws), e.nbytes, L.ptr(e.rdy), L.ptr(e.rx)
+    nred = _reduce_batch() if on_side else 0
+    defer = (L.ReduceItem * n)() if nred > 0 else None
+
+    def run():
+        return L.lib.rh_conv1d_bwd_weight_group_f32(descs, items, n, defer, s)
+
+    if _PROFILE is not None:
+        cost = [_conv_cost(e.d) for e in entries]
+        rc = _timed("conv_wgrad[x6]", sum(c[0] for c in cost), sum(c[1] for c in cost), run)
+    else:
+        rc = run()
+    L.check(rc, "conv1d_bwd_weight_group")
+    for i, e in enumerate(entries):
+        if defer is not None and defer[i].Z > 1:
+            item = L.ReduceItem()
+            item.part, item.out, item.n, item.Z = defer[i].part, defer[i].out, defer[i].n, defer[i].Z
+            _RED_PENDING.append((item, e.ws, e.dw))
+            if len(_RED_PENDING) >= nred:
+                _flush_reduce_pending(s)
+    for e in entries:
+        if e.wn is None:
+            continue
+        v, g, norms, dv, dg = e.wn
+        if on_side and _wn_batch_enabled():
+            _WN_PENDING.append((e.dw, v, g, norms, dv, dg))
+            if len(_WN_PENDING) >= _WN_BATCH_MAX:
+                _flush_wn_pending(s)
+        else:
+            _flush_reduce_pending(s)
+            rows = v.shape[0]
+            L.check(L.lib.rh_weight_norm_bwd_f32(L.ptr(e.dw), L.ptr(v), L.ptr(g), L.ptr(norms), rows, v.numel() // max(rows, 1),
+                                                 L.ptr(dv), L.ptr(dg), s), "weight_norm_bwd")
+
+
+def _wq_flush():
+    launched = []
+    if not _WQ:
+        return launched
+    keys = [k for k in _WQ if _WQ[k]]
+    if _side_enabled():
+        for dev in dict.fromkeys(k[0] for k in keys):
+            side = _side_stream(dev)
+            if torch.cuda.current_stream(dev) != side:
+                side.wait_stream(torch.cuda.current_stream(dev))
+            with torch.cuda.stream(side):
+                for k in keys:
+                    if k[0] == dev:
+                        _wq_launch(k)
+            launched.append(side)
+    else:
+        for k in keys:
+            _wq_launch(k)
+    _WQ.clear()
+    return launched
+
+
+def _wq_end_of_pass() -> None:
+    _WQ_TASK[0] = None
+    if _WQ:
+        join_side_streams()
+
+
+def _wq_push(d, dy, x, alpha, dw, db, nbytes, s, wn=None) -> bool:
+    key = _wq_key(d, dy, alpha, db, wn)
+    if not _wq_wanted(d, key):
+        return False
+    task = _graph_task_id()
+    if _WQ and _WQ_TASK[0] is not None and _WQ_TASK[0] != task:
+        _wq_flush()
+    e = _WqEntry()
+    e.d, e.dy, e.x, e.alpha, e.nbytes, e.wn, e.device = d, dy, x, alpha, nbytes, wn, dy.device
+    e.dw = dw.detach() if wn is None else dw
+    e.db = db.detach() if db is not None else None
+    e.rdy, e.rx = _range_of(dy, s, "wgrad dy"), _range_of(x, s, "wgrad x")
+    e.ws = torch.empty(max(nbytes, 4) // 4, device=dy.device, dtype=torch.float32)
+    q = _WQ.setdefault(key, [])
+    q.append(e)
+    if len(q) >= _WQ_GROUP:
+        _wq_launch(key)
+    if task < 0 or _WQ_TASK[0] != task:
+        try:
+            torch.autograd.Variable._execution_engine.queue_callback(_wq_end_of_pass)
+            _WQ_TASK[0] = task
+        except RuntimeError:
+            _wq_flush()
+    return True
 
 
 def _shapes(x: Tensor, weight: Tensor, g: ConvGeom):
@@ -693,22 +833,32 @@
     return torch.empty(tuple(shape), device=device, dtype=torch.float32)
 
 
-def _wn_bwd(dw, v, g, norms, s, slot_v=None, slot_g=None):
+def _wn_bwd(dw, v, g, norms, s, slot_v=None, slot_g=None, dv=None, dg=None):
     rows = v.shape[0]
     cols = v.numel() // max(rows, 1)
-    dv = _grad_out(slot_v, v.shape, v.device)
-    dg = _grad_out(slot_g, g.shape, g.device)
+    if dv is None:
+        dv = _grad_out(slot_v, v.shape, v.device)
+        dg = _grad_out(slot_g, g.shape, g.device)
     L.check(L.lib.rh_weight_norm_bwd_f32(L.ptr(dw), L.ptr(v), L.ptr(g), L.ptr(norms), rows, cols, L.ptr(dv), L.ptr(dg), s),
             "weight_norm_bwd")
     return dv, dg
 
 
-def _wgrad_wn(d, dy, x, alpha, dw, db, v, g, norms, ws, nbytes, s, slot_v=None, slot_g=None, side=None):
+def _wgrad_wn(d, dy, x, alpha, dw, db, v, g, norms, ws, nbytes, s, slot_v=None, slot_g=None, side=None, queue=False):
+    if queue:
+        dv = _grad_out(slot_v, v.shape, v.device)
+        dg = _grad_out(slot_g, g.shape, g.device)
+        if _wq_push(d, dy, x, alpha, dw, db, nbytes, s, wn=(v, g, norms, dv.detach(), dg.detach())):
+            return dv, dg
+        slot_v = slot_g = None
+    else:
+        dv = dg = None
     if _PROFILE is not None or _SHADOW is not None:
         L.check(_wgrad(d, dy, x, alpha, dw, db, ws, nbytes, s), "conv1d_bwd_weight")
-        return _wn_bwd(dw, v, g, norms, s, slot_v, slot_g)
-    dv = _grad_out(slot_v, v.shape, v.device)
-    dg = _grad_out(slot_g, g.shape, g.device)
+        return _wn_bwd(dw, v, g, norms, s, slot_v, slot_g, dv, dg)
+    if dv is None:
+        dv = _grad_out(slot_v, v.shape, v.device)
+        dg = _grad_out(slot_g, g.shape, g.device)
     if side is not None and side.active and _wn_batch_enabled():
         nred = _reduce_batch()
         if nred > 0:
@@ -810,6 +960,7 @@
 def conv1d(x: Tensor, weight: Tensor, bias: Optional[Tensor] = None, *, geom: ConvGeom,
            alpha: Optional[Tensor] = None, residual: Optional[Tensor] = None,
            weight_g: Optional[Tensor] = None, prepacked=None) -> Tensor:
+    _GRAD_MODE[0] = torch.is_grad_enabled()
     return _ConvFn.apply(x, weight, weight_g, bias, alpha, residual, geom, prepacked)
 
 
@@ -899,25 +1050,28 @@
         nb1 = L.lib.rh_conv1d_workspace_bytes(r1)
         nb3 = L.lib.rh_conv1d_workspace_bytes(r3)
         ws = torch.empty(max(nb1, nb3, 4) // 4, device=dev)
-        with _OnSide(dev, dy, h, dh, x, ws, v3, g3w, n3, v1, g1w, n1, alpha0, alpha2, allow=_single_use(ctx), hold=(dy,)) as side:
+        single = _single_use(ctx)
+        with _OnSide(dev, dy, h, dh, x, ws, v3, g3w, n3, v1, g1w, n1, alpha0, alpha2, allow=single, hold=(dy,)) as side:
             s2 = L.stream()
             if ctx.needs_input_grad[3] or (g1w is not None and ctx.needs_input_grad[4]):
                 s3w, s3g, s1w, s1g = ctx.slots
                 dw1 = _grad_out(s1w if g1w is None else None, ctx.w1shape, dev)
                 side.keep(dw1)
                 if g1w is None:
-                    L.check(_wgrad(d1, dy, h, alpha2, dw1, None, ws, nb1, s2), "unit k1 wgrad")
+                    if not (single and _wq_push(d1, dy, h, alpha2, dw1, None, nb1, s2)):
+                        L.check(_wgrad(d1, dy, h, alpha2, dw1, None, ws, nb1, s2), "unit k1 wgrad")
                 else:
-                    dw1, dg1 = _wgrad_wn(d1, dy, h, alpha2, dw1, None, v1, g1w, n1, ws, nb1, s2, s1w, s1g, side)
+                    dw1, dg1 = _wgrad_wn(d1, dy, h, alpha2, dw1, None, v1, g1w, n1, ws, nb1, s2, s1w, s1g, side, queue=single)
                     side.keep(dw1, dg1)
             if ctx.needs_input_grad[1] or (g3w is not None and ctx.needs_input_grad[2]):
                 s3w, s3g, s1w, s1g = ctx.slots
                 dw3 = _grad_out(s3w if g3w is None else None, ctx.w3shape, dev)
                 side.keep(dw3)
                 if g3w is None:
-                    L.check(_wgrad(d3, dh, x, alpha0, dw3, None, ws, nb3, s2), "unit k3 wgrad")
+                    if not (single and _wq_push(d3, dh, x, alpha0, dw3, None, nb3, s2)):
+                        L.check(_wgrad(d3, dh, x, alpha0, dw3, None, ws, nb3, s2), "unit k3 wgrad")
                 else:
-                    dw3, dg3 = _wgrad_wn(d3, dh, x, alpha0, dw3, None, v3, g3w, n3, ws, nb3, s2, s3w, s3g, side)
+                    dw3, dg3 = _wgrad_wn(d3, dh, x, alpha0, dw3, None, v3, g3w, n3, ws, nb3, s2, s3w, s3g, side, queue=single)
                     side.keep(dw3, dg3)
         if ctx.needs_input_grad[0]:
             dx = torch.empty_like(x)
@@ -927,6 +1081,7 @@
 
 def residual_unit(x, w3, w1, g3: ConvGeom, g1: ConvGeom, alpha0=None, alpha2=None, w3_g=None, w1_g=None,
                   pre3=None, pre1=None) -> Tensor:
+    _GRAD_MODE[0] = torch.is_grad_enabled()
     return _ResidualUnitFn.apply(x, w3, w3_g, w1, w1_g, alpha0, alpha2, g3, g1, pre3, pre1)
 
 
```

Result: no change. 245.2 million samples/s, median of 6 (+0.8%).
